# ushasigh/srsran-edgeric-5g

Measured on AMD Instinct MI355X. Metric: pdsch_slots_per_sec, higher is better.
Workload: dtype u32 bit-packed GF(2) + bf16 grid + f32 IQ

## Files before the change

### profiles/check_re_loop.py

```python
#!/usr/bin/env python3
import os
import subprocess
import tempfile

ROOT = os.path.dirname(os.path.dirname(os.path.abspath(__file__)))
C = os.path.join(ROOT, "srsran-edgeric-5g_amd", "csrc")
with tempfile.TemporaryDirectory() as tmp:
    subprocess.run(["/opt/rocm/bin/hipcc", "--offload-arch=gfx950", "-O3", "-std=c++17", "-fPIC", "-I" + os.path.join(ROOT, "include"), "-I" + C,
                    "-ffp-contract=off", "-x", "hip", "-c", os.path.join(C, "pdsch_kernels.hip"), "-o", os.path.join(tmp, "o.o"), "-save-temps"],
                   cwd=tmp, check=True, capture_output=True)
    isa = open(os.path.join(tmp, "pdsch_kernels-hip-amdgcn-amd-amdhsa-gfx950.s")).read().split("\n")
begin = next(i for i, l in enumerate(isa) if l.startswith("_ZN5nrphy18codeblock_kernel_tILi8ELi4EEE"))
end = next(i for i in range(begin, len(isa)) if "s_endpgm" in isa[i])
k = isa[begin:end + 1]
code = [l for l in k if l.startswith("\t") and not l.strip().startswith(";")]
print("codeblock_kernel_t<8, 4>: %d instructions, v_readlane %d, v_writelane %d (the v_readlane are the wave reductions' row folds)" % (
    len(code), sum("v_readlane" in l for l in code), sum("v_writelane" in l for l in code)))
idx = [i for i, l in enumerate(k) if "v_pk_mul_f32" in l and ", s[" in l][-16:]
start = max(i for i in range(idx[0]) if "Loop Header" in k[i])
stop = next(i for i in range(idx[-1], len(k)) if "s_cbranch" in k[i] or "s_endpgm" in k[i])
body = [l for l in k[start:stop + 1] if l.startswith("\t") and not l.strip().startswith(";")]
print("grid loop, four ports (from its loop header to the branch behind the last product): %d instructions" % len(body))
for what in ("v_pk_mul_f32", "v_pk_fma_f32", "v_pk_add_f32", "v_cvt_pk_bf16_f32", "buffer_store_dword", "ds_read", "global_load", "s_load", "v_readlane", "v_writelane"):
    print("  %-20s %d" % (what, sum(what in l for l in body)))
print("  scalar loads in the loop region (symbol change and the rare group that straddles a symbol; none per 64 RE, none of weights):")
for l in body:
    if "s_load" in l:
        print("     " + l.strip())
```

### srsran-edgeric-5g_amd/csrc/nrphy_host.cpp

```cpp
#include "nrphy_host_internal.h"
#include "nrphy_trace.h"

#include <algorithm>
#include <cmath>
#include <complex>
#include <cstdlib>
#include <cstring>
#include <array>
#include <map>
#include <mutex>
#include <new>
#include <vector>

using namespace nrphy;

namespace {

struct nr_ldpc_edge_t {
  uint8_t  row;
  uint8_t  col;
  uint16_t shift[8];
};
#include "nr_ldpc_bg.inc"

const uint16_t LIFTING_SIZES[NOF_LIFTING_SIZES] = {
    2,  3,  4,  5,  6,  7,  8,  9,  10, 11, 12, 13,  14,  15,  16,  18,  20,  22,  24,  26,  28,  30,  32,  36,  40, 44,
    48, 52, 56, 60, 64, 72, 80, 88, 96, 104, 112, 120, 128, 144, 160, 176, 192, 208, 224, 240, 256, 288, 320, 352, 384};

int lifting_position(unsigned zc)
{
  for (int i = 0; i != NOF_LIFTING_SIZES; ++i) {
    if (LIFTING_SIZES[i] == zc) {
      return i;
    }
  }
  return -1;
}

int lifting_set_index(unsigned zc)
{
  static const unsigned base[8] = {2, 3, 5, 7, 9, 11, 13, 15};
  for (int i = 0; i != 8; ++i) {
    for (unsigned v = base[i]; v <= 384; v *= 2) {
      if (v == zc) {
        return i;
      }
    }
  }
  return -1;
}

unsigned divide_ceil(unsigned a, unsigned b)
{
  return (a + b - 1) / b;
}

bool mask_test(const uint64_t* w, unsigned i)
{
  return (w[i >> 6] >> (i & 63)) & 1U;
}

int mask_lowest(const uint64_t* w)
{
  for (unsigned i = 0; i != 64 * NRPHY_PRB_WORDS; ++i) {
    if (mask_test(w, i)) {
      return (int)i;
    }
  }
  return -1;
}

int mask_highest(const uint64_t* w)
{
  int hi = -1;
  for (unsigned i = 0; i != 64 * NRPHY_PRB_WORDS; ++i) {
    if (mask_test(w, i)) {
      hi = (int)i;
    }
  }
  return hi;
}

void build_lifted_graph(unsigned bg, unsigned zc, LiftedGraph& g)
{
  const nr_ldpc_edge_t* edges   = (bg == 1) ? NR_LDPC_BG1_EDGES : NR_LDPC_BG2_EDGES;
  const unsigned        n_edges = (bg == 1) ? NR_LDPC_BG1_NOF_EDGES : NR_LDPC_BG2_NOF_EDGES;
  const unsigned        kb      = (bg == 1) ? 22 : 10;
  const unsigned        rows    = (bg == 1) ? 46 : 42;
  const int             ils     = lifting_set_index(zc);
  std::memset(&g, 0, sizeof(g));
  int      core_shift[4] = {-1, -1, -1, -1};
  unsigned count         = 0;
  for (unsigned m = 0; m != rows; ++m) {
    g.row_ptr[m] = (uint16_t)count;
    for (unsigned e = 0; e != n_edges; ++e) {
      if (edges[e].row != m) {
        continue;
      }
      unsigned col = edges[e].col, shift = edges[e].shift[ils] % zc;
      if (m < 4) {
        if (col == kb) {
          core_shift[m] = (int)shift;
        }
        if (col >= kb) {
          continue;
        }
      } else if (col >= kb + 4) {
        continue;
      }
      if (m < 4 && (zc & 31U) == 0) {
        const unsigned wpb = zc / 32, sh = shift & 31U, q = shift >> 5;
        const unsigned qd = (sh != 0) ? q : (q + wpb - 1) % wpb, sd = (32U - sh) & 31U;
        g.edge[count++] = ((4U * (2U * wpb * col + qd)) << 16) | sd;
        continue;
      }
      g.edge[count++] = ((col * zc) << 16) | shift;
    }
  }
  for (unsigned m = rows; m != MAX_BG_ROWS + 2; ++m) {
    g.row_ptr[m] = (uint16_t)count;
  }
  unsigned mid = (core_shift[1] >= 0) ? 1 : 2;
  int      s0 = core_shift[0], s3 = core_shift[3], sm = core_shift[mid];
  g.core_mid = (uint16_t)mid;
  g.core_s0  = (uint16_t)s0;
  g.core_s3  = (uint16_t)s3;
  g.core_b   = (uint16_t)((s0 == s3) ? sm : ((s0 == sm) ? s3 : s0));
}

void mat_mul(const uint32_t* a, const uint32_t* b, uint32_t* out)
{
  uint32_t bt[31];
  for (int c = 0; c != 31; ++c) {
    uint32_t col = 0;
    for (int r = 0; r != 31; ++r) {
      col |= ((b[r] >> c) & 1U) << r;
    }
    bt[c] = col;
  }
  uint32_t tmp[31];
  for (int r = 0; r != 31; ++r) {
    uint32_t row = 0;
    for (int c = 0; c != 31; ++c) {
      row |= (uint32_t)(__builtin_popcount(a[r] & bt[c]) & 1) << c;
    }
    tmp[r] = row;
  }
  std::memcpy(out, tmp, sizeof(tmp));
}


void build_tbcrc_tables(TbCrcTables& t)
{
  const CrcField* field[2] = {&CRC24A_FIELD, &CRC16_FIELD};
  for (unsigned s = 0; s != 2; ++s) {
    const CrcField& f  = *field[s];
    const uint32_t  y32 = f.xpow(32), y1k = f.xpow(32 * 1024), y8k = f.xpow(128 * 64), yz = f.xpow(8 * (int64_t)TB_CRC_REGION_BYTES);
    for (unsigned k = 0; k != 4; ++k) {
      for (uint32_t b = 0; b != 256; ++b) {
        t.y32[s][k][b] = f.mul(y32, b << (8 * k));
        t.y1k[s][k][b] = f.mul(y1k, b << (8 * k));
        t.y8k[s][k][b] = f.mul(y8k, b << (8 * k));
        t.yz[s][k][b]  = f.mul(yz, b << (8 * k));
      }
    }
    for (unsigned l = 0; l != 64; ++l) {
      t.lane[s][l] = f.xpow(128 * (63 - (int)l));
    }
  }
}

void build_gold_tables(GoldTables& t, std::vector<uint32_t>& x1_words)
{
  std::memset(&t, 0, sizeof(t));
  uint32_t m[31];
  for (int r = 0; r != 30; ++r) {
    m[r] = 1U << (r + 1);
  }
  m[30] = 0xF;
  for (int k = 0; k != GOLD_JUMP_BITS; ++k) {
    std::memcpy(t.x2_jump[k], m, sizeof(m));
    mat_mul(m, m, m);
  }
  for (int i = 0; i != 31; ++i) {
    uint32_t st = 1U << i;
    for (int n = 0; n != 992; ++n) {
      if (st & 1U) {
        t.x2_head[n & 31][n >> 5] |= 1U << i;
      }
      uint32_t f = ((st >> 3) ^ (st >> 2) ^ (st >> 1) ^ st) & 1U;
      st         = (st >> 1) | (f << 30);
    }
  }
  const uint32_t poly = 0x1800063U, top = 1U << 24;
  uint32_t       v    = 1;
  for (int i = 0; i != CRC_POW_WORDS; ++i) {
    t.crc24b_pow32[i] = v;
    for (int s = 0; s != 32; ++s) {
      v <<= 1;
      if (v & top) {
        v ^= poly;
      }
    }
  }
  for (uint32_t b = 0; b != 256; ++b) {
    uint32_t r = b << 16;
    for (int k = 0; k != 8; ++k) {
      r <<= 1;
      if (r & top) {
        r ^= poly;
      }
    }
    t.crc24b_table[b] = r & (top - 1);
  }
  for (uint32_t b = 0; b != 256; ++b) {
    uint32_t r            = t.crc24b_table[b];
    t.crc24b_slice[0][b] = r;
    for (int k = 1; k != 4; ++k) {
      for (int s = 0; s != 8; ++s) {
        r <<= 1;
        if (r & top) {
          r ^= poly;
        }
      }
      t.crc24b_slice[k][b] = r;
    }
  }
  {
    auto mulx = [&](uint32_t a, unsigned e) {
      for (unsigned s = 0; s != e; ++s) {
        a <<= 1;
        if (a & top) {
          a ^= poly;
        }
      }
      return a;
    };
    for (unsigned m = 0; m != CRC_POW_WORDS; ++m) {
      for (unsigned n = 0; n != 6; ++n) {
        uint32_t e = mulx(t.crc24b_pow32[m], 4 * n);
        uint32_t bit[4];
        for (unsigned k = 0; k != 4; ++k) {
          bit[k] = mulx(e, k);
        }
        for (uint32_t nib = 0; nib != 16; ++nib) {
          uint32_t acc = 0;
          for (unsigned k = 0; k != 4; ++k) {
            acc ^= ((nib >> k) & 1U) ? bit[k] : 0U;
          }
          t.crc24b_mul[m][n][nib] = acc;
        }
      }
    }
  }
  for (unsigned q = 0; q != 4; ++q) {
    const unsigned qm = 2 * (q + 1), h = q + 1;
    for (unsigned idx = 0; idx != (1U << qm); ++idx) {
      int re = 1 - 2 * (int)((idx >> 1) & 1U), im = 1 - 2 * (int)(idx & 1U);
      for (unsigned lvl = 1; lvl < h; ++lvl) {
        re = (1 - 2 * (int)((idx >> (2 * lvl + 1)) & 1U)) * ((1 << lvl) - re);
        im = (1 - 2 * (int)((idx >> (2 * lvl)) & 1U)) * ((1 << lvl) - im);
      }
      t.qam_lut[q][idx] = make_float2((float)re, (float)im);
    }
  }
  x1_words.assign(GOLD_X1_WORDS, 0);
  uint32_t x1 = 1;
  for (int i = 0; i != 1600; ++i) {
    uint32_t f = ((x1 >> 3) ^ x1) & 1U;
    x1         = (x1 >> 1) | (f << 30);
  }
  for (size_t n = 0; n != (size_t)GOLD_X1_WORDS * 32; ++n) {
    if (x1 & 1U) {
      x1_words[n >> 5] |= 0x80000000U >> (n & 31);
    }
    uint32_t f = ((x1 >> 3) ^ x1) & 1U;
    x1         = (x1 >> 1) | (f << 30);
  }
}

}

struct nrphy_pdsch_plan {
  nrphy_ctx*            ctx = nullptr;
  std::vector<PduDev>   pdus;
  std::vector<uint64_t> cw_offset;
  uint64_t              cw_bits = 0;
  uint32_t              nof_grids = 0, grid_nof_ports = 0, grid_nof_subc = 0;
  void*                 d_arena = nullptr;
  bool                  arena_external = false;
  PduDev*               d_pdus = nullptr;
  CbWork*               d_work = nullptr;
  DmrsWork*             d_dmrs = nullptr;
  float*                d_weights = nullptr;
  uint16_t*             d_re_table = nullptr;
  uint32_t*             d_tb_crc = nullptr;
  CrcWork*              d_crc_work = nullptr;
  ScrWork*              d_scr_work = nullptr;
  uint32_t              n_scr_work = 0;
  ZeroWork*             d_zero_work = nullptr;
  ZeroSeg*              d_zero_segs = nullptr;
  uint32_t*             d_scr = nullptr;
  uint64_t              scr_words = 0;
  uint64_t              seed_offset = 0;
  uint32_t              n_zero_work = 0;
  bool                  encode_only = false;
  bool                  dmrs_separate = false;
  uint32_t              n_work = 0, n_dmrs = 0, n_cb = 0, n_crc_work = 0;
  uint32_t              lds_lin_words = 0, lds_symb_words = 0, lds_graph_words = 0, lds_u_words = 0;
  uint32_t              bucket_begin[CB_BUCKETS + 1] = {};
  static constexpr uint32_t MAX_AUX = 3;
  hipStream_t           aux_stream[MAX_AUX] = {};
  hipEvent_t            fork_event = nullptr, join_event[MAX_AUX] = {};
  uint32_t              n_aux = 0;
  std::vector<hipEvent_t> events;
  std::vector<uint8_t>  timed_dmrs;
  uint32_t              timed_runs = 0, max_timed_runs = 0;
  uint32_t              timing_stride = 1, timing_counter = 0;
};

static bool plan_side_streams(nrphy_pdsch_plan* plan, uint32_t want);

struct nrphy_ofdm_plan {
  nrphy_ctx*          ctx = nullptr;
  nrphy_ofdm_config_t cfg;
  uint32_t            nof_ports = 0, nsymb = 14, slot_stride = 0, nsym_subframe = 0;
  const float2*       d_twiddle = nullptr;
  float2*             d_phase = nullptr;
  float2*             d_phase_rx = nullptr;
  uint32_t*           d_cp = nullptr;
  uint32_t*           d_off = nullptr;
  std::vector<uint32_t> cp, off;
  std::map<uint32_t, float2*> d_window_phase;
  std::mutex          window_mutex;
  std::vector<hipEvent_t> events;
  uint32_t            timed_runs = 0, max_timed_runs = 0;
  uint32_t            timing_stride = 1, timing_counter = 0;
  uint4*              d_wire_partials = nullptr;
  size_t              wire_partials_cap = 0;
};

extern "C" const char* nrphy_version(void)
{
  return "mi355-nrphy 0.1 (gfx950)";
}

extern "C" int nrphy_trace_enabled(void)
{
  return trace_enabled() ? 1 : 0;
}

extern "C" const char* nrphy_strerror(int status)
{
  switch (status) {
    case NRPHY_OK:
      return "ok";
    case NRPHY_ERR_INVALID_PDU:
      return "invalid PDSCH PDU (pdsch_pdu_validator::is_valid is false)";
    case NRPHY_ERR_ARGUMENT:
      return "invalid argument";
    case NRPHY_ERR_DEVICE:
      return "HIP device error (no GPU or kernel launch failure); there is no CPU fallback";
    case NRPHY_ERR_CAPACITY:
      return "capacity exceeded";
    default:
      return "unknown status";
  }
}

extern "C" int nrphy_pdsch_validate(const nrphy_pdsch_pdu_t* pdu)
{
  if (pdu == nullptr) {
    return NRPHY_ERR_ARGUMENT;
  }
  const unsigned nsymb = pdu->cp ? 12 : 14;
  const int      lo = mask_lowest(pdu->prb_mask), hi = mask_highest(pdu->prb_mask);
  if (lo < 0 || (unsigned)lo < pdu->bwp_start_rb || (unsigned)hi >= pdu->bwp_start_rb + pdu->bwp_size_rb ||
      pdu->bwp_start_rb + pdu->bwp_size_rb > NRPHY_MAX_RB) {
    return NRPHY_ERR_INVALID_PDU;
  }
  if (pdu->dmrs_symbol_mask == 0 || (pdu->dmrs_symbol_mask >> nsymb) != 0) {
    return NRPHY_ERR_INVALID_PDU;
  }
  const unsigned first_dmrs = (unsigned)__builtin_ctz(pdu->dmrs_symbol_mask);
  const unsigned last_dmrs  = 31U - (unsigned)__builtin_clz(pdu->dmrs_symbol_mask);
  if (first_dmrs < pdu->start_symbol_index || last_dmrs >= pdu->start_symbol_index + pdu->nof_symbols ||
      nsymb < pdu->start_symbol_index + pdu->nof_symbols) {
    return NRPHY_ERR_INVALID_PDU;
  }
  if (pdu->dmrs_type != 1 || pdu->nof_cdm_groups_without_data > 2 || !pdu->vrb_contiguous) {
    return NRPHY_ERR_INVALID_PDU;
  }
  for (int prb = lo; prb <= hi; ++prb) {
    if (!mask_test(pdu->prb_mask, (unsigned)prb)) {
      return NRPHY_ERR_INVALID_PDU;
    }
  }
  if (pdu->nof_ports == 0 || pdu->nof_ports > NRPHY_MAX_PORTS || pdu->nof_layers == 0 ||
      pdu->nof_layers > pdu->nof_ports) {
    return NRPHY_ERR_INVALID_PDU;
  }
  if (pdu->nof_codewords != 1 || pdu->tbs_lbrm_bytes == 0 || pdu->nof_reserved > NRPHY_MAX_RESERVED) {
    return NRPHY_ERR_INVALID_PDU;
  }
  for (unsigned r = 0; r != pdu->nof_reserved; ++r) {
    if (pdu->reserved[r].symbol_mask & pdu->dmrs_symbol_mask) {
      return NRPHY_ERR_INVALID_PDU;
    }
  }
  if ((pdu->qm != 2 && pdu->qm != 4 && pdu->qm != 6 && pdu->qm != 8) || pdu->rv > 3 ||
      (pdu->ldpc_base_graph != 1 && pdu->ldpc_base_graph != 2) || pdu->tb_size_bytes == 0 ||
      pdu->tb_size_bytes > NRPHY_MAX_TB_BYTES || pdu->nof_prg == 0 || pdu->nof_prg > NRPHY_MAX_PRG || pdu->prg_size_rb == 0 || pdu->prg_size_rb > NRPHY_MAX_RB || pdu->precoding == nullptr || pdu->cp > 1) {
    return NRPHY_ERR_INVALID_PDU;
  }
  return NRPHY_OK;
}

namespace {

void data_re_mask(const nrphy_pdsch_pdu_t& pdu, unsigned l, std::vector<uint8_t>& mask)
{
  std::fill(mask.begin(), mask.end(), 0);
  if (l < pdu.start_symbol_index || l >= pdu.start_symbol_index + pdu.nof_symbols) {
    return;
  }
  const unsigned nof_prb = (unsigned)mask.size() / 12;
  for (unsigned p = 0; p != nof_prb; ++p) {
    if (mask_test(pdu.prb_mask, p)) {
      std::fill(mask.begin() + 12 * p, mask.begin() + 12 * p + 12, 1);
    }
  }
  for (unsigned r = 0; r != pdu.nof_reserved; ++r) {
    const nrphy_re_pattern_t& pat = pdu.reserved[r];
    if (!((pat.symbol_mask >> l) & 1U)) {
      continue;
    }
    for (unsigned p = 0; p != nof_prb; ++p) {
      if (!mask_test(pat.prb_mask, p)) {
        continue;
      }
      for (unsigned k = 0; k != 12; ++k) {
        if ((pat.re_mask >> k) & 1U) {
          mask[12 * p + k] = 0;
        }
      }
    }
  }
  if ((pdu.dmrs_symbol_mask >> l) & 1U) {
    for (unsigned p = pdu.bwp_start_rb; p < pdu.bwp_start_rb + pdu.bwp_size_rb && p < nof_prb; ++p) {
      for (unsigned k = 0; k != 12; ++k) {
        if ((k % 2) < pdu.nof_cdm_groups_without_data) {
          mask[12 * p + k] = 0;
        }
      }
    }
  }
}

void derive(const nrphy_pdsch_pdu_t& pdu, unsigned nof_re, nrphy_pdsch_derived_t& d,
            const uint32_t* nref_override = nullptr)
{
  const unsigned bg      = pdu.ldpc_base_graph;
  const unsigned tb_bits = 8 * pdu.tb_size_bytes;
  const unsigned tb_crc  = (tb_bits <= 3824) ? 16 : 24;
  const unsigned b       = tb_bits + tb_crc;
  const unsigned kcb     = (bg == 1) ? 8448 : 3840;
  const unsigned C       = (b <= kcb) ? 1 : divide_ceil(b, kcb - 24);
  const unsigned b_out   = b + ((C > 1) ? 24 * C : 0);
  unsigned       ref_len = 22;
  if (bg == 2) {
    ref_len = (b > 640) ? 10 : (b > 560) ? 9 : (b > 192) ? 8 : 6;
  }
  unsigned zc = 0;
  for (unsigned i = 0; i != NOF_LIFTING_SIZES; ++i) {
    if (LIFTING_SIZES[i] * C * ref_len >= b_out) {
      zc = LIFTING_SIZES[i];
      break;
    }
  }
  const unsigned K      = ((bg == 1) ? 22 : 10) * zc;
  const unsigned cb_crc = (C > 1) ? 24 : 0;
  const unsigned info   = divide_ceil(b_out, C) - cb_crc;
  const unsigned N      = ((bg == 1) ? 66 : 50) * zc;
  uint64_t       nref   = ((uint64_t)pdu.tbs_lbrm_bytes * 8 * 3) / (2 * C);
  if (nref_override != nullptr) {
    nref = *nref_override;
  }
  nref                  = std::min<uint64_t>(nref, 66 * 384);
  d.nof_re              = nof_re;
  d.nof_codeblocks      = C;
  d.lifting_size        = zc;
  d.segment_length      = K;
  d.cb_info_bits        = info;
  d.nof_filler_bits     = K - info - cb_crc;
  d.nof_tb_crc_bits     = tb_crc;
  d.nof_cb_crc_bits     = cb_crc;
  d.zero_pad            = (info + cb_crc) * C - b_out;
  d.full_length         = N;
  d.n_ref               = (uint32_t)nref;
  d.n_cb                = (nref > 0 && nref < N) ? (uint32_t)nref : N;
  static const double shift_bg1[4] = {0, 17, 33, 56};
  static const double shift_bg2[4] = {0, 13, 25, 43};
  const double tmp      = (((bg == 1) ? shift_bg1 : shift_bg2)[pdu.rv] * d.n_cb) / N;
  d.k0                  = (uint32_t)((uint16_t)std::floor(tmp)) * zc;
  d.nof_short_segments  = C - (nof_re % C);
  d.rm_length_short     = (nof_re / C) * pdu.nof_layers * pdu.qm;
  d.rm_length_long      = divide_ceil(nof_re, C) * pdu.nof_layers * pdu.qm;
  d.codeword_bits       = nof_re * pdu.nof_layers * pdu.qm;
}

unsigned count_data_re(const nrphy_pdsch_pdu_t& pdu)
{
  std::vector<uint8_t> mask(NRPHY_MAX_RB * 12);
  unsigned             count = 0;
  for (unsigned l = 0; l != NRPHY_NSYMB; ++l) {
    data_re_mask(pdu, l, mask);
    for (uint8_t m : mask) {
      count += m;
    }
  }
  return count;
}

}

extern "C" int nrphy_pdsch_derive(const nrphy_pdsch_pdu_t* pdu, nrphy_pdsch_derived_t* out)
{
  if (pdu == nullptr || out == nullptr || pdu->tb_size_bytes == 0 || pdu->nof_layers == 0 || pdu->qm == 0 ||
      (pdu->ldpc_base_graph != 1 && pdu->ldpc_base_graph != 2) || pdu->rv > 3) {
    return NRPHY_ERR_ARGUMENT;
  }
  derive(*pdu, count_data_re(*pdu), *out);
  return NRPHY_OK;
}

extern "C" uint32_t nrphy_tbs_calculate(uint32_t nof_symb_sh, uint32_t nof_dmrs_prb, uint32_t nof_oh_prb, uint32_t qm,
                                        float target_code_rate, uint32_t nof_layers, uint32_t n_prb)
{
  static const uint16_t table[93] = {
      24,   32,   40,   48,   56,   64,   72,   80,   88,   96,   104,  112,  120,  128,  136,  144,  152,  160,  168,
      176,  184,  192,  208,  224,  240,  256,  272,  288,  304,  320,  336,  352,  368,  384,  408,  432,  456,  480,
      504,  528,  552,  576,  608,  640,  672,  704,  736,  768,  808,  848,  888,  928,  984,  1032, 1064, 1128, 1160,
      1192, 1224, 1256, 1288, 1320, 1352, 1416, 1480, 1544, 1608, 1672, 1736, 1800, 1864, 1928, 2024, 2088, 2152, 2216,
      2280, 2408, 2472, 2536, 2600, 2664, 2728, 2792, 2856, 2976, 3104, 3240, 3368, 3496, 3624, 3752, 3824};
  const unsigned nof_re_prime = 12 * nof_symb_sh - nof_dmrs_prb - nof_oh_prb;
  const unsigned nof_re       = std::min(nof_re_prime, 156U) * n_prb;
  const float    tcr          = target_code_rate * (1.F / 1024);
  const float    nof_info     = 1.0F * (float)nof_re * tcr * (float)qm * (float)nof_layers;
  if (nof_info <= 3824) {
    unsigned n = 3;
    if (nof_info > 512) {
      n = (unsigned)std::floor(std::log2(nof_info)) - 6U;
    }
    const unsigned p2    = 1U << n;
    const unsigned prime = std::max(24U, p2 * (unsigned)std::floor(nof_info / (float)p2));
    for (uint16_t v : table) {
      if (v >= prime) {
        return v;
      }
    }
    return 3824;
  }
  const unsigned n     = (unsigned)(std::floor(std::log2(nof_info - 24)) - 5.0F);
  const unsigned p2    = 1U << n;
  const unsigned prime = std::max(3840U, p2 * (unsigned)std::round((nof_info - 24) / (float)p2));
  unsigned       C     = 1;
  if (tcr <= 0.25F) {
    C = divide_ceil(prime + 24, 3816);
  } else if (prime > 8424) {
    C = divide_ceil(prime + 24, 8424);
  }
  return 8 * C * divide_ceil(prime + 24, 8 * C) - 24;
}

namespace {

unsigned cp_length(const nrphy_ofdm_config_t& c, unsigned symbol_index)
{
  const unsigned mu    = c.numerology;
  unsigned       units = 144U >> mu;
  if (c.cp) {
    units = 512U >> mu;
  } else if (symbol_index == 0 || symbol_index == 7U * (1U << mu)) {
    units += 16;
  }
  return (unsigned)(((uint64_t)units * c.dft_size * (1U << mu)) / 2048U);
}

}

extern "C" uint32_t nrphy_ofdm_symbol_size(const nrphy_ofdm_config_t* cfg, uint32_t symbol_index)
{
  return cp_length(*cfg, symbol_index) + cfg->dft_size;
}

extern "C" uint32_t nrphy_ofdm_slot_size(const nrphy_ofdm_config_t* cfg, uint32_t slot_index)
{
  const unsigned nsymb = cfg->cp ? 12 : 14;
  unsigned       n     = 0;
  for (unsigned l = 0; l != nsymb; ++l) {
    n += nrphy_ofdm_symbol_size(cfg, nsymb * slot_index + l);
  }
  return n;
}


Tunables read_tunables()
{
  Tunables t;
  auto     number = [](const char* name, int unset) {
    const char* e = std::getenv(name);
    return (e != nullptr && e[0] != 0) ? std::atoi(e) : unset;
  };
  t.cb_dispatch       = number("NRPHY_CB_DISPATCH", 0);
  t.crc_regions       = number("NRPHY_CRC_REGIONS", 0);
  t.scr_parts_big     = number("NRPHY_SCR_PARTS_BIG", 0);
  t.extras_nt         = (uint32_t)number("NRPHY_EXTRAS_NT", 1);
  t.prologue_order    = (uint32_t)number("NRPHY_PROLOGUE_ORDER", 0);
  t.decoder_pairs     = number("NRPHY_DECODER_PAIRS", -1);
  t.decoder_msg       = number("NRPHY_DECODER_MSG", -1);
  t.decoder_ldsmsg    = number("NRPHY_DECODER_LDSMSG", -1);
  t.decoder_slots_all = number("NRPHY_DECODER_SLOTS_ALL", 0) == 1;
#ifdef NRPHY_PROBES
  t.profile_stage = (uint32_t)number("NRPHY_PROFILE_STAGE", 0);
  t.ofdm_probe    = (uint32_t)number("NRPHY_OFDM_PROBE", 0);
#endif
  return t;
}

extern "C" int nrphy_create(nrphy_ctx_t** out, int device_id)
{
  if (out == nullptr) {
    return NRPHY_ERR_ARGUMENT;
  }
  *out      = nullptr;
  int count = 0;
  if (hipGetDeviceCount(&count) != hipSuccess || count <= 0 || device_id < 0 || device_id >= count) {
    return NRPHY_ERR_DEVICE;
  }
  HIP_TRY(hipSetDevice(device_id));
  nrphy_ctx* ctx = new (std::nothrow) nrphy_ctx;
  if (ctx == nullptr) {
    return NRPHY_ERR_CAPACITY;
  }
  ctx->device = device_id;
  ctx->tune   = read_tunables();
  {
    hipDeviceProp_t prop;
    if (hipGetDeviceProperties(&prop, device_id) == hipSuccess && prop.multiProcessorCount > 0) {
      ctx->nof_cus = (uint32_t)prop.multiProcessorCount;
    }
  }
  if (hipStreamCreateWithFlags(&ctx->stream, hipStreamNonBlocking) != hipSuccess) {
    delete ctx;
    return NRPHY_ERR_DEVICE;
  }
  std::vector<LiftedGraph> graphs(NOF_GRAPHS);
  for (unsigned bg = 1; bg <= 2; ++bg) {
    for (int i = 0; i != NOF_LIFTING_SIZES; ++i) {
      build_lifted_graph(bg, LIFTING_SIZES[i], graphs[(bg - 1) * NOF_LIFTING_SIZES + i]);
    }
  }
  GoldTables            gold;
  std::vector<uint32_t> x1;
  build_gold_tables(gold, x1);
  ctx->graphs = graphs;
  std::vector<TbCrcTables> tbcrc(1);
  build_tbcrc_tables(tbcrc[0]);
  if (upload(&ctx->d_tbcrc, tbcrc.data(), sizeof(TbCrcTables)) != hipSuccess ||
      upload(&ctx->d_graphs, graphs.data(), graphs.size() * sizeof(LiftedGraph)) != hipSuccess ||
      upload(&ctx->d_gold, &gold, sizeof(gold)) != hipSuccess ||
      upload(&ctx->d_x1, x1.data(), x1.size() * sizeof(uint32_t)) != hipSuccess) {
    nrphy_destroy(ctx);
    return NRPHY_ERR_DEVICE;
  }
  *out = ctx;
  return NRPHY_OK;
}

extern "C" int nrphy_destroy(nrphy_ctx_t* ctx)
{
  if (ctx == nullptr) {
    return NRPHY_OK;
  }
  (void)hipSetDevice(ctx->device);
  (void)hipFree(ctx->d_graphs);
  (void)hipFree(ctx->d_gold);
  (void)hipFree(ctx->d_tbcrc);
  for (void* b : ctx->scratch) {
    (void)hipFree(b);
  }
  for (DecoderGraph* g : ctx->d_dec_graph) {
    (void)hipFree(g);
  }
  for (uint32_t* a : ctx->d_dec_addr) {
    (void)hipFree(a);
  }
  for (auto& kv : ctx->d_dec_crc) {
    (void)hipFree(kv.second);
  }
  for (auto& kv : ctx->d_tb_crc_w) {
    (void)hipFree(kv.second);
  }
  (void)hipFree(ctx->d_x1);
  for (auto& kv : ctx->d_twiddle) {
    (void)hipFree(kv.second);
  }
  if (ctx->stream) {
    (void)hipStreamDestroy(ctx->stream);
  }
  delete ctx;
  return NRPHY_OK;
}

extern "C" int nrphy_synchronize(nrphy_ctx_t* ctx, void* stream)
{
  if (ctx == nullptr) {
    return NRPHY_ERR_ARGUMENT;
  }
  HIP_TRY(hipStreamSynchronize(stream ? (hipStream_t)stream : ctx->stream));
  return NRPHY_OK;
}

namespace {

const float2* get_twiddle(nrphy_ctx* ctx, uint32_t size)
{
  if (!dft_size_supported(size)) {
    return nullptr;
  }
  std::lock_guard<std::recursive_mutex> lock(ctx->host_mutex);
  auto it = ctx->d_twiddle.find(size);
  if (it != ctx->d_twiddle.end()) {
    return it->second;
  }
  std::vector<float2> tw(size);
  for (uint32_t k = 0; k != size; ++k) {
    double ang = 2.0 * M_PI * (double)k / (double)size;
    tw[k]      = make_float2((float)std::cos(ang), (float)std::sin(ang));
  }
  float2* d = nullptr;
  if (upload(&d, tw.data(), tw.size() * sizeof(float2)) != hipSuccess) {
    return nullptr;
  }
  ctx->d_twiddle[size] = d;
  return d;
}

}

namespace {

void append_allocation_signature(const nrphy_pdsch_pdu_t& pdu, std::vector<uint64_t>& sig)
{
  sig.insert(sig.end(), std::begin(pdu.prb_mask), std::end(pdu.prb_mask));
  sig.push_back(((uint64_t)pdu.start_symbol_index << 48) | ((uint64_t)pdu.nof_symbols << 40) |
                ((uint64_t)pdu.nof_cdm_groups_without_data << 36) | ((uint64_t)pdu.nof_layers << 32) |
                pdu.dmrs_symbol_mask);
  sig.push_back(((uint64_t)pdu.bwp_start_rb << 32) | ((uint64_t)pdu.bwp_size_rb << 8) | pdu.nof_reserved);
  for (unsigned r = 0; r != pdu.nof_reserved; ++r) {
    sig.insert(sig.end(), std::begin(pdu.reserved[r].prb_mask), std::end(pdu.reserved[r].prb_mask));
    sig.push_back(((uint64_t)pdu.reserved[r].re_mask << 32) | pdu.reserved[r].symbol_mask);
  }
}

struct ReMapping {
  uint32_t sym_re_start[NRPHY_NSYMB + 1];
  uint32_t sym_kind[NRPHY_NSYMB];
  uint32_t sym_arg[NRPHY_NSYMB];
};

}

struct PlanShapeCache {
  struct Remap {
    ReMapping             m;
    std::vector<uint16_t> table;
  };
  struct Zero {
    std::vector<ZeroSeg> segs;
    uint32_t             nof_long = 0;
  };
  std::map<std::vector<uint64_t>, Remap> remap;
  std::map<std::vector<uint64_t>, Zero>  zero;
  static constexpr size_t MAX_ENTRIES = 256;
};

PlanShapeCache* plan_shape_cache_create()
{
  return new (std::nothrow) PlanShapeCache;
}
void plan_shape_cache_destroy(PlanShapeCache* c)
{
  delete c;
}

namespace {

struct EncodeOnly {
  uint32_t nof_re;
  uint32_t nref;
};

int plan_create(nrphy_ctx_t* ctx, uint32_t n_pdu, const nrphy_pdsch_pdu_t* pdus, const uint64_t* tb_offset,
                const uint32_t* grid_index, uint32_t nof_grids, uint32_t grid_nof_ports, uint32_t grid_nof_subc,
                const EncodeOnly* enc, nrphy_pdsch_plan_t** out, PlanPlacement* place = nullptr);

}

int nrphy_pdsch_plan_create_placed(nrphy_ctx_t* ctx, uint32_t n_pdu, const nrphy_pdsch_pdu_t* pdus, const uint64_t* tb_offset,
                                   const uint32_t* grid_index, uint32_t nof_grids, uint32_t grid_nof_ports,
                                   uint32_t grid_nof_subc, PlanPlacement* place, nrphy_pdsch_plan_t** out)
{
  return plan_create(ctx, n_pdu, pdus, tb_offset, grid_index, nof_grids, grid_nof_ports, grid_nof_subc, nullptr, out, place);
}

extern "C" int nrphy_pdsch_plan_create(nrphy_ctx_t* ctx, uint32_t n_pdu, const nrphy_pdsch_pdu_t* pdus,
                                       const uint64_t* tb_offset, const uint32_t* grid_index, uint32_t nof_grids,
                                       uint32_t grid_nof_ports, uint32_t grid_nof_subc, nrphy_pdsch_plan_t** out)
{
  return plan_create(ctx, n_pdu, pdus, tb_offset, grid_index, nof_grids, grid_nof_ports, grid_nof_subc, nullptr, out);
}

namespace {

int plan_create(nrphy_ctx_t* ctx, uint32_t n_pdu, const nrphy_pdsch_pdu_t* pdus, const uint64_t* tb_offset,
                const uint32_t* grid_index, uint32_t nof_grids, uint32_t grid_nof_ports, uint32_t grid_nof_subc,
                const EncodeOnly* enc, nrphy_pdsch_plan_t** out, PlanPlacement* place)
{
  if (ctx == nullptr || out == nullptr || (n_pdu != 0 && (pdus == nullptr || tb_offset == nullptr)) ||
      grid_nof_ports == 0 || grid_nof_ports > NRPHY_MAX_PORTS || grid_nof_subc == 0 || grid_nof_subc % 12 != 0 ||
      grid_nof_subc > NRPHY_MAX_RB * 12) {
    return NRPHY_ERR_ARGUMENT;
  }
  *out = nullptr;
  if (place == nullptr) {
    HIP_TRY(hipSetDevice(ctx->device));
  }
  nrphy_pdsch_plan* plan = new (std::nothrow) nrphy_pdsch_plan;
  if (plan == nullptr) {
    return NRPHY_ERR_CAPACITY;
  }
  PlanShapeCache* shapes = place ? place->cache : nullptr;
  if (shapes != nullptr && shapes->remap.size() + shapes->zero.size() > PlanShapeCache::MAX_ENTRIES) {
    shapes->remap.clear();
    shapes->zero.clear();
  }
  plan->ctx            = ctx;
  plan->nof_grids      = nof_grids;
  plan->grid_nof_ports = grid_nof_ports;
  plan->grid_nof_subc  = grid_nof_subc;
  plan->encode_only    = enc != nullptr;

  std::vector<CbWork>   work;
  std::vector<DmrsWork> dmrs;
  std::vector<CrcWork>  crc_work;
  std::vector<uint64_t> remap_sig;
  std::map<std::vector<uint64_t>, ReMapping> remap_cache;
  std::vector<ScrWork>  scr_work;
  std::vector<std::vector<uint32_t>> pdus_of_grid(nof_grids);
  std::vector<float>    weights;
  std::vector<uint16_t> re_table;
  std::vector<uint8_t>  mask(grid_nof_subc);
  std::vector<uint16_t> list;
  uint64_t              cw_bits = 0;
  int                   status  = NRPHY_OK;

  for (uint32_t i = 0; i != n_pdu && status == NRPHY_OK; ++i) {
    const nrphy_pdsch_pdu_t& pdu = pdus[i];
    if (enc == nullptr ? nrphy_pdsch_validate(&pdu) != NRPHY_OK
                       : (pdu.qm < 2 || pdu.qm > 8 || (pdu.qm & 1U) || pdu.rv > 3 || pdu.nof_layers == 0 ||
                          pdu.nof_layers > NRPHY_MAX_LAYERS || pdu.tb_size_bytes == 0 ||
                          pdu.tb_size_bytes > NRPHY_MAX_TB_BYTES || (pdu.ldpc_base_graph != 1 && pdu.ldpc_base_graph != 2))) {
      status = NRPHY_ERR_INVALID_PDU;
      break;
    }
    const uint32_t g = grid_index ? grid_index[i] : 0;
    if (g >= nof_grids || pdu.nof_ports > grid_nof_ports || (tb_offset[i] & 3U) != 0 ||
        (enc == nullptr && 12U * (unsigned)(mask_highest(pdu.prb_mask) + 1) > grid_nof_subc)) {
      status = NRPHY_ERR_ARGUMENT;
      break;
    }
    PduDev pd;
    std::memset(&pd, 0, sizeof(pd));
    unsigned nof_re = 0;
    remap_sig.clear();
    append_allocation_signature(pdu, remap_sig);
    auto cached = remap_cache.find(remap_sig);
    if (enc != nullptr) {
      nof_re = enc[i].nof_re;
      for (unsigned l = 0; l <= NRPHY_NSYMB; ++l) {
        pd.sym_re_start[l] = (l == NRPHY_NSYMB) ? nof_re : 0;
      }
    } else if (cached != remap_cache.end()) {
      std::memcpy(pd.sym_re_start, cached->second.sym_re_start, sizeof(pd.sym_re_start));
      std::memcpy(pd.sym_kind, cached->second.sym_kind, sizeof(pd.sym_kind));
      std::memcpy(pd.sym_arg, cached->second.sym_arg, sizeof(pd.sym_arg));
      nof_re = pd.sym_re_start[NRPHY_NSYMB];
    } else {
      PlanShapeCache::Remap        built;
      const PlanShapeCache::Remap* rel = nullptr;
      if (shapes != nullptr) {
        auto known = shapes->remap.find(remap_sig);
        if (known != shapes->remap.end()) {
          rel = &known->second;
        }
      }
      if (rel == nullptr) {
        for (unsigned l = 0; l != NRPHY_NSYMB; ++l) {
          built.m.sym_re_start[l] = nof_re;
          built.m.sym_arg[l]      = 0;
          data_re_mask(pdu, l, mask);
          list.clear();
          for (unsigned k = 0; k != grid_nof_subc; ++k) {
            if (mask[k]) {
              list.push_back((uint16_t)k);
            }
          }
          if (list.empty()) {
            built.m.sym_kind[l] = SYM_NONE;
          } else if ((unsigned)(list.back() - list.front()) + 1 == list.size()) {
            built.m.sym_kind[l] = SYM_CONTIGUOUS;
            built.m.sym_arg[l]  = list.front();
          } else {
            built.m.sym_kind[l] = SYM_TABLE;
            built.m.sym_arg[l]  = (uint32_t)built.table.size();
            for (unsigned lp = 0; lp != l; ++lp) {
              if (built.m.sym_kind[lp] == SYM_TABLE && built.m.sym_re_start[lp + 1] - built.m.sym_re_start[lp] == list.size() &&
                  std::equal(list.begin(), list.end(), built.table.begin() + built.m.sym_arg[lp])) {
                built.m.sym_arg[l] = built.m.sym_arg[lp];
                break;
              }
            }
            if (built.m.sym_arg[l] == built.table.size()) {
              built.table.insert(built.table.end(), list.begin(), list.end());
            }
          }
          nof_re += (unsigned)list.size();
          built.m.sym_re_start[l + 1] = nof_re;
        }
        rel = &built;
        if (shapes != nullptr) {
          rel = &shapes->remap.insert({remap_sig, built}).first->second;
        }
      }
      const uint32_t base = (uint32_t)re_table.size();
      re_table.insert(re_table.end(), rel->table.begin(), rel->table.end());
      std::memcpy(pd.sym_re_start, rel->m.sym_re_start, sizeof(pd.sym_re_start));
      std::memcpy(pd.sym_kind, rel->m.sym_kind, sizeof(pd.sym_kind));
      for (unsigned l = 0; l != NRPHY_NSYMB; ++l) {
        pd.sym_arg[l] = rel->m.sym_arg[l] + (rel->m.sym_kind[l] == SYM_TABLE ? base : 0U);
      }
      nof_re = pd.sym_re_start[NRPHY_NSYMB];
      ReMapping m;
      std::memcpy(m.sym_re_start, pd.sym_re_start, sizeof(m.sym_re_start));
      std::memcpy(m.sym_kind, pd.sym_kind, sizeof(m.sym_kind));
      std::memcpy(m.sym_arg, pd.sym_arg, sizeof(m.sym_arg));
      remap_cache.insert({remap_sig, m});
    }
    if (nof_re == 0) {
      status = NRPHY_ERR_INVALID_PDU;
      break;
    }
    nrphy_pdsch_derived_t d;
    derive(pdu, nof_re, d, enc ? &enc[i].nref : nullptr);
    if (d.lifting_size == 0 || d.nof_codeblocks > NRPHY_MAX_CODEBLOCKS || d.nof_codeblocks > nof_re ||
        d.rm_length_short == 0) {
      status = NRPHY_ERR_INVALID_PDU;
      break;
    }
    const unsigned kb = (pdu.ldpc_base_graph == 1) ? 22 : 10;
    pd.tb_offset      = tb_offset[i];
    pd.cw_bit_offset  = cw_bits;
    pd.tb_bytes       = pdu.tb_size_bytes;
    pd.grid_index     = g;
    pd.graph          = (pdu.ldpc_base_graph - 1) * NOF_LIFTING_SIZES + (uint32_t)lifting_position(d.lifting_size);
    pd.zc             = d.lifting_size;
    pd.kb             = kb;
    pd.K              = d.segment_length;
    pd.info_bits      = d.cb_info_bits;
    pd.filler         = d.nof_filler_bits;
    pd.tb_crc_bits    = d.nof_tb_crc_bits;
    pd.cb_crc_bits    = d.nof_cb_crc_bits;
    pd.zero_pad       = d.zero_pad;
    pd.C              = d.nof_codeblocks;
    pd.n_short        = d.nof_short_segments;
    pd.e_short        = d.rm_length_short;
    pd.e_long         = d.rm_length_long;
    pd.n_cb           = d.n_cb;
    pd.k0             = d.k0;
    pd.qm             = pdu.qm;
    pd.nof_layers     = pdu.nof_layers;
    pd.nof_ports      = pdu.nof_ports;
    pd.c_init         = (pdu.rnti << 15) + pdu.n_id;
    pd.nof_re         = nof_re;
    {
      const unsigned nsys = (kb - 2) * d.lifting_size;
      unsigned       fs = std::min(nsys - d.nof_filler_bits, d.n_cb), fe = std::min(nsys, d.n_cb);
      const unsigned flen = fe - fs, n_valid = d.n_cb - flen;
      const unsigned rank0 = d.k0 < fs ? d.k0 : (d.k0 < fe ? fs : d.k0 - flen);
      unsigned       last;
      if (rank0 + d.rm_length_long > n_valid) {
        last = d.n_cb - 1;
      } else {
        unsigned u = rank0 + d.rm_length_long - 1;
        last       = u < fs ? u : u + flen;
      }
      const unsigned nodes = divide_ceil(last + 1 + 2 * d.lifting_size, d.lifting_size);
      pd.nof_rows          = std::max(4U, nodes > kb ? nodes - kb : 0U);
    }
    {
      const float avg     = (pdu.qm == 2) ? 2.0F : (pdu.qm == 4) ? 10.0F : (pdu.qm == 6) ? 42.0F : 170.0F;
      float       scaling = std::sqrt(1 / avg);
      const float cfg     = std::pow(10.0F, -pdu.ratio_pdsch_data_to_sss_dB / 20.0F);
      if (std::isnormal(cfg)) {
        scaling *= cfg;
      }
      const unsigned nw      = 2 * pdu.nof_prg * pdu.nof_ports * pdu.nof_layers;
      pd.weights_offset      = (uint32_t)weights.size();
      for (unsigned k = 0; k != nw; ++k) {
        weights.push_back(pdu.precoding ? pdu.precoding[k] * scaling : 0.0F);
      }
      pd.dmrs_weights_offset = (uint32_t)weights.size();
      for (unsigned k = 0; k != nw; ++k) {
        weights.push_back(pdu.precoding ? pdu.precoding[k] : 0.0F);
      }
      pd.nof_prg       = pdu.nof_prg;
      pd.prg_size_subc = pdu.prg_size_rb * 12;
    }
    pd.dmrs_symbol_mask = pdu.dmrs_symbol_mask;
    pd.dmrs_zero_other_group = (pdu.nof_cdm_groups_without_data == 2 && (pdu.nof_layers + 1) / 2 == 1) ? 1U : 0U;
    pd.dmrs_ref_rb      = (pdu.ref_point == 1) ? pdu.bwp_start_rb : 0;
    {
      const float amp   = std::pow(10.0F, -pdu.ratio_pdsch_dmrs_to_sss_dB / 20.0F);
      pd.dmrs_amplitude = (float)(M_SQRT1_2 * (double)amp);
    }
    for (unsigned l = 0; l != NRPHY_NSYMB; ++l) {
      const uint64_t a  = (uint64_t)(14 * pdu.slot_index + l + 1) * (2 * pdu.scrambling_id + 1);
      pd.dmrs_c_init[l] = (uint32_t)(((a << 17) + (2 * pdu.scrambling_id + (pdu.n_scid ? 1 : 0))) & 0x7FFFFFFFULL);
      if ((pdu.dmrs_symbol_mask >> l) & 1U) {
        const uint32_t first = (uint32_t)mask_lowest(pdu.prb_mask), end = (uint32_t)mask_highest(pdu.prb_mask) + 1;
        for (uint32_t b = first; b < end; b += DMRS_PRB_CHUNK) {
          dmrs.push_back({i, l, b, std::min<uint32_t>(end, b + DMRS_PRB_CHUNK)});
        }
      }
    }
    for (unsigned w = 0; w != NRPHY_PRB_WORDS; ++w) {
      pd.prb_mask[2 * w]     = (uint32_t)pdu.prb_mask[w];
      pd.prb_mask[2 * w + 1] = (uint32_t)(pdu.prb_mask[w] >> 32);
    }
    pd.first_prb = (uint32_t)mask_lowest(pdu.prb_mask);
    pd.end_prb   = (uint32_t)mask_highest(pdu.prb_mask) + 1;
    if (pdu.nof_cdm_groups_without_data < (pdu.nof_layers + 1) / 2) {
      plan->dmrs_separate = true;
    }
    pdus_of_grid[g].push_back(i);
    {
      const CrcField& f = (d.nof_tb_crc_bits == 16) ? CRC16_FIELD : CRC24A_FIELD;
      const uint32_t  n = pdu.tb_size_bytes;
      const uint32_t  regions = divide_ceil(n, TB_CRC_REGION_BYTES);
      const uint32_t  want  = std::max<uint32_t>(1, std::min<uint32_t>(regions, TB_CRC_TARGET_WORK / std::max<uint32_t>(1, n_pdu)));
      uint32_t        per   = std::min<uint32_t>(TB_CRC_MAX_REGIONS_PER_WORK, divide_ceil(regions, want));
      if (ctx->tune.crc_regions > 0) {
        per = std::max(1, std::min((int)TB_CRC_MAX_REGIONS_PER_WORK, ctx->tune.crc_regions));
      }
      pd.crc_first      = (uint32_t)crc_work.size();
      pd.crc_count      = divide_ceil(regions, per);
      if (pd.crc_count > 64) {
        status = NRPHY_ERR_INVALID_PDU;
        break;
      }
      for (uint32_t region = 0; region < regions; region += per) {
        const uint32_t count      = std::min(per, regions - region);
        const int64_t  region_end = (int64_t)(region + count) * TB_CRC_REGION_BYTES;
        crc_work.push_back({i, region, f.xpow((int64_t)f.order + 8 * ((int64_t)n - region_end)), count});
      }
    }
    const unsigned lq = pdu.nof_layers * pdu.qm;
    for (unsigned cb = 0; cb != d.nof_codeblocks; ++cb) {
      const unsigned nre = ((cb < d.nof_short_segments) ? d.rm_length_short : d.rm_length_long) / lq;
      for (unsigned begin = 0; begin < nre; begin += RE_CHUNK) {
        const unsigned count = std::min<unsigned>(RE_CHUNK, nre - begin);
        work.push_back({i, cb, begin, count});
        {
          const uint64_t bit0 = (uint64_t)(cb < d.nof_short_segments ? cb * d.rm_length_short
                                                                     : d.nof_short_segments * d.rm_length_short +
                                                                           (cb - d.nof_short_segments) * d.rm_length_long) +
                                (uint64_t)begin * lq;
          const uint32_t need = std::max<uint32_t>(31U, (uint32_t)(((bit0 & 31U) + (uint64_t)count * lq + 31U) / 32U) + 1U);
          plan->lds_lin_words = std::max<uint32_t>(plan->lds_lin_words, (need + 3U) & ~3U);
        }
        plan->lds_symb_words = std::max<uint32_t>(plan->lds_symb_words,
                                                  (((count * pdu.nof_layers + 31) / 32) * 8 + 8 + 3) & ~3U);
      }
    }
    plan->lds_lin_words = std::max<uint32_t>(plan->lds_lin_words,
                                             ((((kb + pd.nof_rows) * d.lifting_size + 31) / 32) + 2 + 3) & ~3U);
    plan->lds_graph_words = std::max<uint32_t>(
        plan->lds_graph_words, (48U + ctx->graphs[pd.graph].row_ptr[std::min<uint32_t>(pd.nof_rows, MAX_BG_ROWS)] + 3U) & ~3U);
    pd.scr_words  = (d.codeword_bits + 31U) / 32U + 1U + 31U;
    pd.dmrs_seq_offset = (uint32_t)plan->scr_words;
    pd.dmrs_seq_words  = (12U * (pd.end_prb - pd.dmrs_ref_rb) + 31U) / 32U + 1U;
    plan->scr_words += ((uint64_t)pd.dmrs_seq_words * (unsigned)__builtin_popcount(pdu.dmrs_symbol_mask) + 3U) & ~3ULL;
    {
      const uint32_t     parts_big = ctx->tune.scr_parts_big > 0 ? (uint32_t)std::min((int)SCR_PARTS, ctx->tune.scr_parts_big) : 1U;
      const uint32_t parts_max = n_pdu >= 128 ? parts_big : SCR_PARTS;
      const uint32_t parts     = std::min<uint32_t>(parts_max, std::max<uint32_t>(1, pd.scr_words >> 11));
      const uint32_t chunk = divide_ceil(pd.scr_words, parts);
      for (uint32_t first = 0, k = 0; first < pd.scr_words; first += chunk, ++k) {
        scr_work.push_back({i, first, std::min(chunk, pd.scr_words - first), k == 0 ? 1U : 0U});
      }
    }
    plan->n_cb += d.nof_codeblocks;
    plan->cw_offset.push_back(cw_bits);
    cw_bits += (d.codeword_bits + 31U) & ~31ULL;
    plan->pdus.push_back(pd);
  }
  if (status != NRPHY_OK) {
    delete plan;
    return status;
  }
  std::vector<ZeroWork> zero_work;
  std::vector<ZeroSeg>  zero_segs;
  {
    std::map<std::vector<uint64_t>, std::array<uint32_t, 3>> seen;
    std::vector<uint8_t>  cov((size_t)NRPHY_NSYMB * grid_nof_subc);
    std::vector<uint64_t> key, sig;
    std::map<std::vector<uint64_t>, std::array<uint32_t, 3>> by_signature;
    for (uint32_t g = 0; g != (enc ? 0U : nof_grids); ++g) {
      for (uint32_t port = 0; port != grid_nof_ports; ++port) {
        sig.clear();
        for (uint32_t i : pdus_of_grid[g]) {
          const nrphy_pdsch_pdu_t& pdu = pdus[i];
          if (port >= pdu.nof_ports) {
            continue;
          }
          append_allocation_signature(pdu, sig);
        }
        auto known = by_signature.find(sig);
        if (known != by_signature.end()) {
          if (known->second[1] != 0) {
            zero_work.push_back({g, port, known->second[0], known->second[1], known->second[2]});
          }
          continue;
        }
        if (shapes != nullptr) {
          sig.push_back(((uint64_t)grid_nof_subc << 32) | port);
          auto kept = shapes->zero.find(sig);
          sig.pop_back();
          if (kept != shapes->zero.end()) {
            const std::array<uint32_t, 3> where = {(uint32_t)zero_segs.size(), (uint32_t)kept->second.segs.size(),
                                                   kept->second.nof_long};
            zero_segs.insert(zero_segs.end(), kept->second.segs.begin(), kept->second.segs.end());
            by_signature.insert({sig, where});
            if (where[1] != 0) {
              zero_work.push_back({g, port, where[0], where[1], where[2]});
            }
            continue;
          }
        }
        std::fill(cov.begin(), cov.end(), 0);
        for (uint32_t i : pdus_of_grid[g]) {
          const nrphy_pdsch_pdu_t& pdu = pdus[i];
          if (port >= pdu.nof_ports) {
            continue;
          }
          for (unsigned l = 0; l != NRPHY_NSYMB; ++l) {
            uint8_t* row = &cov[(size_t)l * grid_nof_subc];
            data_re_mask(pdu, l, mask);
            for (unsigned k = 0; k != grid_nof_subc; ++k) {
              row[k] |= mask[k];
            }
            if ((pdu.dmrs_symbol_mask >> l) & 1U) {
              const unsigned groups = (pdu.nof_cdm_groups_without_data == 2) ? 2 : (pdu.nof_layers + 1) / 2;
              for (unsigned prb = 0; 12 * prb < grid_nof_subc; ++prb) {
                if (mask_test(pdu.prb_mask, prb)) {
                  for (unsigned k = 0; k != 12; ++k) {
                    row[12 * prb + k] |= (k % 2) < groups;
                  }
                }
              }
            }
          }
        }
        key.clear();
        for (unsigned l = 0; l != NRPHY_NSYMB; ++l) {
          const uint8_t* row = &cov[(size_t)l * grid_nof_subc];
          unsigned       k   = 0;
          while (k < grid_nof_subc) {
            if (row[k]) {
              ++k;
              continue;
            }
            unsigned k0 = k;
            while (k < grid_nof_subc && !row[k]) {
              ++k;
            }
            key.push_back(((uint64_t)l << 32) | ((uint64_t)k0 << 16) | (k - k0));
          }
        }
        if (key.empty()) {
          by_signature.insert({sig, {0, 0, 0}});
          if (shapes != nullptr) {
            sig.push_back(((uint64_t)grid_nof_subc << 32) | port);
            shapes->zero.insert({sig, PlanShapeCache::Zero()});
            sig.pop_back();
          }
          continue;
        }
        auto it = seen.find(key);
        if (it == seen.end()) {
          const uint32_t begin = (uint32_t)zero_segs.size();
          uint32_t       nof_long = 0;
          for (int pass = 0; pass != 2; ++pass) {
            for (uint64_t v : key) {
              const bool is_long = (v & 0xFFFF) >= ZERO_LONG_RUN;
              if (is_long == (pass == 0)) {
                zero_segs.push_back({(uint16_t)(v >> 32), (uint16_t)((v >> 16) & 0xFFFF), (uint16_t)(v & 0xFFFF), 0});
                nof_long += is_long ? 1U : 0U;
              }
            }
          }
          it = seen.insert({key, {begin, (uint32_t)key.size(), nof_long}}).first;
        }
        by_signature.insert({sig, it->second});
        zero_work.push_back({g, port, it->second[0], it->second[1], it->second[2]});
        if (shapes != nullptr) {
          PlanShapeCache::Zero z;
          z.segs.assign(zero_segs.begin() + it->second[0], zero_segs.begin() + it->second[0] + it->second[1]);
          z.nof_long = it->second[2];
          sig.push_back(((uint64_t)grid_nof_subc << 32) | port);
          shapes->zero.insert({sig, std::move(z)});
          sig.pop_back();
        }
      }
    }
  }
  plan->n_zero_work = (uint32_t)zero_work.size();
  plan->cw_bits = cw_bits;
  plan->n_work  = (uint32_t)work.size();
  {
    const auto bucket_of = [&](const CbWork& w) { return cb_bucket(plan->pdus[w.pdu].qm, plan->pdus[w.pdu].nof_layers); };
    std::stable_sort(work.begin(), work.end(), [&](const CbWork& a, const CbWork& b) { return bucket_of(a) < bucket_of(b); });
    for (const CbWork& w : work) {
      ++plan->bucket_begin[bucket_of(w) + 1];
    }
    for (uint32_t b = 0; b != CB_BUCKETS; ++b) {
      plan->bucket_begin[b + 1] += plan->bucket_begin[b];
    }
    for (size_t k = work.size(); k-- != 0;) {
      plan->pdus[work[k].pdu].item_first = (uint32_t)k;
    }
    plan->scr_words  = (plan->scr_words + 3U) & ~3ULL;
    plan->seed_offset = plan->scr_words;
    plan->scr_words += 32ULL * work.size();
    weights.insert(weights.end(), 2 * NRPHY_MAX_PORTS * NRPHY_MAX_PORTS, 0.0F);
  }
  plan->n_dmrs  = (uint32_t)dmrs.size();
  plan->n_crc_work = (uint32_t)crc_work.size();
  plan->n_scr_work = (uint32_t)scr_work.size();
  {
    DeviceArena          arena;
    arena.add(&plan->d_crc_work, crc_work.data(), crc_work.size() * sizeof(CrcWork));
    arena.add(&plan->d_scr_work, scr_work.data(), scr_work.size() * sizeof(ScrWork));
    arena.add(&plan->d_pdus, plan->pdus.data(), plan->pdus.size() * sizeof(PduDev));
    arena.add(&plan->d_work, work.data(), work.size() * sizeof(CbWork));
    arena.add(&plan->d_dmrs, dmrs.data(), dmrs.size() * sizeof(DmrsWork));
    arena.add(&plan->d_weights, weights.data(), weights.size() * sizeof(float));
    arena.add(&plan->d_re_table, re_table.data(), re_table.size() * sizeof(uint16_t));
    arena.add(&plan->d_zero_work, zero_work.data(), zero_work.size() * sizeof(ZeroWork));
    arena.add(&plan->d_zero_segs, zero_segs.data(), zero_segs.size() * sizeof(ZeroSeg));
    void* scratch = nullptr;
    const uint64_t scr_alloc = (std::max<uint64_t>(4, plan->scr_words) + 3U) & ~3ULL;
    const uint64_t scratch_words = scr_alloc + std::max<size_t>(4, crc_work.size());
    if (place != nullptr) {
      if (arena.bytes() > place->table_capacity || scratch_words > place->scratch_capacity_words) {
        delete plan;
        return NRPHY_ERR_CAPACITY;
      }
      arena.place(place->h_tables, place->d_tables);
      place->table_bytes  = arena.bytes();
      plan->arena_external = true;
      scratch              = place->d_scratch;
    } else if (arena.commit(&plan->d_arena, sizeof(uint32_t) * scratch_words, &scratch) != hipSuccess) {
      nrphy_pdsch_plan_destroy(plan);
      return NRPHY_ERR_DEVICE;
    }
    plan->d_scr    = (uint32_t*)scratch;
    plan->d_tb_crc = plan->d_scr + scr_alloc;
  }
  {
    uint32_t nof_buckets = 0;
    for (uint32_t b = 0; b != CB_BUCKETS; ++b) {
      nof_buckets += plan->bucket_begin[b + 1] != plan->bucket_begin[b] ? 1U : 0U;
    }
    if (place == nullptr && nof_buckets > 1 && plan->n_work >= CB_MIXED_MAX_WORK &&
        !plan_side_streams(plan, std::min<uint32_t>(nof_buckets - 1, nrphy_pdsch_plan::MAX_AUX))) {
      nrphy_pdsch_plan_destroy(plan);
      return NRPHY_ERR_DEVICE;
    }
  }
  plan->lds_lin_words = std::max<uint32_t>(plan->lds_lin_words, 64);
  plan->lds_u_words = std::max<uint32_t>({256U * NRPHY_CRC_SLICES, NRPHY_CB_U_GRAPH_OFFSET + plan->lds_graph_words, 512U + plan->lds_symb_words});
  *out = plan;
  return NRPHY_OK;
}

}

static bool plan_side_streams(nrphy_pdsch_plan* plan, uint32_t want)
{
  while (plan->n_aux < want) {
    const uint32_t k = plan->n_aux;
    if (plan->fork_event == nullptr && hipEventCreateWithFlags(&plan->fork_event, hipEventDisableTiming) != hipSuccess) {
      return false;
    }
    if (hipStreamCreateWithFlags(&plan->aux_stream[k], hipStreamNonBlocking) != hipSuccess) {
      return false;
    }
    if (hipEventCreateWithFlags(&plan->join_event[k], hipEventDisableTiming) != hipSuccess) {
      (void)hipStreamDestroy(plan->aux_stream[k]);
      return false;
    }
    ++plan->n_aux;
  }
  return true;
}

extern "C" int nrphy_pdsch_plan_destroy(nrphy_pdsch_plan_t* plan)
{
  if (plan == nullptr) {
    return NRPHY_OK;
  }
  if (!plan->arena_external) {
    (void)hipSetDevice(plan->ctx->device);
    (void)hipFree(plan->d_arena);
  }
  for (uint32_t k = 0; k != plan->n_aux; ++k) {
    (void)hipStreamDestroy(plan->aux_stream[k]);
    (void)hipEventDestroy(plan->join_event[k]);
  }
  if (plan->fork_event != nullptr) {
    (void)hipEventDestroy(plan->fork_event);
  }
  for (hipEvent_t e : plan->events) {
    (void)hipEventDestroy(e);
  }
  delete plan;
  return NRPHY_OK;
}

extern "C" uint32_t nrphy_pdsch_plan_nof_codeblocks(const nrphy_pdsch_plan_t* plan)
{
  return plan ? plan->n_cb : 0;
}

extern "C" uint64_t nrphy_pdsch_plan_codeword_bits(const nrphy_pdsch_plan_t* plan)
{
  return plan ? plan->cw_bits : 0;
}

extern "C" uint64_t nrphy_pdsch_plan_codeword_offset(const nrphy_pdsch_plan_t* plan, uint32_t pdu)
{
  return (plan && pdu < plan->cw_offset.size()) ? plan->cw_offset[pdu] : 0;
}

extern "C" int nrphy_pdsch_run(nrphy_pdsch_plan_t* plan, const uint8_t* d_tb, void* d_grid, uint8_t* d_cw_rm,
                               uint8_t* d_cw_scrambled, int zero_grids, void* stream)
{
  if (plan == nullptr || d_tb == nullptr || (plan->encode_only && d_grid != nullptr)) {
    return NRPHY_ERR_ARGUMENT;
  }
  const TraceRange trace_run("process_pdsch");
  nrphy_ctx*  ctx = plan->ctx;
  hipStream_t s   = stream ? (hipStream_t)stream : ctx->stream;
  PdschLaunch p;
  p.pdus           = plan->d_pdus;
  p.work           = plan->d_work;
  p.dmrs_work      = plan->d_dmrs;
  p.crc_work       = plan->d_crc_work;
  p.scr_work       = plan->d_scr_work;
  p.n_scr_work     = plan->n_scr_work;
  p.tbcrc          = ctx->d_tbcrc;
  p.n_crc_work     = plan->n_crc_work;
  p.weights        = plan->d_weights;
  p.re_table       = plan->d_re_table;
  p.graphs         = ctx->d_graphs;
  p.gold           = ctx->d_gold;
  p.x1_words       = ctx->d_x1;
  p.tb_crc_part        = plan->d_tb_crc;
  const bool merge_dmrs = d_grid != nullptr && !plan->dmrs_separate;
  p.zero_work          = plan->d_zero_work;
  p.zero_segs          = plan->d_zero_segs;
  p.scr                = plan->d_scr;
  p.scr_seed           = plan->d_scr + plan->seed_offset;
  p.n_zero_work        = (d_grid != nullptr && zero_grids) ? plan->n_zero_work : 0;
  p.zero_fill          = (d_grid != nullptr && zero_grids) ? 1U : 0U;
  p.n_dmrs_in_launch   = merge_dmrs ? plan->n_dmrs : 0;
  p.n_pdu          = (uint32_t)plan->pdus.size();
  p.n_work         = plan->n_work;
  p.work_base      = 0;
  p.n_dmrs_work    = plan->n_dmrs;
  p.grid_nof_ports = plan->grid_nof_ports;
  p.grid_nof_subc  = plan->grid_nof_subc;
  p.lds_lin_words  = plan->lds_lin_words;
  p.lds_u_words    = plan->lds_u_words;
  p.extras_nt      = ctx->tune.extras_nt;
  p.prologue_order = ctx->tune.prologue_order;
#ifdef NRPHY_PROBES
  p.profile_stage = ctx->tune.profile_stage;
#else
  p.profile_stage = 0;
#endif
  const size_t cw_bytes = (size_t)(plan->cw_bits / 8);
  if (d_cw_rm) {
    HIP_TRY(hipMemsetAsync(d_cw_rm, 0, cw_bytes, s));
  }
  if (d_cw_scrambled) {
    HIP_TRY(hipMemsetAsync(d_cw_scrambled, 0, cw_bytes, s));
  }
  hipEvent_t* ev = nullptr;
  if (plan->timed_runs < plan->max_timed_runs && plan->timing_counter++ % plan->timing_stride == 0) {
    ev = &plan->events[4 * plan->timed_runs++];
    HIP_TRY(hipEventRecord(ev[0], s));
  }
  HIP_TRY(launch_prologue(p, d_tb, s));
  if (ev) {
    HIP_TRY(hipEventRecord(ev[1], s));
  }
  {
    const TraceRange trace_cb("CB batch");
    const int   dispatch     = ctx->tune.cb_dispatch;
    uint32_t    nof_buckets  = 0;
    hipStream_t streams[1 + nrphy_pdsch_plan::MAX_AUX] = {s};
    uint32_t    n_streams = 1;
    if (codeblocks_take_bucket_launches(p, plan->bucket_begin, dispatch, &nof_buckets) && nof_buckets > 1) {
      const uint32_t want = std::min<uint32_t>(nof_buckets - 1, nrphy_pdsch_plan::MAX_AUX);
      if (!plan_side_streams(plan, want)) {
        return NRPHY_ERR_DEVICE;
      }
      HIP_TRY(hipEventRecord(plan->fork_event, s));
      for (uint32_t k = 0; k != want; ++k) {
        HIP_TRY(hipStreamWaitEvent(plan->aux_stream[k], plan->fork_event, 0));
        streams[n_streams++] = plan->aux_stream[k];
      }
    }
    HIP_TRY(launch_codeblocks(p, plan->bucket_begin, dispatch, d_tb, (uint32_t*)d_grid, (uint32_t*)d_cw_rm,
                              (uint32_t*)d_cw_scrambled, streams, n_streams));
    for (uint32_t k = 1; k < n_streams; ++k) {
      HIP_TRY(hipEventRecord(plan->join_event[k - 1], streams[k]));
      HIP_TRY(hipStreamWaitEvent(s, plan->join_event[k - 1], 0));
    }
  }
  if (ev) {
    HIP_TRY(hipEventRecord(ev[2], s));
  }
  if (d_grid && !merge_dmrs) {
    const TraceRange trace_dmrs("process_dmrs");
    HIP_TRY(launch_dmrs(p, (uint32_t*)d_grid, s));
    if (ev) {
      HIP_TRY(hipEventRecord(ev[3], s));
    }
  }
  if (ev) {
    plan->timed_dmrs[plan->timed_runs - 1] = (d_grid && !merge_dmrs) ? 1 : 0;
  }
  return NRPHY_OK;
}

extern "C" int nrphy_pdsch_plan_enable_timing(nrphy_pdsch_plan_t* plan, uint32_t max_runs)
{
  if (plan == nullptr) {
    return NRPHY_ERR_ARGUMENT;
  }
  for (hipEvent_t e : plan->events) {
    (void)hipEventDestroy(e);
  }
  plan->events.assign(4 * (size_t)max_runs, nullptr);
  for (hipEvent_t& e : plan->events) {
    HIP_TRY(hipEventCreate(&e));
  }
  plan->timed_dmrs.assign(max_runs, 0);
  plan->max_timed_runs = max_runs;
  plan->timed_runs     = 0;
  plan->timing_counter = 0;
  return NRPHY_OK;
}

extern "C" int nrphy_pdsch_plan_timing_stride(nrphy_pdsch_plan_t* plan, uint32_t stride)
{
  if (plan == nullptr || stride == 0) {
    return NRPHY_ERR_ARGUMENT;
  }
  plan->timing_stride  = stride;
  plan->timing_counter = 0;
  return NRPHY_OK;
}

extern "C" int nrphy_pdsch_plan_kernel_times(nrphy_pdsch_plan_t* plan, float avg_ms[4], uint32_t* nof_runs)
{
  if (plan == nullptr || avg_ms == nullptr) {
    return NRPHY_ERR_ARGUMENT;
  }
  double sum[4] = {0, 0, 0, 0};
  for (uint32_t r = 0; r != plan->timed_runs; ++r) {
    hipEvent_t*    ev   = &plan->events[4 * r];
    const unsigned last = plan->timed_dmrs[r] ? 3 : 2;
    HIP_TRY(hipEventSynchronize(ev[last]));
    float ms = 0;
    for (unsigned k = 0; k != last; ++k) {
      HIP_TRY(hipEventElapsedTime(&ms, ev[k], ev[k + 1]));
      sum[k] += ms;
    }
    HIP_TRY(hipEventElapsedTime(&ms, ev[0], ev[last]));
    sum[3] += ms;
  }
  for (int k = 0; k != 4; ++k) {
    avg_ms[k] = plan->timed_runs ? (float)(sum[k] / plan->timed_runs) : 0.f;
  }
  if (nof_runs) {
    *nof_runs = plan->timed_runs;
  }
  plan->timed_runs = 0;
  return NRPHY_OK;
}

extern "C" int nrphy_pdsch_process_host(nrphy_ctx_t* ctx, const nrphy_pdsch_pdu_t* pdu, const uint8_t* tb, void* grid,
                                        uint32_t grid_nof_ports, uint32_t grid_nof_subc, uint8_t* cw_rm,
                                        uint8_t* cw_scrambled)
{
  if (ctx == nullptr || pdu == nullptr || tb == nullptr) {
    return NRPHY_ERR_ARGUMENT;
  }
  HostCall            call(ctx);
  nrphy_pdsch_plan_t* plan   = nullptr;
  uint64_t            tb_off = 0;
  uint32_t            gi     = 0;
  int rc = nrphy_pdsch_plan_create(ctx, 1, pdu, &tb_off, &gi, 1, grid_nof_ports, grid_nof_subc, &plan);
  if (rc != NRPHY_OK) {
    return rc;
  }
  const size_t tb_alloc   = ((size_t)pdu->tb_size_bytes + 7) & ~(size_t)3;
  const size_t grid_bytes = (size_t)grid_nof_ports * NRPHY_NSYMB * grid_nof_subc * 4;
  const size_t cw_bytes   = (size_t)(plan->cw_bits / 8);
  uint8_t* d_tb   = call.mem<uint8_t>(SCRATCH_TB, tb_alloc);
  uint8_t* d_grid = grid ? call.mem<uint8_t>(SCRATCH_GRID, grid_bytes) : nullptr;
  uint8_t* d_rm   = cw_rm ? call.mem<uint8_t>(SCRATCH_CW_RM, cw_bytes) : nullptr;
  uint8_t* d_scr  = cw_scrambled ? call.mem<uint8_t>(SCRATCH_CW_SCR, cw_bytes) : nullptr;
  rc = NRPHY_ERR_DEVICE;
  do {
    if (d_tb == nullptr || (grid && d_grid == nullptr) || (cw_rm && d_rm == nullptr) ||
        (cw_scrambled && d_scr == nullptr)) {
      break;
    }
    if (hipMemsetAsync(d_tb + (tb_alloc - 8), 0, 8, ctx->stream) != hipSuccess ||
        hipMemcpyAsync(d_tb, tb, pdu->tb_size_bytes, hipMemcpyHostToDevice, ctx->stream) != hipSuccess) {
      break;
    }
    if (grid && hipMemcpyAsync(d_grid, grid, grid_bytes, hipMemcpyHostToDevice, ctx->stream) != hipSuccess) {
      break;
    }
    rc = nrphy_pdsch_run(plan, d_tb, d_grid, d_rm, d_scr, 0, ctx->stream);
    if (rc != NRPHY_OK) {
      break;
    }
    rc = NRPHY_ERR_DEVICE;
    nrphy_pdsch_derived_t d;
    nrphy_pdsch_derive(pdu, &d);
    const size_t cw_out = (d.codeword_bits + 7) / 8;
    if (grid && hipMemcpyAsync(grid, d_grid, grid_bytes, hipMemcpyDeviceToHost, ctx->stream) != hipSuccess) {
      break;
    }
    if (cw_rm && hipMemcpyAsync(cw_rm, d_rm, cw_out, hipMemcpyDeviceToHost, ctx->stream) != hipSuccess) {
      break;
    }
    if (cw_scrambled && hipMemcpyAsync(cw_scrambled, d_scr, cw_out, hipMemcpyDeviceToHost, ctx->stream) != hipSuccess) {
      break;
    }
    if (call.sync() != hipSuccess) {
      break;
    }
    rc = NRPHY_OK;
  } while (false);
  nrphy_pdsch_plan_destroy(plan);
  return rc;
}

extern "C" int nrphy_pdsch_process_slot_host(nrphy_ctx_t* ctx, uint32_t n_pdu, const nrphy_pdsch_pdu_t* pdus,
                                             const uint8_t* const* tbs, void* grid, uint32_t grid_nof_ports, uint32_t grid_nof_subc)
{
  if (ctx == nullptr || grid == nullptr || (n_pdu != 0 && (pdus == nullptr || tbs == nullptr))) {
    return NRPHY_ERR_ARGUMENT;
  }
  if (n_pdu == 0) {
    return NRPHY_OK;
  }
  std::vector<uint64_t> tb_off(n_pdu);
  std::vector<uint32_t> grid_of(n_pdu, 0);
  size_t                tb_total = 0;
  for (uint32_t i = 0; i != n_pdu; ++i) {
    if (tbs[i] == nullptr) {
      return NRPHY_ERR_ARGUMENT;
    }
    tb_off[i] = tb_total;
    tb_total += ((size_t)pdus[i].tb_size_bytes + 7) & ~(size_t)3;
  }
  HostCall            call(ctx);
  nrphy_pdsch_plan_t* plan = nullptr;
  int rc = nrphy_pdsch_plan_create(ctx, n_pdu, pdus, tb_off.data(), grid_of.data(), 1, grid_nof_ports, grid_nof_subc, &plan);
  if (rc != NRPHY_OK) {
    return rc;
  }
  const size_t grid_bytes = (size_t)grid_nof_ports * NRPHY_NSYMB * grid_nof_subc * 4;
  uint8_t* d_tb   = call.mem<uint8_t>(SCRATCH_TB, tb_total + 8);
  uint8_t* d_grid = call.mem<uint8_t>(SCRATCH_GRID, grid_bytes);
  rc              = NRPHY_ERR_DEVICE;
  do {
    if (d_tb == nullptr || d_grid == nullptr || hipMemsetAsync(d_tb, 0, tb_total + 8, ctx->stream) != hipSuccess) {
      break;
    }
    bool ok = true;
    for (uint32_t i = 0; ok && i != n_pdu; ++i) {
      ok = hipMemcpyAsync(d_tb + tb_off[i], tbs[i], pdus[i].tb_size_bytes, hipMemcpyHostToDevice, ctx->stream) == hipSuccess;
    }
    if (!ok || hipMemcpyAsync(d_grid, grid, grid_bytes, hipMemcpyHostToDevice, ctx->stream) != hipSuccess) {
      break;
    }
    rc = nrphy_pdsch_run(plan, d_tb, d_grid, nullptr, nullptr, 0, ctx->stream);
    if (rc != NRPHY_OK) {
      break;
    }
    rc = NRPHY_ERR_DEVICE;
    if (hipMemcpyAsync(grid, d_grid, grid_bytes, hipMemcpyDeviceToHost, ctx->stream) != hipSuccess ||
        call.sync() != hipSuccess) {
      break;
    }
    rc = NRPHY_OK;
  } while (false);
  nrphy_pdsch_plan_destroy(plan);
  return rc;
}

extern "C" int nrphy_pdsch_encode_host(nrphy_ctx_t* ctx, const nrphy_pdsch_encoder_cfg_t* cfg, const uint8_t* tb,
                                       uint8_t* codeword_bits, uint8_t* codeword_packed)
{
  if (ctx == nullptr || cfg == nullptr || tb == nullptr || cfg->nof_layers == 0 ||
      cfg->nof_ch_symbols % cfg->nof_layers != 0) {
    return NRPHY_ERR_ARGUMENT;
  }
  nrphy_pdsch_pdu_t pdu;
  std::memset(&pdu, 0, sizeof(pdu));
  pdu.qm              = cfg->qm;
  pdu.rv              = cfg->rv;
  pdu.nof_codewords   = 1;
  pdu.ldpc_base_graph = cfg->base_graph;
  pdu.tb_size_bytes   = cfg->tb_size_bytes;
  pdu.nof_layers      = cfg->nof_layers;
  pdu.nof_ports       = 1;
  pdu.nof_prg         = 1;
  pdu.prg_size_rb     = NRPHY_MAX_RB;
  pdu.tbs_lbrm_bytes  = 1;
  const EncodeOnly    enc    = {cfg->nof_ch_symbols / cfg->nof_layers, cfg->nref};
  std::vector<uint8_t> packed_local;
  HostCall             call(ctx);
  nrphy_pdsch_plan_t* plan   = nullptr;
  uint64_t            tb_off = 0;
  uint32_t            gi     = 0;
  int                 rc     = plan_create(ctx, 1, &pdu, &tb_off, &gi, 1, 1, 12, &enc, &plan);
  if (rc != NRPHY_OK) {
    return rc;
  }
  const size_t cw_bits  = (size_t)cfg->nof_ch_symbols * cfg->qm;
  const size_t cw_bytes = (size_t)(plan->cw_bits / 8);
  const size_t tb_alloc = ((size_t)cfg->tb_size_bytes + 7) & ~(size_t)3;
  uint8_t*     packed   = codeword_packed;
  if (packed == nullptr) {
    packed_local.resize((cw_bits + 7) / 8);
    packed = packed_local.data();
  }
  uint8_t* d_tb = call.mem<uint8_t>(SCRATCH_TB, tb_alloc);
  uint8_t* d_rm = call.mem<uint8_t>(SCRATCH_CW_RM, cw_bytes);
  rc            = NRPHY_ERR_DEVICE;
  do {
    if (d_tb == nullptr || d_rm == nullptr ||
        hipMemsetAsync(d_tb + (tb_alloc - 8), 0, 8, ctx->stream) != hipSuccess ||
        hipMemcpyAsync(d_tb, tb, cfg->tb_size_bytes, hipMemcpyHostToDevice, ctx->stream) != hipSuccess) {
      break;
    }
    rc = nrphy_pdsch_run(plan, d_tb, nullptr, d_rm, nullptr, 0, ctx->stream);
    if (rc != NRPHY_OK) {
      break;
    }
    rc = NRPHY_ERR_DEVICE;
    if (hipMemcpyAsync(packed, d_rm, (cw_bits + 7) / 8, hipMemcpyDeviceToHost, ctx->stream) != hipSuccess ||
        call.sync() != hipSuccess) {
      break;
    }
    rc = NRPHY_OK;
  } while (false);
  nrphy_pdsch_plan_destroy(plan);
  if (rc == NRPHY_OK && codeword_bits != nullptr) {
    for (size_t i = 0; i != cw_bits; ++i) {
      codeword_bits[i] = (packed[i >> 3] >> (7U - (i & 7U))) & 1U;
    }
  }
  return rc;
}

namespace {
// ... 1809 lines not shown
```

### srsran-edgeric-5g_amd/csrc/nrphy_host_internal.h

```cpp
#pragma once

#include "nrphy_internal.h"

#include <algorithm>
#include <cstring>
#include <map>
#include <mutex>
#include <vector>

using namespace nrphy;

#define HIP_TRY(expr)                                                                                                  \
  do {                                                                                                                 \
    if ((expr) != hipSuccess) {                                                                                        \
      return NRPHY_ERR_DEVICE;                                                                                         \
    }                                                                                                                  \
  } while (0)

namespace {

struct CrcField {
  uint32_t poly, order;
  uint32_t mul(uint32_t a, uint32_t b) const
  {
    const uint32_t top = 1U << order;
    uint32_t       r   = 0;
    for (int k = 31; k >= 0; --k) {
      r <<= 1;
      if (r & top) {
        r ^= poly;
      }
      if ((b >> k) & 1U) {
        r ^= a;
      }
    }
    return r;
  }
  uint32_t xpow(int64_t e) const
  {
    uint32_t base = (e >= 0) ? 2U : (poly >> 1);
    uint64_t n    = (uint64_t)(e >= 0 ? e : -e);
    uint32_t r    = 1;
    while (n) {
      if (n & 1U) {
        r = mul(r, base);
      }
      base = mul(base, base);
      n >>= 1;
    }
    return r;
  }
};
const CrcField CRC24A_FIELD = {0x1864CFBU, 24};
const CrcField CRC16_FIELD  = {0x11021U, 16};

template <typename T>
hipError_t upload(T** dptr, const void* src, size_t bytes)
{
  *dptr = nullptr;
  if (bytes == 0) {
    bytes = 16;
    hipError_t e = hipMalloc((void**)dptr, bytes);
    return e;
  }
  hipError_t e = hipMalloc((void**)dptr, bytes);
  if (e != hipSuccess) {
    return e;
  }
  return hipMemcpy(*dptr, src, bytes, hipMemcpyHostToDevice);
}

class DeviceArena
{
public:
  template <typename T>
  void add(T** dptr, const void* src, size_t bytes)
  {
    items.push_back({(void**)dptr, src, bytes, total});
    total += (bytes + 255) & ~(size_t)255;
  }
  size_t bytes() const { return std::max<size_t>(total, 256); }
  void place(uint8_t* h_base, uint8_t* d_base)
  {
    for (const Item& it : items) {
      if (it.bytes != 0) {
        std::memcpy(h_base + it.offset, it.src, it.bytes);
      }
      *it.dptr = d_base + it.offset;
    }
  }
  hipError_t commit(void** base, size_t scratch_bytes, void** scratch)
  {
    std::vector<uint8_t> staging(std::max<size_t>(total, 256), 0);
    for (const Item& it : items) {
      if (it.bytes != 0) {
        std::memcpy(&staging[it.offset], it.src, it.bytes);
      }
    }
    hipError_t e = hipMalloc(base, staging.size() + scratch_bytes);
    if (e != hipSuccess) {
      return e;
    }
    for (const Item& it : items) {
      *it.dptr = (uint8_t*)*base + it.offset;
    }
    *scratch = (uint8_t*)*base + staging.size();
    return hipMemcpy(*base, staging.data(), staging.size(), hipMemcpyHostToDevice);
  }

private:
  struct Item {
    void**      dptr;
    const void* src;
    size_t      bytes, offset;
  };
  std::vector<Item> items;
  size_t            total = 0;
};

}

struct Tunables {
  int      cb_dispatch     = 0;
  int      crc_regions     = 0;
  int      scr_parts_big   = 0;
  uint32_t extras_nt       = 1;
  uint32_t prologue_order  = 0;
  int      decoder_pairs   = -1;
  int      decoder_msg     = -1;
  int      decoder_ldsmsg  = -1;
  bool     decoder_slots_all = false;
#ifdef NRPHY_PROBES
  uint32_t profile_stage   = 0;
  uint32_t ofdm_probe      = 0;
#endif
};
Tunables read_tunables();

enum ScratchSlot { SCRATCH_TB = 0, SCRATCH_GRID, SCRATCH_CW_RM, SCRATCH_CW_SCR, SCRATCH_IQ, SCRATCH_SMALL,
                   SCRATCH_DECODER, SCRATCH_RX, SCRATCH_COUNT };

struct nrphy_ctx {
  int          device   = 0;
  Tunables     tune;
  uint32_t     nof_cus  = 256;
  hipStream_t  stream   = nullptr;
  LiftedGraph* d_graphs = nullptr;
  GoldTables*  d_gold   = nullptr;
  TbCrcTables* d_tbcrc  = nullptr;
  uint32_t*    d_x1     = nullptr;
  std::map<uint32_t, float2*> d_twiddle;
  DecoderGraph* d_dec_graph[NOF_GRAPHS] = {};
  uint32_t*     d_dec_addr[NOF_GRAPHS]  = {};
  std::map<uint64_t, uint32_t*> d_dec_crc;
  std::map<uint32_t, uint32_t*> d_tb_crc_w;
  std::vector<LiftedGraph> graphs;
  std::recursive_mutex host_mutex;
  void*      scratch[SCRATCH_COUNT]       = {};
  size_t     scratch_bytes[SCRATCH_COUNT] = {};
};

struct PlanShapeCache;
PlanShapeCache* plan_shape_cache_create();
void            plan_shape_cache_destroy(PlanShapeCache* cache);
struct PlanPlacement {
  uint8_t*        h_tables = nullptr;
  uint8_t*        d_tables = nullptr;
  size_t          table_capacity = 0;
  size_t          table_bytes    = 0;
  uint32_t*       d_scratch = nullptr;
  size_t          scratch_capacity_words = 0;
  PlanShapeCache* cache = nullptr;
};
int nrphy_pdsch_plan_create_placed(nrphy_ctx_t* ctx, uint32_t n_pdu, const nrphy_pdsch_pdu_t* pdus, const uint64_t* tb_offset,
                                   const uint32_t* grid_index, uint32_t nof_grids, uint32_t grid_nof_ports,
                                   uint32_t grid_nof_subc, PlanPlacement* place, nrphy_pdsch_plan_t** out);

namespace {

void* ctx_scratch(nrphy_ctx* ctx, ScratchSlot slot, size_t bytes)
{
  if (bytes > ctx->scratch_bytes[slot]) {
    (void)hipFree(ctx->scratch[slot]);
    ctx->scratch[slot]       = nullptr;
    ctx->scratch_bytes[slot] = 0;
    const size_t want        = (bytes + (bytes >> 2) + 4095) & ~(size_t)4095;
    if (hipMalloc(&ctx->scratch[slot], want) != hipSuccess) {
      return nullptr;
    }
    ctx->scratch_bytes[slot] = want;
  }
  return ctx->scratch[slot];
}

class HostCall
{
public:
  explicit HostCall(nrphy_ctx* c) : ctx(c), lock(c->host_mutex), device_set(hipSetDevice(c->device) == hipSuccess) {}
  HostCall(const HostCall&)            = delete;
  HostCall& operator=(const HostCall&) = delete;
  ~HostCall()
  {
    if (!drained) {
      (void)hipStreamSynchronize(ctx->stream);
    }
  }
  template <typename T = void>
  T* mem(ScratchSlot slot, size_t bytes)
  {
    return device_set ? (T*)ctx_scratch(ctx, slot, bytes) : nullptr;
  }
  template <size_t N>
  bool carve(ScratchSlot slot, const size_t (&bytes)[N], uint8_t* (&piece)[N])
  {
    size_t offset[N + 1] = {};
    for (size_t i = 0; i != N; ++i) {
      offset[i + 1] = offset[i] + ((bytes[i] + 255) & ~(size_t)255);
    }
    uint8_t* base = mem<uint8_t>(slot, offset[N]);
    for (size_t i = 0; i != N; ++i) {
      piece[i] = base ? base + offset[i] : nullptr;
    }
    return base != nullptr;
  }
  hipError_t sync()
  {
    drained = true;
    return hipStreamSynchronize(ctx->stream);
  }

private:
  nrphy_ctx*                            ctx;
  std::lock_guard<std::recursive_mutex> lock;
  bool                                  device_set;
  bool                                  drained = false;
};

class StreamStaging
{
public:
  explicit StreamStaging(hipStream_t s) : stream(s) {}
  StreamStaging(const StreamStaging&)            = delete;
  StreamStaging& operator=(const StreamStaging&) = delete;
  ~StreamStaging()
  {
    if (ptr != nullptr) {
      (void)hipFreeAsync(ptr, stream);
    }
  }
  void* alloc(size_t bytes)
  {
    if (hipMallocAsync(&ptr, std::max<size_t>(bytes, 16), stream) != hipSuccess) {
      ptr = nullptr;
    }
    return ptr;
  }

private:
  hipStream_t stream;
  void*       ptr = nullptr;
};

}
```

### srsran-edgeric-5g_amd/csrc/nrphy_internal.h

```cpp
#pragma once

#include "mi355_nrphy.h"

#include <hip/hip_runtime.h>
#include <stdint.h>

namespace nrphy {

constexpr int NOF_LIFTING_SIZES = 51;
constexpr int NOF_GRAPHS        = 2 * NOF_LIFTING_SIZES;
constexpr int MAX_BG_ROWS       = 46;
constexpr int MAX_BG_EDGES      = 316;

struct LiftedGraph {
  uint16_t row_ptr[MAX_BG_ROWS + 2];
  uint16_t core_b;
  uint16_t core_s0;
  uint16_t core_s3;
  uint16_t core_mid;
  uint32_t edge[MAX_BG_EDGES];
};

constexpr int GOLD_JUMP_BITS  = 24;
constexpr int GOLD_X1_WORDS   = 1 << 16;

constexpr uint32_t SCR_PARTS = 4;

constexpr int CRC_POW_WORDS = 288;

struct GoldTables {
  uint32_t x2_jump[GOLD_JUMP_BITS][32];
  uint32_t x2_head[32][32];
  uint32_t crc24b_pow32[CRC_POW_WORDS];
  uint32_t crc24b_table[256];
  uint32_t crc24b_slice[4][256];
  uint32_t crc24b_mul[CRC_POW_WORDS][6][16];
  float2 qam_lut[4][256];
};

constexpr int RE_CHUNK = 512;
#ifndef NRPHY_CRC_SLICES
#define NRPHY_CRC_SLICES 3
#endif
#define NRPHY_CB_U_GRAPH_OFFSET (2 * 22 * 12 + 80)

enum SymKind : uint32_t { SYM_NONE = 0, SYM_CONTIGUOUS = 1, SYM_TABLE = 2 };

struct PduDev {
  uint64_t tb_offset;
  uint64_t cw_bit_offset;
  uint32_t tb_bytes;
  uint32_t grid_index;
  uint32_t graph;
  uint32_t zc;
  uint32_t kb;
  uint32_t K;
  uint32_t info_bits;
  uint32_t filler;
  uint32_t tb_crc_bits;
  uint32_t cb_crc_bits;
  uint32_t zero_pad;
  uint32_t C;
  uint32_t n_short;
  uint32_t e_short;
  uint32_t e_long;
  uint32_t n_cb;
  uint32_t k0;
  uint32_t nof_rows;
  uint32_t qm;
  uint32_t nof_layers;
  uint32_t nof_ports;
  uint32_t c_init;
  uint32_t item_first;
  uint32_t scr_words;
  uint32_t nof_re;
  uint32_t weights_offset;
  uint32_t dmrs_weights_offset;
  uint32_t nof_prg;
  uint32_t prg_size_subc;
  uint32_t sym_re_start[NRPHY_NSYMB + 1];
  uint32_t sym_kind[NRPHY_NSYMB];
  uint32_t sym_arg[NRPHY_NSYMB];
  uint32_t dmrs_symbol_mask;
  uint32_t dmrs_zero_other_group;
  uint32_t dmrs_c_init[NRPHY_NSYMB];
  uint32_t dmrs_ref_rb;
  uint32_t dmrs_seq_offset;
  uint32_t dmrs_seq_words;
  float    dmrs_amplitude;
  uint32_t prb_mask[2 * NRPHY_PRB_WORDS];
  uint32_t first_prb;
  uint32_t end_prb;
  uint32_t crc_first;
  uint32_t crc_count;
};

struct CbWork {
  uint32_t pdu;
  uint32_t cb;
  uint32_t re_begin;
  uint32_t re_count;
};

constexpr int DMRS_PRB_CHUNK = 32;
#ifndef NRPHY_CRC_WORDS_PER_THREAD
#define NRPHY_CRC_WORDS_PER_THREAD 16
#endif
constexpr uint32_t TB_CRC_REGION_WORDS = 256 * NRPHY_CRC_WORDS_PER_THREAD;
constexpr uint32_t TB_CRC_REGION_BYTES = 4 * TB_CRC_REGION_WORDS;

struct TbCrcTables {
  uint32_t y32[2][4][256];
  uint32_t y1k[2][4][256];
  uint32_t y8k[2][4][256];
  uint32_t yz[2][4][256];
  uint32_t lane[2][64];
};

struct DmrsWork {
  uint32_t pdu;
  uint32_t symbol;
  uint32_t prb_begin;
  uint32_t prb_end;
};

struct ScrWork {
  uint32_t pdu;
  uint32_t first;
  uint32_t count;
  uint32_t with_dmrs;
};

struct CrcWork {
  uint32_t pdu;
  uint32_t region;
  uint32_t factor;
  uint32_t count;
};
constexpr uint32_t TB_CRC_MAX_REGIONS_PER_WORK = 8;
constexpr uint32_t TB_CRC_TARGET_WORK          = 1024;

struct ZeroSeg {
  uint16_t symbol;
  uint16_t k0;
  uint16_t count;
  uint16_t pad_;
};
constexpr uint32_t ZERO_LONG_RUN = 32;
struct ZeroWork {
  uint32_t grid;
  uint32_t port;
  uint32_t seg_begin;
  uint32_t seg_count;
  uint32_t seg_long;
};

struct PdschLaunch {
  const ZeroWork*    zero_work;
  const ZeroSeg*     zero_segs;
  uint32_t           n_zero_work;
  uint32_t           n_dmrs_in_launch;
  uint32_t*          scr;
  uint32_t*          scr_seed;
  const PduDev*      pdus;
  const CbWork*      work;
  const DmrsWork*    dmrs_work;
  const CrcWork*     crc_work;
  const ScrWork*     scr_work;
  uint32_t           n_scr_work;
  const TbCrcTables* tbcrc;
  uint32_t           n_crc_work;
  const float*       weights;
  const uint16_t*    re_table;
  const LiftedGraph* graphs;
  const GoldTables*  gold;
  const uint32_t*    x1_words;
  uint32_t*          tb_crc_part;
  uint32_t           n_pdu;
  uint32_t           n_work;
  uint32_t           work_base;
  uint32_t           n_dmrs_work;
  uint32_t           grid_nof_ports;
  uint32_t           grid_nof_subc;
  uint32_t           lds_lin_words;
  uint32_t           lds_u_words;
  uint32_t           profile_stage;
  uint32_t           extras_nt;
  uint32_t           prologue_order;
  uint32_t           zero_fill;
};

hipError_t launch_prologue(const PdschLaunch& p, const uint8_t* d_tb, hipStream_t stream);
constexpr uint32_t CB_BUCKETS        = 16;
constexpr uint32_t CB_MIXED_MAX_WORK = 4096;
inline uint32_t cb_bucket(uint32_t qm, uint32_t nof_layers)
{
  return (qm / 2u - 1u) * 4u + (nof_layers - 1u);
}
bool       codeblocks_take_bucket_launches(const PdschLaunch& p, const uint32_t* bucket_begin, int dispatch, uint32_t* nof_buckets);
hipError_t launch_codeblocks(const PdschLaunch& p, const uint32_t* bucket_begin, int dispatch, const uint8_t* d_tb,
                             uint32_t* d_grid, uint32_t* d_cw_rm, uint32_t* d_cw_scr, const hipStream_t* streams, uint32_t n_streams);
hipError_t launch_dmrs(const PdschLaunch& p, uint32_t* d_grid, hipStream_t stream);
hipError_t launch_ldpc_encode(const LiftedGraph* graphs, uint32_t graph, uint32_t kb, uint32_t zc, uint32_t n_cb,
                              const uint8_t* d_msg, uint32_t msg_stride, uint32_t out_bits, uint8_t* d_out,
                              uint32_t out_stride, hipStream_t stream);

struct DecoderGraph {
  uint32_t row_ptr[MAX_BG_ROWS + 2];
  uint32_t pair_ptr[MAX_BG_ROWS + 2];
  uint32_t quad_ptr[MAX_BG_ROWS + 2];
  uint32_t edge[MAX_BG_EDGES];
};

constexpr uint32_t DEC_CRC_TABLE_WORDS = 8 * 16;

struct LdpcDecodeLaunch {
  const DecoderGraph* graph;
  const uint32_t*     pair_addr;
  const int8_t*       llr;
  uint2*              scratch;
  uint32_t*           slot_flags;
  uint32_t            nof_slots;
  uint32_t            slot_bytes;
  uint8_t*            out;
  uint32_t*           iterations;
  const uint32_t*     crc_weight;
  const uint8_t*      skip;
  uint8_t*            ok_flags;
  uint32_t            crc_at_end;
  uint32_t            zc, bg_k, nof_nodes, nof_layers_max;
  uint32_t            nof_llr, llr_stride, out_stride, nof_filler;
  uint32_t            crc_poly, crc_order;
  uint32_t            max_iterations;
  float               scaling_factor;
  uint32_t            lm_lds_bytes;
  uint32_t            lds_tail_off;
  uint32_t            scale_arithmetic;
  uint32_t            scale_fixed;
  int                 knob_pairs, knob_msg, knob_ldsmsg;
};
hipError_t launch_ldpc_decode(const LdpcDecodeLaunch& p, uint32_t n_cb, hipStream_t stream);

enum DematchKind : uint32_t { DEMATCH_ZERO = 0, DEMATCH_FILL, DEMATCH_COPY, DEMATCH_COMBINE };
struct DematchOp {
  uint32_t kind, begin, count, src;
};
constexpr uint32_t MAX_DEMATCH_OPS = 60;
struct DematchLaunch {
  const int8_t* in;
  int8_t*       out;
  uint32_t      in_stride, out_stride, block_length, qm, cols, n_ops;
  uint32_t      in_stride_outer, out_stride_outer;
  uint32_t      skip_load;
  uint32_t      disjoint;
  const DematchOp* ops_ext;
  DematchOp        ops[MAX_DEMATCH_OPS];
};
hipError_t launch_ldpc_dematch(const DematchLaunch& p, uint32_t n_cb, hipStream_t stream, uint32_t n_outer = 1);

struct PuschAssembleLaunch {
  const uint8_t* cb_msg;
  uint8_t*       cb_ok;
  const uint32_t* cb_iter;
  const uint8_t* skipped;
  uint8_t*       tb;
  uint32_t*      result;
  const uint32_t* crc_weight;
  const TbCrcTables* tbcrc;
  uint32_t       crc_factor;
  uint32_t       C, msg_stride, tb_stride, tb_bytes, cb_info_bits, max_iterations;
};
constexpr uint32_t PUSCH_ASSEMBLE_THREADS = 1024;
hipError_t launch_pusch_assemble(const PuschAssembleLaunch& p, uint32_t n_tb, hipStream_t stream);

constexpr uint32_t CSI_RS_MAX_SEQ_WORDS = 128;
struct CsiRsWork {
  uint32_t grid_index, symbol, c_init;
  uint32_t advance, seq_len;
  uint32_t rb_begin, rb_stride, re_mask, n_re_prb;
  uint32_t nof_ports, first_layer, group_size;
  uint32_t weights_offset;
  float    amplitude;
};
struct CsiRsLaunch {
  const CsiRsWork*  work;
  const float*      weights;
  const GoldTables* gold;
  const uint32_t*   x1_words;
  uint32_t*         grid;
  uint32_t          grid_nof_ports, grid_nof_subc;
};
hipError_t launch_csi_rs(const CsiRsLaunch& p, uint32_t n_work, hipStream_t stream);
hipError_t launch_llr_descramble(const GoldTables* gold, const uint32_t* x1_words, const uint32_t* d_c_init, uint32_t n_cw,
                                 uint32_t length, const int8_t* d_in, size_t in_stride, int8_t* d_out, size_t out_stride,
                                 hipStream_t stream);
constexpr uint32_t DEMOD_MAX_PAIRS = 4;
struct DemodLaunch {
  uint32_t modulation;
  uint32_t span_len;
  uint32_t nof_vector;
  float    range, scale;
  float    qam16_gain, qam16_threshold;
  uint32_t nof_intervals[DEMOD_MAX_PAIRS];
  float    width[DEMOD_MAX_PAIRS], rcp_width[DEMOD_MAX_PAIRS];
  float    slope[DEMOD_MAX_PAIRS][16], intercept[DEMOD_MAX_PAIRS][16];
};
hipError_t launch_demodulate_soft(const DemodLaunch& p, uint32_t nof_spans, const float* d_symbols, const float* d_noise,
                                  int8_t* d_llr, hipStream_t stream);
bool demod_params(uint32_t modulation, uint32_t span_len, DemodLaunch& p);

constexpr uint32_t PUSCH_DEMOD_THREADS = 256;
struct PuschDemodDesc {
  uint32_t grid_index, nof_rx_ports, nof_layers, qm;
  uint32_t equalizer, c_init, prb_first, dmrs_re_per_prb;
  uint32_t rx_ports[NRPHY_MAX_PORTS];
  uint8_t  dmrs_subc[NRPHY_NRE];
  uint32_t item_first, nof_items;
  uint64_t ce_offset;
};
struct PuschDemodItem {
  uint32_t pusch, symbol, dmrs;
  uint32_t re_first, count;
  uint32_t bit_offset;
  uint32_t span_pos, nof_vector;
};
struct PuschDemodLaunch {
  const PuschDemodDesc* desc;
  const PuschDemodItem* items;
  const uint16_t*       prbs;
  const DemodLaunch*    demod;
  const GoldTables*     gold;
  const uint32_t*       x1_words;
  const uint32_t*       grid;
  const uint32_t*       ch;
  const float*          noise;
  int8_t*               llr;
  uint64_t              llr_stride;
  double*               partial;
  float*                sinr;
  uint32_t              grid_nof_ports, grid_nof_subc, n_pusch, n_items;
};
hipError_t launch_pusch_demod(const PuschDemodLaunch& p, hipStream_t stream);
struct EqualizeLaunch {
  uint32_t        algorithm, n_batch, nof_re, nof_layers, nof_rx_ports;
  float           tx_scaling;
  const uint32_t* rx;
  const uint32_t* ch;
  const float*    noise;
  float*          eq;
  float*          eq_nvars;
};
hipError_t launch_channel_equalize(const EqualizeLaunch& p, hipStream_t stream);
constexpr uint32_t PUSCH_CHEST_TA_WINDOW  = 144;
constexpr uint32_t PUSCH_CHEST_MAX_LAYERS = 2;
struct PuschChestDesc {
  uint32_t grid_index, nof_rx_ports, nof_layers, nprb;
  uint32_t prb_first;
  uint32_t first_symbol, nof_symbols, nof_dmrs;
  uint32_t nwords;
  uint32_t ntaps, nof_v;
  uint32_t dc;
  uint32_t scs_hz;
  uint32_t rx_ports[NRPHY_MAX_PORTS];
  uint32_t dmrs_symbol[NRPHY_NSYMB];
  uint32_t c_init[NRPHY_NSYMB];
  float    epoch[NRPHY_NSYMB];
  float    taps[16];
  float    beta, ls_scale;
  uint64_t ce_offset;
  uint64_t row_offset;
};
struct PuschChestLaunch {
  const PuschChestDesc*     desc;
  const uint32_t*           jobs;
  const uint16_t*           prbs;
  const float2*             twiddle;
  const GoldTables*         gold;
  const uint32_t*           x1_words;
  const uint32_t*           grid;
  uint32_t*                 ch;
  float*                    noise_vars;
  nrphy_pusch_chest_meas_t* meas;
  uint32_t*                 rows;
  float2*                   rot;
  uint32_t                  grid_nof_ports, grid_nof_subc, n_jobs;
};
hipError_t launch_pusch_chest(const PuschChestLaunch& p, hipStream_t stream);
hipError_t launch_grid_put(const uint32_t* d_index, const uint32_t* d_value, uint32_t n, uint32_t* d_grid, hipStream_t stream);

struct PdcchWork {
  uint32_t grid_index;
  uint32_t A, E, N;
  uint32_t mode;
  uint32_t rnti, crc_const;
  uint32_t c_init_data;
  uint32_t start_symbol, duration, n_prb, ref_rb, top_prb;
  uint32_t nof_ports, prg_size_subc;
  uint32_t dmrs_c_init[3];
  float    data_amp, dmrs_amp;
  uint32_t weights_offset, src_offset, prb_offset, payload_offset, crcw_offset, enc_offset;
};
struct SsbWork {
  uint32_t grid_index, l0, k0, pci;
  uint32_t a_bits;
  uint32_t scr_mask;
  uint32_t scr_adv;
  uint32_t ssb_adv;
  uint32_t dmrs_c_init;
  uint32_t m_pss, m0, m1;
  float    pss_amp;
  uint32_t nof_ports;
  uint8_t  ports[NRPHY_MAX_PORTS];
  uint32_t src_offset, crcw_offset, enc_offset;
};
struct DlControlLaunch {
  const PdcchWork*  pdcch;
  const SsbWork*    ssb;
  const float*      weights;
  const uint16_t*   tab16;
  const uint8_t*    bytes;
  const uint32_t*   words;
  const GoldTables* gold;
  const uint32_t*   x1_words;
  uint32_t*         grid;
  uint8_t*          enc;
  uint32_t          grid_nof_ports, grid_nof_subc;
};
hipError_t launch_pdcch(const DlControlLaunch& p, uint32_t n, hipStream_t stream);
hipError_t launch_ssb(const DlControlLaunch& p, uint32_t n, hipStream_t stream);

struct OfdmLaunch {
  uint32_t       dft_size;
  uint32_t       rg_size;
  uint32_t       nof_ports;
  uint32_t       nsymb;
  uint32_t       slot_stride;
  const float2*  twiddle;
  const float2*  phase;
  const float2*  window_phase;
  const uint32_t* cp_len;
  const uint32_t* sym_offset;
  uint32_t       probe;
  uint32_t       wire = 0, wire_clip = 0;
  float          wire_gain = 1.f, wire_ceiling = 0.f, wire_scale = 1.f;
  float          wire_limit = 0.f;
  nrphy_amplitude_stats_t* wire_stats = nullptr;
  uint4*         wire_partials = nullptr;
};

struct AmplitudeLaunch {
  const float* in;
  float*       out;
  size_t       in_stride, out_stride;
  uint32_t     nof_samples, measure, clip;
  float        gain, ceiling;
  nrphy_amplitude_stats_t* stats;
};
hipError_t launch_amplitude(const AmplitudeLaunch& p, uint32_t n_buffers, hipStream_t stream);
hipError_t launch_convert_ci16(const float* in, size_t in_stride, int16_t* out, size_t out_stride, uint32_t n_buffers,
                               uint32_t nof_samples, float scale, hipStream_t stream);
struct OfhCompressLaunch {
  const uint32_t* prbs;
  uint8_t*        out;
  size_t          row_stride, out_row_stride;
  uint32_t        nof_prb, data_width, bfp, whole_span;
  float           scale;
};
hipError_t launch_ofh_compress(const OfhCompressLaunch& p, uint32_t n_rows, hipStream_t stream);
hipError_t launch_ofdm(const OfdmLaunch& p, uint32_t nof_grids, const uint32_t* d_grid, const uint32_t* d_slot_index,
                       float2* d_iq, hipStream_t stream);
hipError_t launch_ofdm_demod(const OfdmLaunch& p, uint32_t nof_grids, const float2* d_iq, const uint32_t* d_slot_index,
                             uint32_t window_offset, uint32_t* d_grid, hipStream_t stream);
bool       dft_split(uint32_t size, uint32_t* n1, uint32_t* n2);
bool       dft_size_supported(uint32_t size);
inline bool dft_size_in_lds(uint32_t size)
{
  uint32_t n1 = 0, n2 = 0;
  return dft_split(size, &n1, &n2) && n1 == 1;
}
hipError_t launch_dft(uint32_t size, int inverse, uint32_t batch, const float2* twiddle, const float2* twiddle_n2,
                      float2* d_tmp, const float2* d_in, float2* d_out, hipStream_t stream);

}
```

### srsran-edgeric-5g_amd/csrc/pdsch_kernels.hip

```cpp
#include "ldpc_device.h"

#ifndef NRPHY_PHASE_A_STAGED
#define NRPHY_PHASE_A_STAGED 1
#endif

#ifdef NRPHY_PROBES
#define NRPHY_STAGE(p) ((p).profile_stage)
#else
#define NRPHY_STAGE(p) 0u
#endif

namespace nrphy {

__global__ __launch_bounds__(TB_CRC_THREADS) void prologue_kernel(PdschLaunch p, const uint8_t* __restrict__ d_tb)
{
  constexpr uint32_t LDS_WORDS = TB_CRC_LDS_WORDS;
  __shared__ __attribute__((aligned(16))) uint32_t lds[LDS_WORDS];
  static_assert(LDS_WORDS >= GOLD_RING_WORDS, "LDS of the sequence role");
  const uint32_t tid = threadIdx.x;

  uint32_t scr_index = blockIdx.x, crc_index = blockIdx.x - p.n_scr_work;
  bool     scr_role  = blockIdx.x < p.n_scr_work;
  if (p.prologue_order == 1 && p.n_scr_work != 0 && p.n_crc_work != 0) {
    const uint32_t total = p.n_scr_work + p.n_crc_work;
    const uint32_t xcd = blockIdx.x & 7u, turn = blockIdx.x >> 3, q = total >> 3, r = total & 7u;
    const uint32_t pos = xcd * q + (xcd < r ? xcd : r) + turn;
    const uint32_t s0 = (uint32_t)(((uint64_t)pos * p.n_scr_work + total - 1u) / total);
    const uint32_t s1 = (uint32_t)(((uint64_t)(pos + 1u) * p.n_scr_work + total - 1u) / total);
    scr_role  = s1 > s0;
    scr_index = s0;
    crc_index = pos - s0;
  }
  NRPHY_WG_TRACE_MARK(0);
  NRPHY_WG_TRACE_WHERE(scr_role ? 1 : 2);
  if (scr_role) {
    if (NRPHY_STAGE(p) == 8) {
      return;
    }
    const auto*    swc   = to_constant(&p.scr_work[scr_index]);
    const uint32_t first = swc->first, count = swc->count;
    const bool     with_dmrs = swc->with_dmrs != 0;
    PduRef         pd    = *to_constant(&p.pdus[swc->pdu]);
    const uint32_t wave = tid / WAVE, lane = tid % WAVE;
    constexpr uint32_t DMRS_WAVES = TB_CRC_THREADS / WAVE - 1, DMRS_SCRATCH = (GOLD_RING_WORDS - 2048u) / DMRS_WAVES;
    static_assert(GOLD_SEED_WORDS <= 2048u && GOLD_RING_WORDS > 2048u, "LDS of the sequence role");
    static_assert((12u * NRPHY_MAX_RB + 31u) / 32u + 1u <= DMRS_SCRATCH, "DM-RS scratch per wave");
    if (wave == 0) {
      const uint32_t lq = pd.qm * pd.nof_layers, n_short = pd.n_short, e_short = pd.e_short, e_long = pd.e_long, C = pd.C;
      const uint32_t nre_short = e_short / lq, nre_long = e_long / lq;
      struct Cursor {
        uint32_t cb, re_begin, item, bit_cb, nre;
      };
      Cursor resume = {0u, 0u, pd.item_first, 0u, n_short != 0 ? nre_short : nre_long};
      auto   advance = [&](Cursor& c) {
        c.re_begin += RE_CHUNK;
        if (c.re_begin >= c.nre) {
          c.bit_cb += c.cb < n_short ? e_short : e_long;
          ++c.cb;
          c.re_begin = 0;
          c.nre      = c.cb < n_short ? nre_short : nre_long;
        }
        ++c.item;
      };
      gold_sequence_blocks_wave(p.gold, pd.c_init, first, count, lds, lane, [&](uint32_t base, uint32_t avail) {
        const uint32_t lo = first + base, hi = lo + avail;
        Cursor c        = resume;
        bool   resuming = false;
        while (c.cb < C) {
          const uint32_t w0 = (c.bit_cb + c.re_begin * lq) >> 5;
          if (w0 >= hi) {
            break;
          }
          if (w0 + 31u > lo) {
            const uint32_t k = w0 + lane;
            if (lane < 31u && k >= lo && k < hi) {
              p.scr_seed[(size_t)c.item * 32u + lane] = lds[k - lo];
            }
          }
          if (w0 + 31u > hi && !resuming) {
            resume   = c;
            resuming = true;
          }
          advance(c);
        }
        if (!resuming) {
          resume = c;
        }
      });
      NRPHY_WG_TRACE_MARK(6);
    } else if (with_dmrs && pd.dmrs_seq_words <= DMRS_SCRATCH) {
      uint32_t ordinal = 0;
      for (uint32_t mask = pd.dmrs_symbol_mask; mask != 0; mask &= mask - 1u, ++ordinal) {
        if (ordinal % DMRS_WAVES == wave - 1u) {
          const uint32_t l = (uint32_t)__ffs(mask) - 1u;
          gold_sequence_wave(p.gold, p.x1_words, pd.dmrs_c_init[l], pd.dmrs_seq_words,
                             p.scr + pd.dmrs_seq_offset + ordinal * pd.dmrs_seq_words,
                             lds + 2048u + (wave - 1u) * DMRS_SCRATCH, lane);
        }
      }
    }
    return;
  }

  if (NRPHY_STAGE(p) == 9) {
    return;
  }
  const auto*     wkc = to_constant(&p.crc_work[crc_index]);
  const uint32_t  wk_pdu = wkc->pdu, wk_region = wkc->region, wk_factor = wkc->factor, wk_count = wkc->count;
  PduRef          pd  = *to_constant(&p.pdus[wk_pdu]);
  const uint32_t  sel = (pd.tb_crc_bits == 16) ? 1u : 0u;
  const CrcPoly   c   = sel ? crc16() : crc24a();
  const uint32_t  n   = pd.tb_bytes;
  const uint32_t* tbw = reinterpret_cast<const uint32_t*>(d_tb + pd.tb_offset);
#ifdef NRPHY_WG_TRACE
  asm volatile("s_waitcnt lgkmcnt(0)" ::: "memory");
  NRPHY_WG_TRACE_MARK(3);
#endif
  const uint32_t share = tbcrc_regions_workgroup(p.tbcrc, sel, c, tbw, n, wk_region, wk_count, wk_factor, lds, tid);
  if (tid == 0) {
    p.tb_crc_part[crc_index] = share;
  }
  NRPHY_WG_TRACE_MARK(6);
}

#ifdef NRPHY_WG_TRACE
extern "C" int nrphy_debug_wg_trace(uint64_t* out, uint32_t nof_blocks)
{
  const size_t n = 8 * (size_t)(nof_blocks < WG_TRACE_MAX ? nof_blocks : WG_TRACE_MAX) * sizeof(uint64_t);
  return (int)hipMemcpyFromSymbol(out, HIP_SYMBOL(g_wg_trace), n, 0, hipMemcpyDeviceToHost);
}
#endif

hipError_t launch_prologue(const PdschLaunch& p, const uint8_t* d_tb, hipStream_t stream)
{
  if (p.n_crc_work + p.n_scr_work == 0) {
    return hipSuccess;
  }
  hipLaunchKernelGGL(prologue_kernel, dim3(p.n_crc_work + p.n_scr_work), dim3(TB_CRC_THREADS), 0, stream, p, d_tb);
  return hipGetLastError();
}

constexpr uint32_t CB_U_QAM_WORDS     = 512;
constexpr uint32_t CB_U_LDPC_WORDS    = (sizeof(LdpcScratch) / 4u + 3u) & ~3u;
constexpr uint32_t CB_U_GRAPH_OFFSET  = LDPC_DBL_WORDS + CB_U_LDPC_WORDS;
static_assert(CB_U_GRAPH_OFFSET == NRPHY_CB_U_GRAPH_OFFSET, "host and device agree on the layout of the scratch region");

struct CbShared {
  uint32_t* lin;
  uint32_t* u;
  uint32_t* symb;
  uint32_t* graph;
  LdpcScratch* ldpc;
};

#ifndef NRPHY_LDS_PROBE
#define NRPHY_LDS_PROBE 0
#endif
__device__ __forceinline__ uint32_t lds_probe_index(uint32_t idx, uint32_t bit)
{
  if ((NRPHY_LDS_PROBE >> bit) & 1) {
    uint32_t zero = 0;
    asm volatile("" : "+v"(zero));
    const uint32_t lane = __builtin_amdgcn_mbcnt_hi(~0u, __builtin_amdgcn_mbcnt_lo(~0u, 0u));
    return (idx & zero) + lane;
  }
  return idx;
}

__device__ __forceinline__ uint32_t crc24_word_step(const uint32_t* tab, uint32_t reg, uint32_t word)
{
#if NRPHY_CRC_SLICES == 4
  const uint32_t v = (reg << 8) ^ word;
  return tab[v & 0xFFu] ^ tab[256u + ((v >> 8) & 0xFFu)] ^ tab[512u + ((v >> 16) & 0xFFu)] ^ tab[768u + (v >> 24)];
#else
  const uint32_t v = reg ^ (word >> 8);
  uint32_t       r = tab[lds_probe_index(v & 0xFFu, 1)] ^ tab[256u + lds_probe_index((v >> 8) & 0xFFu, 1)] ^ tab[512u + lds_probe_index(v >> 16, 1)];
  return ((r << 8) & 0xFFFFFFu) ^ tab[lds_probe_index(((r >> 16) ^ word) & 0xFFu, 1)];
#endif
}

__device__ inline void build_codeblock(PduRef pd, uint32_t cb, const uint32_t* tbw, const uint32_t* tb_crc_part,
                                       const GoldTables* tables, CbShared* sh, uint32_t total_words, uint32_t lane,
                                       uint32_t profile_stage)
{
  const bool     last    = (cb == pd.C - 1);
  const uint32_t used    = pd.info_bits - (last ? pd.tb_crc_bits + pd.zero_pad : 0u);
  const uint32_t tb_pos  = cb * pd.info_bits;
  const uint32_t tb_bits = pd.tb_bytes * 8u;
  const uint4* crc_src = reinterpret_cast<const uint4*>(&tables->crc24b_slice[0][0]);
  const uint4  crc_tab0 = crc_src[lane], crc_tab1 = crc_src[lane + WAVE], crc_tab2 = crc_src[lane + 2 * WAVE];
#if NRPHY_CRC_SLICES == 4
  const uint4 crc_tab3 = crc_src[lane + 3 * WAVE];
#endif
  constexpr uint32_t SEG_UNROLL = 5;
  for (uint32_t base = lane; base < total_words; base += WAVE * SEG_UNROLL) {
    uint32_t hi[SEG_UNROLL], lo[SEG_UNROLL];
#pragma unroll
    for (uint32_t k = 0; k != SEG_UNROLL; ++k) {
      const uint32_t pos = 32u * (base + WAVE * k);
      hi[k] = 0;
      lo[k] = 0;
      if (pos < used) {
        const uint32_t abs_pos = tb_pos + pos;
        const uint32_t i = abs_pos >> 5, sft = abs_pos & 31u;
        hi[k] = tbw[i];
        if (sft != 0 && 32u * (i + 1) < tb_bits) {
          lo[k] = tbw[i + 1];
        }
      }
    }
#pragma unroll
    for (uint32_t k = 0; k != SEG_UNROLL; ++k) {
      const uint32_t j = base + WAVE * k, pos = 32u * j;
      if (j < total_words) {
        uint32_t v = 0;
        if (pos < used) {
          v = __funnelshift_l(__builtin_bswap32(lo[k]), __builtin_bswap32(hi[k]), (tb_pos + pos) & 31u);
          const uint32_t remaining = used - pos;
          if (remaining < 32u) {
            v &= topmask(remaining);
          }
        }
        sh->lin[j] = v;
      }
    }
  }
  {
    uint4* dst           = reinterpret_cast<uint4*>(sh->u);
    dst[lane]            = crc_tab0;
    dst[lane + WAVE]     = crc_tab1;
    dst[lane + 2 * WAVE] = crc_tab2;
#if NRPHY_CRC_SLICES == 4
    dst[lane + 3 * WAVE] = crc_tab3;
#endif
  }
  wave_sync();
  if (profile_stage == 7) {
    return;
  }
  if (last) {
    const uint32_t tb_crc = wave_xor(lane < pd.crc_count ? tb_crc_part[pd.crc_first + lane] : 0u);
    if (lane == 0) {
      or_bits_lds_exclusive(sh->lin, used, tb_crc << (32u - pd.tb_crc_bits), pd.tb_crc_bits);
    }
  }
  wave_sync();
  if (pd.cb_crc_bits) {
    const uint32_t n   = pd.info_bits;
    const uint32_t pad = (32u - (n & 31u)) & 31u;
    const uint32_t nw  = (n + pad) >> 5;
    const uint32_t per = (nw + WAVE - 1) / WAVE;
    uint32_t       a   = lane * per;
    uint32_t       b   = a + per;
    a                  = a > nw ? nw : a;
    b                  = b > nw ? nw : b;
    uint32_t reg       = 0;
    for (uint32_t j = a; j < b; ++j) {
      uint32_t word;
      if (pad == 0) {
        word = sh->lin[j];
      } else if (j == 0) {
        word = sh->lin[0] >> pad;
      } else {
        word = ext32(sh->lin, 32u * j - pad);
      }
      reg = crc24_word_step(sh->u, reg, word);
    }
    uint32_t part = 0;
    {
      const uint32_t m = nw - b;
#pragma unroll
      for (uint32_t k = 0; k != 6; ++k) {
        part ^= tables->crc24b_mul[m][k][(reg >> (4u * k)) & 15u];
      }
    }
    uint32_t crc = wave_xor(part);
    if (lane == 0) {
      or_bits_lds_exclusive(sh->lin, n, crc << 8, 24);
    }
    wave_sync();
  }
}

struct RmIndex {
  uint32_t fs;
  uint32_t flen;
  uint32_t n_valid;
  uint32_t rank0;
  float    inv_valid;
};

__device__ __forceinline__ RmIndex rm_index_init(PduRef pd)
{
  RmIndex  r;
  uint32_t nsys = (pd.kb - 2u) * pd.zc;
  uint32_t fs   = nsys - pd.filler;
  uint32_t fe   = nsys;
  fs            = fs > pd.n_cb ? pd.n_cb : fs;
  fe            = fe > pd.n_cb ? pd.n_cb : fe;
  r.fs          = fs;
  r.flen        = fe - fs;
  r.n_valid     = pd.n_cb - r.flen;
  r.rank0       = pd.k0 < fs ? pd.k0 : (pd.k0 < fe ? fs : pd.k0 - r.flen);
  r.inv_valid   = 1.0f / (float)r.n_valid;
  return r;
}

template <bool WRAP>
__device__ __forceinline__ uint32_t rm_gather32(const RmIndex& r, const uint32_t* lin, uint32_t zc2, uint32_t t)
{
  uint32_t u = r.rank0 + t;
  if (WRAP && u >= r.n_valid) {
    uint32_t q = (uint32_t)((float)u * r.inv_valid);
    u -= q * r.n_valid;
    if ((int32_t)u < 0) {
      u += r.n_valid;
    } else if (u >= r.n_valid) {
      u -= r.n_valid;
    }
  }
  uint32_t run = (u < r.fs) ? r.fs - u : r.n_valid - u;
  uint32_t out = ext32(lin, (u < r.fs ? u : u + r.flen) + zc2);
  if (run >= 32u) {
    return out;
  }
  out &= topmask(run);
  uint32_t filled = run;
  while (filled < 32u) {
    u += run;
    if (u >= r.n_valid) {
      if (!WRAP) {
        break;
      }
      u = 0;
    }
    run            = (u < r.fs) ? r.fs - u : r.n_valid - u;
    run            = run > 32u - filled ? 32u - filled : run;
    uint32_t piece = ext32(lin, (u < r.fs ? u : u + r.flen) + zc2);
    out |= (piece & topmask(run)) >> filled;
    filled += run;
  }
  return out;
}

__device__ __forceinline__ uint32_t bit_select(uint32_t m, uint32_t a, uint32_t b)
{
  return __builtin_amdgcn_bitop3_b32(m, a, b, 0xCA);
}

__device__ __forceinline__ void transpose8x8(uint32_t& hi, uint32_t& lo)
{
  hi = bit_select(0xAA55AA55u, hi, bit_select(0x55005500u, hi << 7, hi >> 7));
  lo = bit_select(0xAA55AA55u, lo, bit_select(0x55005500u, lo << 7, lo >> 7));
  hi = bit_select(0xCCCC3333u, hi, bit_select(0x33330000u, hi << 14, hi >> 14));
  lo = bit_select(0xCCCC3333u, lo, bit_select(0x33330000u, lo << 14, lo >> 14));
  const uint32_t nhi = bit_select(0xF0F0F0F0u, hi, lo >> 4);
  const uint32_t nlo = bit_select(0x0F0F0F0Fu, lo, hi << 4);
  hi                 = nhi;
  lo                 = nlo;
}

__device__ __forceinline__ void cmul_ref(float xr, float xi, float wr, float wi, float& outr, float& outi)
{
  float t0 = __fmul_rn(xi, wi);
  float t1 = __fmul_rn(xr, wi);
  outr     = __fmaf_rn(xr, wr, -t0);
  outi     = __fmaf_rn(xi, wr, t1);
}

typedef float cf2 __attribute__((ext_vector_type(2)));
__device__ __forceinline__ cf2 cmul_ref_packed(cf2 x, cf2 w)
{
  cf2 t, r;
  asm("v_pk_mul_f32 %0, %1, %2 op_sel:[1,1] op_sel_hi:[0,1]" : "=v"(t) : "v"(x), "v"(w));
  asm("v_pk_fma_f32 %0, %1, %2, %3 op_sel_hi:[1,0,1] neg_lo:[0,0,1]" : "=v"(r) : "v"(x), "v"(w), "v"(t));
  return r;
}
__device__ __forceinline__ cf2 cmul_ref_packed_uniform(cf2 x, cf2 w)
{
  cf2 t, r;
  asm("v_pk_mul_f32 %0, %1, %2 op_sel:[1,1] op_sel_hi:[0,1]" : "=v"(t) : "v"(x), "s"(w));
  asm("v_pk_fma_f32 %0, %1, %2, %3 op_sel_hi:[1,0,1] neg_lo:[0,0,1]" : "=v"(r) : "v"(x), "s"(w), "v"(t));
  return r;
}

typedef __bf16 bf16x2_t __attribute__((ext_vector_type(2)));
typedef float  f32x2_t __attribute__((ext_vector_type(2)));
__device__ __forceinline__ uint32_t pack_cbf16(float re, float im)
{
  f32x2_t  v = {re, im};
  bf16x2_t b = __builtin_convertvector(v, bf16x2_t);
  return *reinterpret_cast<uint32_t*>(&b);
}

__device__ __forceinline__ void grid_store(uint32_t* p, uint32_t v)
{
  __builtin_nontemporal_store(v, p);
}

#ifndef NRPHY_GRID_STORE_AUX
#define NRPHY_GRID_STORE_AUX 2
#endif
#ifndef NRPHY_GRID_BUFFER_STORES
#define NRPHY_GRID_BUFFER_STORES 1
#endif

struct ChunkGeom {
  uint32_t E;
  uint32_t cw_cb;
  uint32_t bit0;
};

template <int QM, int L, bool WRAP>
__device__ __forceinline__ void phase_a(const PdschLaunch& p, PduRef pd, const CbWork& wk, const CbShared& sh,
                                        uint32_t E, uint32_t lane)
{
  const uint32_t esym = E / QM;
  const uint32_t zc2  = 2u * pd.zc;
  const RmIndex  rm   = rm_index_init(pd);
  const uint32_t s0   = wk.re_begin * L;
  const uint32_t nblk = (wk.re_count * L + 31u) >> 5;
  constexpr uint32_t LUT_TRIPS = ((1u << QM) + WAVE - 1u) / WAVE;
  float2             lut[LUT_TRIPS];
#pragma unroll
  for (uint32_t k = 0; k != LUT_TRIPS; ++k) {
    lut[k] = lane + WAVE * k < (1u << QM) ? p.gold->qam_lut[QM / 2 - 1][lane + WAVE * k] : make_float2(0.f, 0.f);
  }
#if NRPHY_PHASE_A_STAGED
  for (uint32_t item = lane; item < QM * nblk; item += WAVE) {
    const uint32_t blk = item / QM, j = item - blk * QM;
    sh.symb[8u * blk + j] = rm_gather32<WRAP>(rm, sh.lin, zc2, j * esym + s0 + 32u * blk);
  }
  wave_sync();
  const uint8_t* rows = reinterpret_cast<const uint8_t*>(sh.symb);
  for (uint32_t item = lane; item < 4u * nblk; item += WAVE) {
    const uint32_t blk = item >> 2, m = item & 3u;
    const uint8_t* b   = rows + 32u * blk + (3u - m);
    uint32_t       r8[8];
#pragma unroll
    for (int j = 0; j != 8; ++j) {
      r8[j] = (j < QM) ? b[4 * j] : 0u;
    }
    uint32_t hi = (r8[0] << 24) | (r8[1] << 16) | (r8[2] << 8) | r8[3];
    uint32_t lo = (r8[4] << 24) | (r8[5] << 16) | (r8[6] << 8) | r8[7];
    transpose8x8(hi, lo);
    sh.symb[8u * blk + 2u * m]      = hi;
    sh.symb[8u * blk + 2u * m + 1u] = lo;
  }
#else
  for (uint32_t blk = lane; blk < nblk; blk += WAVE) {
    uint32_t row[8];
#pragma unroll
    for (int j = 0; j != 8; ++j) {
      row[j] = (j < QM) ? rm_gather32<WRAP>(rm, sh.lin, zc2, (uint32_t)j * esym + s0 + 32u * blk) : 0u;
    }
#pragma unroll
    for (int m = 0; m != 4; ++m) {
      const int sft = 24 - 8 * m;
      uint32_t  hi  = (((row[0] >> sft) & 0xFFu) << 24) | (((row[1] >> sft) & 0xFFu) << 16) |
                    (((row[2] >> sft) & 0xFFu) << 8) | ((row[3] >> sft) & 0xFFu);
      uint32_t lo = (((row[4] >> sft) & 0xFFu) << 24) | (((row[5] >> sft) & 0xFFu) << 16) |
                    (((row[6] >> sft) & 0xFFu) << 8) | ((row[7] >> sft) & 0xFFu);
      transpose8x8(hi, lo);
      sh.symb[8u * blk + 2u * m]      = hi;
      sh.symb[8u * blk + 2u * m + 1u] = lo;
    }
  }
#endif
  if (lane < 8) {
    sh.symb[8u * nblk + lane] = 0;
  }
#pragma unroll
  for (uint32_t k = 0; k != LUT_TRIPS; ++k) {
    if (lane + WAVE * k < (1u << QM)) {
      reinterpret_cast<float2*>(sh.u)[lane + WAVE * k] = lut[k];
    }
  }
  wave_sync();
}

__device__ __forceinline__ void pin_scalar(cf2& w)
{
  asm volatile("" : "+s"(w));
}

struct ChunkMap {
  uint32_t re0;
  uint32_t word0;
  bool     aligned;
};

template <int QM, int L>
__device__ __forceinline__ uint32_t x1_bits(const PdschLaunch& p, const ChunkGeom& g, const ChunkMap& cm, uint32_t re_count,
                                            uint32_t r)
{
  uint32_t bits = 0;
  if (r < re_count) {
    if (QM * L == 32 && cm.aligned) {
      bits = (p.x1_words + cm.word0)[r];
    } else {
      bits = ext32(p.x1_words, g.bit0 + r * (uint32_t)(QM * L));
    }
  }
  return bits;
}
template <int QM, int L>
__device__ __forceinline__ uint32_t x2_bits(const uint32_t* x2, const ChunkGeom& g, const ChunkMap& cm, uint32_t r)
{
  if (QM * L == 32 && cm.aligned) {
    return x2[r];
  }
  return ext32(x2, (g.bit0 & 31u) + r * (uint32_t)(QM * L));
}

template <int QM, int L>
__device__ __forceinline__ void re_bits(const PdschLaunch& p, const CbShared& sh, const ChunkGeom& g, const ChunkMap& cm,
                                        uint32_t re_count, uint32_t r, uint32_t& bytes, uint32_t& gbits)
{
  if constexpr (L == 4) {
    bytes = sh.symb[r];
  } else {
    bytes = ext32(sh.symb, 8u * r * L);
  }
  gbits = x1_bits<QM, L>(p, g, cm, re_count, r) ^ x2_bits<QM, L>(sh.lin, g, cm, r);
}

template <int QM, int L, int P>
__device__ __forceinline__ void phase_b_grid(const PdschLaunch& p, PduRef pd, const PduDev* __restrict__ pd_global,
                                             const CbWork& wk, const CbShared& sh, const ChunkGeom& g, const ChunkMap& cm,
                                             uint32_t first_gbits, uint32_t lane, uint32_t* __restrict__ d_grid)
{
  const size_t   grid_base   = (size_t)pd.grid_index * p.grid_nof_ports * NRPHY_NSYMB * p.grid_nof_subc;
  const uint32_t plane_words = NRPHY_NSYMB * p.grid_nof_subc;
  const __amdgpu_buffer_rsrc_t grid_rsrc = __builtin_amdgcn_make_buffer_rsrc(
      d_grid + grid_base, 0, (int)(NRPHY_STAGE(p) == 11 ? 0u : p.grid_nof_ports * plane_words * 4u), 0x00020000);
  cf2 wu[P > 0 ? P : 1][L];
  if constexpr (P > 0) {
    const float NRPHY_CONSTANT* wuni = to_constant(p.weights + pd.weights_offset);
#pragma unroll
    for (int port = 0; port != P; ++port) {
#pragma unroll
      for (int l = 0; l != L; ++l) {
        wu[port][l] = cf2{wuni[2 * (port * L + l)], wuni[2 * (port * L + l) + 1]};
      }
    }
#pragma unroll
    for (int port = 0; port != P; ++port) {
#pragma unroll
      for (int l = 0; l != L; ++l) {
        pin_scalar(wu[port][l]);
      }
    }
  }
  uint32_t l_cur = 0;
#pragma unroll 1
  while (l_cur + 1u < NRPHY_NSYMB && cm.re0 >= pd.sym_re_start[l_cur + 1u]) {
    ++l_cur;
  }
  uint32_t cur_start = pd.sym_re_start[l_cur], cur_end = pd.sym_re_start[l_cur + 1u];
  uint32_t cur_arg = pd.sym_arg[l_cur], cur_row = l_cur * p.grid_nof_subc;
  bool     cur_table = pd.sym_kind[l_cur] == SYM_TABLE;
  uint32_t gbits_next = first_gbits;

  for (uint32_t r0 = 0; r0 < wk.re_count; r0 += WAVE) {
    const uint32_t r        = r0 + lane;
    const uint32_t x1       = gbits_next;
    gbits_next              = x1_bits<QM, L>(p, g, cm, wk.re_count, r + WAVE);
    const uint32_t re_first = cm.re0 + r0;
    const uint32_t re_last  = re_first + ((wk.re_count - r0 < WAVE ? wk.re_count - r0 : WAVE) - 1u);
    if (re_first >= cur_end && l_cur + 1u < NRPHY_NSYMB) {
#pragma unroll 1
      do {
        ++l_cur;
        cur_start = cur_end;
        cur_end   = pd.sym_re_start[l_cur + 1u];
      } while (re_first >= cur_end && l_cur + 1u < NRPHY_NSYMB);
      cur_arg   = pd.sym_arg[l_cur];
      cur_row   = l_cur * p.grid_nof_subc;
      cur_table = pd.sym_kind[l_cur] == SYM_TABLE;
    }
    if (r >= wk.re_count) {
      continue;
    }
    __builtin_assume(r < (uint32_t)RE_CHUNK + WAVE);
    const uint32_t gbits = x1 ^ x2_bits<QM, L>(sh.lin, g, cm, r);
    uint32_t bytes;
    if constexpr (L == 4) {
      bytes = sh.symb[r];
    } else {
      bytes = ext32(sh.symb, 8u * r * L);
    }
    const uint32_t re_pdu = re_first + lane;
    uint32_t       subc, word_offset;
    if (re_last < cur_end) {
      subc = cur_arg + (re_pdu - cur_start);
      if (cur_table) {
        subc = (uint32_t)p.re_table[subc];
      }
      word_offset = cur_row + subc;
    } else {
      uint32_t l_sym = l_cur, start = cur_start, end = cur_end;
#pragma unroll 1
      while (re_pdu >= end && l_sym + 1u < NRPHY_NSYMB) {
        ++l_sym;
        start = end;
        end   = pd_global->sym_re_start[l_sym + 1u];
      }
      subc = pd_global->sym_arg[l_sym] + (re_pdu - start);
      if (pd_global->sym_kind[l_sym] == SYM_TABLE) {
        subc = (uint32_t)p.re_table[subc];
      }
      word_offset = l_sym * p.grid_nof_subc + subc;
    }
    cf2 x[L];
#pragma unroll
    for (int l = 0; l != L; ++l) {
      const uint32_t raw   = ((bytes >> (24 - 8 * l)) & 0xFFu) >> (8 - QM);
      const uint32_t idx   = raw ^ ((gbits >> (32 - (l + 1) * QM)) & ((1u << QM) - 1u));
      const float2   point = reinterpret_cast<const float2*>(sh.u)[lds_probe_index(idx, 0)];
      x[l]                 = cf2{point.x, point.y};
    }
    if constexpr (P > 0) {
#pragma unroll
      for (int port = 0; port != P; ++port) {
        cf2 acc = cmul_ref_packed_uniform(x[0], wu[port][0]);
#pragma unroll
        for (int l = 1; l != L; ++l) {
          acc += cmul_ref_packed_uniform(x[l], wu[port][l]);
        }
        __builtin_amdgcn_raw_buffer_store_b32(pack_cbf16(acc.x, acc.y), grid_rsrc, (int)(word_offset * 4u),
                                              (int)(port * plane_words * 4u), NRPHY_GRID_STORE_AUX);
      }
    } else {
      const uint32_t nof_ports = pd.nof_ports;
      uint32_t       prg       = subc / pd.prg_size_subc;
      prg                      = prg >= pd.nof_prg ? pd.nof_prg - 1 : prg;
      const float* w = p.weights + pd.weights_offset + 2u * prg * nof_ports * L;
#pragma unroll 1
      for (uint32_t port = 0; port != nof_ports; ++port) {
        cf2 acc = cmul_ref_packed(x[0], cf2{w[2 * port * L], w[2 * port * L + 1]});
#pragma unroll
        for (int l = 1; l != L; ++l) {
          acc += cmul_ref_packed(x[l], cf2{w[2 * (port * L + l)], w[2 * (port * L + l) + 1]});
        }
        __builtin_amdgcn_raw_buffer_store_b32(pack_cbf16(acc.x, acc.y), grid_rsrc, (int)(word_offset * 4u),
                                              (int)(port * plane_words * 4u), NRPHY_GRID_STORE_AUX);
      }
    }
  }
}

template <int QM, int L>
__device__ __forceinline__ void phase_b(const PdschLaunch& p, PduRef pd, const PduDev* __restrict__ pd_global,
                                        const CbWork& wk, const CbShared& sh, const ChunkGeom& g, const ChunkMap& cm,
                                        uint32_t first_gbits, uint32_t lane, uint32_t* __restrict__ d_grid,
                                        uint32_t* __restrict__ d_cw_rm, uint32_t* __restrict__ d_cw_scr)
{
  constexpr uint32_t LQ = QM * L;
  if (d_cw_rm != nullptr || d_cw_scr != nullptr) {
    const uint64_t cw_bit0 = pd.cw_bit_offset + g.cw_cb + (uint64_t)wk.re_begin * LQ;
    for (uint32_t r = lane; r < wk.re_count; r += WAVE) {
      uint32_t bytes, gbits;
      re_bits<QM, L>(p, sh, g, cm, wk.re_count, r, bytes, gbits);
      uint32_t v_rm = 0;
#pragma unroll
      for (int l = 0; l != L; ++l) {
        const uint32_t raw = ((bytes >> (24 - 8 * l)) & 0xFFu) >> (8 - QM);
        v_rm |= raw << (32 - (l + 1) * QM);
      }
      if (d_cw_rm) {
        or_bits_global(d_cw_rm, cw_bit0 + (uint64_t)r * LQ, v_rm, LQ);
      }
      if (d_cw_scr) {
        or_bits_global(d_cw_scr, cw_bit0 + (uint64_t)r * LQ, v_rm ^ (gbits & topmask(LQ)), LQ);
      }
    }
  }
  if (d_grid == nullptr) {
    return;
  }
  const uint32_t nof_ports = pd.nof_prg == 1 ? pd.nof_ports : 0u;
  if (nof_ports == 4u) {
    phase_b_grid<QM, L, 4>(p, pd, pd_global, wk, sh, g, cm, first_gbits, lane, d_grid);
  } else if (L <= 3 && nof_ports == 3u) {
    phase_b_grid<QM, (L <= 3 ? L : 1), 3>(p, pd, pd_global, wk, sh, g, cm, first_gbits, lane, d_grid);
  } else if (L <= 2 && nof_ports == 2u) {
    phase_b_grid<QM, (L <= 2 ? L : 1), 2>(p, pd, pd_global, wk, sh, g, cm, first_gbits, lane, d_grid);
  } else if (L == 1 && nof_ports == 1u) {
    phase_b_grid<QM, 1, 1>(p, pd, pd_global, wk, sh, g, cm, first_gbits, lane, d_grid);
  } else {
    phase_b_grid<QM, L, 0>(p, pd, pd_global, wk, sh, g, cm, first_gbits, lane, d_grid);
  }
}

template <int QM, int L>
__device__ __forceinline__ void map_chunk(const PdschLaunch& p, PduRef pd, const PduDev* pd_global, const CbWork& wk,
                                          uint32_t item, const CbShared& sh, uint32_t lane, uint32_t* d_grid,
                                          uint32_t* d_cw_rm, uint32_t* d_cw_scr)
{
  const bool is_long = wk.cb >= pd.n_short;
  ChunkGeom  g;
  g.E     = is_long ? pd.e_long : pd.e_short;
  g.cw_cb = is_long ? pd.n_short * pd.e_short + (wk.cb - pd.n_short) * pd.e_long : wk.cb * pd.e_short;
  g.bit0  = g.cw_cb + wk.re_begin * (uint32_t)(QM * L);
  if (NRPHY_STAGE(p) == 3) {
    return;
  }
  ChunkMap cm;
  cm.re0     = g.cw_cb / (uint32_t)(QM * L) + wk.re_begin;
  cm.word0   = g.bit0 >> 5;
  cm.aligned = (g.bit0 & 31u) == 0;
  const uint32_t seed_word   = lane < 31u ? p.scr_seed[(size_t)item * 32u + lane] : 0u;
  const uint32_t first_gbits = x1_bits<QM, L>(p, g, cm, wk.re_count, lane);
  {
    const RmIndex rm = rm_index_init(pd);
    if (rm.rank0 + g.E > rm.n_valid) {
      phase_a<QM, L, true>(p, pd, wk, sh, g.E, lane);
    } else {
      phase_a<QM, L, false>(p, pd, wk, sh, g.E, lane);
    }
  }
  if (NRPHY_STAGE(p) == 4) {
    return;
  }
  NRPHY_WG_TRACE_MARK(3);
  static_assert((31u + (uint32_t)RE_CHUNK * 32u + 31u) / 32u + 1u <= GOLD_EXPAND_MAX_WORDS, "a work item's scrambling words");
  gold_expand_seed_wave(sh.lin, seed_word, ((g.bit0 & 31u) + wk.re_count * (uint32_t)(QM * L) + 31u) / 32u + 1u, lane);
  phase_b<QM, L>(p, pd, pd_global, wk, sh, g, cm, first_gbits, lane, d_grid, d_cw_rm, d_cw_scr);
}

template <int QM>
__device__ __forceinline__ void map_chunk_layers(const PdschLaunch& p, PduRef pd, const PduDev* pd_global,
                                                 const CbWork& wk, uint32_t item, const CbShared& sh, uint32_t lane,
                                                 uint32_t* d_grid, uint32_t* d_cw_rm, uint32_t* d_cw_scr)
{
  switch (pd.nof_layers) {
    case 1:
      map_chunk<QM, 1>(p, pd, pd_global, wk, item, sh, lane, d_grid, d_cw_rm, d_cw_scr);
      break;
    case 2:
      map_chunk<QM, 2>(p, pd, pd_global, wk, item, sh, lane, d_grid, d_cw_rm, d_cw_scr);
      break;
    case 3:
      map_chunk<QM, 3>(p, pd, pd_global, wk, item, sh, lane, d_grid, d_cw_rm, d_cw_scr);
      break;
    default:
      map_chunk<QM, 4>(p, pd, pd_global, wk, item, sh, lane, d_grid, d_cw_rm, d_cw_scr);
      break;
  }
}

template <int L, typename W>
__device__ __forceinline__ void dmrs_port_words(float dr, float di, bool odd, uint32_t port, W w, uint32_t (&word)[(L + 1) / 2])
{
  const float sr = odd ? -dr : dr, si = odd ? -di : di;
#pragma unroll
  for (int g = 0; g != (L + 1) / 2; ++g) {
    float accr, acci;
    cmul_ref(dr, di, w[2 * (port * L + 2 * g)], w[2 * (port * L + 2 * g) + 1], accr, acci);
    if (2 * g + 1 < L) {
      float pr, pi;
      cmul_ref(sr, si, w[2 * (port * L + 2 * g + 1)], w[2 * (port * L + 2 * g + 1) + 1], pr, pi);
      accr = __fadd_rn(accr, pr);
      acci = __fadd_rn(acci, pi);
    }
    word[g] = pack_cbf16(accr, acci);
  }
}

typedef uint32_t u32x2_t __attribute__((ext_vector_type(2)));
typedef uint32_t u32x4_t __attribute__((ext_vector_type(4)));
template <int L>
__device__ __forceinline__ void dmrs_store(uint32_t* out, const uint32_t (&word)[(L + 1) / 2], bool zero_other_group, bool nt = false)
{
  if ((L + 1) / 2 == 2 || zero_other_group) {
    const u32x2_t v = {word[0], (L + 1) / 2 == 2 ? word[(L + 1) / 2 - 1] : 0u};
    if (nt) {
      __builtin_nontemporal_store(v, reinterpret_cast<u32x2_t*>(out));
    } else {
      *reinterpret_cast<u32x2_t*>(out) = v;
    }
  } else if (nt) {
    __builtin_nontemporal_store(word[0], out);
  } else {
    out[0] = word[0];
  }
}

template <int L, typename W>
__device__ __forceinline__ void dmrs_precode(float dr, float di, bool odd, uint32_t P, W w, uint32_t* out,
                                             size_t port_stride, bool zero_other_group)
{
#pragma unroll 1
  for (uint32_t port = 0; port != P; ++port) {
    uint32_t word[(L + 1) / 2];
    dmrs_port_words<L>(dr, di, odd, port, w, word);
    dmrs_store<L>(out + port * port_stride, word, zero_other_group);
  }
}

template <int L>
__device__ __forceinline__ void dmrs_items(const PdschLaunch& p, PduRef pd, const DmrsWork& wk,
                                           uint32_t* __restrict__ d_grid, uint32_t lane, uint32_t* tab)
{
  const uint32_t  P       = pd.nof_ports;
  const uint32_t  ordinal = __popc(pd.dmrs_symbol_mask & ((1u << wk.symbol) - 1u));
  const uint32_t* seq     = p.scr + pd.dmrs_seq_offset + ordinal * pd.dmrs_seq_words;
  const float     a       = pd.dmrs_amplitude;
  const uint32_t  nof_items = (wk.prb_end - wk.prb_begin) * 6u;
  const size_t    port_stride = (size_t)NRPHY_NSYMB * p.grid_nof_subc;
  uint32_t*       row = d_grid + (size_t)pd.grid_index * p.grid_nof_ports * port_stride + (size_t)wk.symbol * p.grid_nof_subc;
  const bool      wideband = pd.nof_prg == 1;
  const bool      zero_other = pd.dmrs_zero_other_group != 0 && p.zero_fill != 0;
  if (wideband) {
    if (lane < 8u) {
      const float dr = (lane & 4u) ? -a : a, di = (lane & 2u) ? -a : a;
#pragma unroll 1
      for (uint32_t port = 0; port != P; ++port) {
        uint32_t word[(L + 1) / 2];
        dmrs_port_words<L>(dr, di, (lane & 1u) != 0, port, to_constant(p.weights + pd.dmrs_weights_offset), word);
        tab[(lane * NRPHY_MAX_PORTS + port) * 2u]      = word[0];
        tab[(lane * NRPHY_MAX_PORTS + port) * 2u + 1u] = word[(L + 1) / 2 - 1];
      }
    }
    wave_sync();
  }
  for (uint32_t item = lane; item < nof_items; item += WAVE) {
    const uint32_t prb = wk.prb_begin + item / 6u;
    const uint32_t kp  = item % 6u;
    if (!((pd.prb_mask[prb >> 5] >> (prb & 31u)) & 1u)) {
      continue;
    }
    const uint32_t bit  = 12u * (prb - pd.dmrs_ref_rb) + 2u * kp;
    const uint32_t word = seq[bit >> 5] << (bit & 31u);
    uint32_t*      out  = row + 12u * prb + 2u * kp;
    if (wideband) {
      const uint32_t variant = ((word >> 29) & 6u) | (kp & 1u);
#pragma unroll 1
      for (uint32_t port = 0; port != P; ++port) {
        uint32_t words[(L + 1) / 2];
        words[0] = tab[(variant * NRPHY_MAX_PORTS + port) * 2u];
        if ((L + 1) / 2 == 2) {
          words[(L + 1) / 2 - 1] = tab[(variant * NRPHY_MAX_PORTS + port) * 2u + 1u];
        }
        dmrs_store<L>(out + port * port_stride, words, zero_other, p.extras_nt != 0);
      }
      continue;
    }
    const float dr = (word & 0x80000000u) ? -a : a;
    const float di = (word & 0x40000000u) ? -a : a;
    uint32_t    prg = (12u * prb) / pd.prg_size_subc;
    prg             = prg >= pd.nof_prg ? pd.nof_prg - 1 : prg;
    dmrs_precode<L>(dr, di, (kp & 1u) != 0, P, p.weights + pd.dmrs_weights_offset + 2u * prg * P * L, out, port_stride,
                    zero_other);
  }
}

__device__ __forceinline__ void dmrs_wave(const PdschLaunch& p, uint32_t item_index, uint32_t* __restrict__ d_grid,
                                          uint32_t lane, uint32_t* tab)
{
  const auto*    wkc = to_constant(&p.dmrs_work[item_index]);
  const DmrsWork wk  = {wkc->pdu, wkc->symbol, wkc->prb_begin, wkc->prb_end};
  PduRef         pd  = *to_constant(&p.pdus[wk.pdu]);
  switch (pd.nof_layers) {
    case 1:
      dmrs_items<1>(p, pd, wk, d_grid, lane, tab);
      break;
    case 2:
      dmrs_items<2>(p, pd, wk, d_grid, lane, tab);
      break;
    case 3:
      dmrs_items<3>(p, pd, wk, d_grid, lane, tab);
      break;
    default:
      dmrs_items<4>(p, pd, wk, d_grid, lane, tab);
      break;
  }
}

__device__ __forceinline__ void zero_wave(const PdschLaunch& p, uint32_t item_index, uint32_t* __restrict__ d_grid, uint32_t lane)
{
  const auto*    wkc  = to_constant(&p.zero_work[item_index]);
  const uint32_t seg_begin = wkc->seg_begin, seg_count = wkc->seg_count, seg_long = wkc->seg_long;
  uint32_t*      base = d_grid + ((size_t)wkc->grid * p.grid_nof_ports + wkc->port) * NRPHY_NSYMB * p.grid_nof_subc;
  static_assert(sizeof(ZeroSeg) == 8, "one run descriptor per lane as two dwords");
  for (uint32_t first = 0; first < seg_long; first += WAVE) {
    const uint32_t n = seg_long - first < WAVE ? seg_long - first : WAVE;
    uint2          d = make_uint2(0u, 0u);
    if (lane < n) {
      d = *reinterpret_cast<const uint2*>(&p.zero_segs[seg_begin + first + lane]);
    }
    for (uint32_t i = 0; i != n; ++i) {
      const uint32_t lo_word = (uint32_t)__builtin_amdgcn_readlane((int)d.x, (int)i);
      const uint32_t count   = (uint32_t)__builtin_amdgcn_readlane((int)d.y, (int)i) & 0xFFFFu;
      uint32_t*      row     = base + (size_t)(lo_word & 0xFFFFu) * p.grid_nof_subc + (lo_word >> 16);
      const uint32_t off      = (uint32_t)((reinterpret_cast<uintptr_t>(row) >> 2) & 3u);
      uint32_t*      aligned  = row - off;
      const uint32_t n_chunks = (off + count + 3u) >> 2;
      for (uint32_t c = lane; c < n_chunks; c += WAVE) {
        const uint32_t lo = 4u * c;
        if (lo >= off && lo + 4u <= off + count) {
          if (p.extras_nt != 0) {
          __builtin_nontemporal_store(u32x4_t{0u, 0u, 0u, 0u}, reinterpret_cast<u32x4_t*>(aligned + lo));
        } else {
          *reinterpret_cast<uint4*>(aligned + lo) = make_uint4(0u, 0u, 0u, 0u);
        }
        } else {
#pragma unroll
          for (uint32_t w = 0; w != 4; ++w) {
            if (lo + w >= off && lo + w < off + count) {
              aligned[lo + w] = 0u;
            }
          }
        }
      }
    }
  }
  for (uint32_t i = seg_long + lane; i < seg_count; i += WAVE) {
    const ZeroSeg  sg  = p.zero_segs[seg_begin + i];
    uint32_t*      row = base + (size_t)sg.symbol * p.grid_nof_subc + sg.k0;
    for (uint32_t k = 0; k != sg.count; ++k) {
      row[k] = 0u;
    }
  }
}


#ifndef NRPHY_CB_WAVES
#define NRPHY_CB_WAVES 4
#endif
constexpr uint32_t CB_WAVES = NRPHY_CB_WAVES;

struct CbWave {
  uint32_t  lane;
  uint32_t  wave;
  uint32_t* lds;
};
__device__ __forceinline__ CbWave cb_wave(const PdschLaunch& p, uint32_t* dyn_lds)
{
  CbWave w;
  w.lane = threadIdx.x % WAVE;
  w.wave = (uint32_t)__builtin_amdgcn_readfirstlane((int)(threadIdx.x / WAVE));
  w.lds  = dyn_lds + w.wave * (p.lds_lin_words + p.lds_u_words);
  return w;
}
__host__ __device__ __forceinline__ uint32_t cb_blocks(uint32_t n_units)
{
  return (n_units + CB_WAVES - 1u) / CB_WAVES;
}

__device__ __forceinline__ bool extra_wave(const PdschLaunch& p, const CbWave& w, uint32_t* __restrict__ d_grid)
{
  const uint32_t nb = cb_blocks(p.n_work);
  if (blockIdx.x < nb) {
    return false;
  }
  const uint32_t extra = (blockIdx.x - nb) * CB_WAVES + w.wave;
  if (extra < p.n_dmrs_in_launch) {
    dmrs_wave(p, extra, d_grid, w.lane, w.lds);
  } else if (extra - p.n_dmrs_in_launch < p.n_zero_work) {
    zero_wave(p, extra - p.n_dmrs_in_launch, d_grid, w.lane);
  }
  return true;
}

__device__ __forceinline__ uint32_t xcd_work_item(uint32_t n_work, const CbWave& w)
{
  const uint32_t nb  = cb_blocks(n_work);
  const uint32_t xcd = blockIdx.x & 7u, turn = blockIdx.x >> 3;
  const uint32_t q = nb >> 3, r = nb & 7u;
  const uint32_t item = (xcd * q + (xcd < r ? xcd : r) + turn) * CB_WAVES + w.wave;
  return item < n_work ? item : n_work;
}

__device__ __forceinline__ bool codeblock_front(const PdschLaunch& p, PduRef pd, const CbWork& wk, CbShared& sh,
                                                const uint8_t* __restrict__ d_tb, uint32_t lane)
{
  const uint32_t zc = pd.zc, kb = pd.kb;
  if (NRPHY_STAGE(p) == 5 || NRPHY_STAGE(p) == 6) {
    return false;
  }
  const uint32_t total_words = (((kb + pd.nof_rows) * zc + 31u) >> 5) + 2u;
  GraphRows rows;
  rows.fetch(&p.graphs[pd.graph], pd.nof_rows, lane);
  build_codeblock(pd, wk.cb, reinterpret_cast<const uint32_t*>(d_tb + pd.tb_offset), p.tb_crc_part, p.gold, &sh,
                  total_words, lane, NRPHY_STAGE(p));
  if (NRPHY_STAGE(p) == 1 || NRPHY_STAGE(p) == 7) {
    return false;
  }
  NRPHY_WG_TRACE_MARK(1);
  rows.store(pd.nof_rows, sh.graph, lane);
  ldpc_encode_wave(&p.graphs[pd.graph], sh.graph, kb, zc, pd.nof_rows, sh.lin, sh.u, sh.ldpc, lane);
  NRPHY_WG_TRACE_MARK(2);
  return NRPHY_STAGE(p) != 2;
}

template <int QM, int L>
__global__ __launch_bounds__(WAVE * CB_WAVES) void codeblock_kernel_t(PdschLaunch p, const uint8_t* __restrict__ d_tb,
                                                              uint32_t* __restrict__ d_grid, uint32_t* __restrict__ d_cw_rm,
                                                              uint32_t* __restrict__ d_cw_scr)
{
  extern __shared__ __attribute__((aligned(16))) uint32_t dyn_lds[];
  const CbWave   w    = cb_wave(p, dyn_lds);
  const uint32_t lane = w.lane;
  CbShared       sh;
  sh.lin   = w.lds;
  sh.u     = w.lds + p.lds_lin_words;
  sh.symb  = sh.u + CB_U_QAM_WORDS;
  sh.graph = sh.u + CB_U_GRAPH_OFFSET;
  sh.ldpc  = reinterpret_cast<LdpcScratch*>(sh.u + LDPC_DBL_WORDS);
  if (NRPHY_STAGE(p) == 10 || extra_wave(p, w, d_grid)) {
    return;
  }
  const uint32_t item = xcd_work_item(p.n_work, w);
  if (item == p.n_work) {
    return;
  }
  NRPHY_WG_TRACE_MARK(0);
  NRPHY_WG_TRACE_WHERE(3);
  const auto*  wkc = to_constant(&p.work[item]);
  const CbWork wk  = {wkc->pdu, wkc->cb, wkc->re_begin, wkc->re_count};
  PduRef       pd  = *to_constant(&p.pdus[wk.pdu]);
  if (!codeblock_front(p, pd, wk, sh, d_tb, lane)) {
    return;
  }
  map_chunk<QM, L>(p, pd, &p.pdus[wk.pdu], wk, p.work_base + item, sh, lane, d_grid, d_cw_rm, d_cw_scr);
  NRPHY_WG_TRACE_MARK(6);
}

__global__ __launch_bounds__(WAVE * CB_WAVES) void codeblock_kernel(PdschLaunch p, const uint8_t* __restrict__ d_tb,
                                                         uint32_t* __restrict__ d_grid, uint32_t* __restrict__ d_cw_rm,
                                                         uint32_t* __restrict__ d_cw_scr)
{
  extern __shared__ __attribute__((aligned(16))) uint32_t dyn_lds[];
  const CbWave   w    = cb_wave(p, dyn_lds);
  const uint32_t lane = w.lane;
  CbShared       sh;
  sh.lin   = w.lds;
  sh.u     = w.lds + p.lds_lin_words;
  sh.symb  = sh.u + CB_U_QAM_WORDS;
  sh.graph = sh.u + CB_U_GRAPH_OFFSET;
  sh.ldpc  = reinterpret_cast<LdpcScratch*>(sh.u + LDPC_DBL_WORDS);
  if (NRPHY_STAGE(p) == 10 || extra_wave(p, w, d_grid)) {
    return;
  }
  const uint32_t item = xcd_work_item(p.n_work, w);
  if (item == p.n_work) {
    return;
  }
  const auto*  wkc = to_constant(&p.work[item]);
  const CbWork wk  = {wkc->pdu, wkc->cb, wkc->re_begin, wkc->re_count};
  PduRef       pd  = *to_constant(&p.pdus[wk.pdu]);
  if (!codeblock_front(p, pd, wk, sh, d_tb, lane)) {
    return;
  }
  switch (pd.qm) {
    case 2:
      map_chunk_layers<2>(p, pd, &p.pdus[wk.pdu], wk, p.work_base + item, sh, lane, d_grid, d_cw_rm, d_cw_scr);
      break;
    case 4:
      map_chunk_layers<4>(p, pd, &p.pdus[wk.pdu], wk, p.work_base + item, sh, lane, d_grid, d_cw_rm, d_cw_scr);
      break;
    case 6:
      map_chunk_layers<6>(p, pd, &p.pdus[wk.pdu], wk, p.work_base + item, sh, lane, d_grid, d_cw_rm, d_cw_scr);
      break;
    default:
      map_chunk_layers<8>(p, pd, &p.pdus[wk.pdu], wk, p.work_base + item, sh, lane, d_grid, d_cw_rm, d_cw_scr);
      break;
  }
}

typedef void (*CodeblockKernel)(PdschLaunch, const uint8_t*, uint32_t*, uint32_t*, uint32_t*);

static CodeblockKernel bucket_kernel(uint32_t bucket)
{
  static const CodeblockKernel table[CB_BUCKETS] = {
      codeblock_kernel_t<2, 1>, codeblock_kernel_t<2, 2>, codeblock_kernel_t<2, 3>, codeblock_kernel_t<2, 4>,
      codeblock_kernel_t<4, 1>, codeblock_kernel_t<4, 2>, codeblock_kernel_t<4, 3>, codeblock_kernel_t<4, 4>,
      codeblock_kernel_t<6, 1>, codeblock_kernel_t<6, 2>, codeblock_kernel_t<6, 3>, codeblock_kernel_t<6, 4>,
      codeblock_kernel_t<8, 1>, codeblock_kernel_t<8, 2>, codeblock_kernel_t<8, 3>, codeblock_kernel_t<8, 4>};
  return table[bucket];
}

bool codeblocks_take_bucket_launches(const PdschLaunch& p, const uint32_t* bucket_begin, int dispatch, uint32_t* nof_buckets)
{
  uint32_t n = 0;
  for (uint32_t b = 0; b != CB_BUCKETS; ++b) {
    n += bucket_begin[b + 1] != bucket_begin[b] ? 1u : 0u;
  }
  *nof_buckets = n;
  return !(dispatch == 1 || (dispatch == 0 && n > 1 && p.n_work < CB_MIXED_MAX_WORK));
}

hipError_t launch_codeblocks(const PdschLaunch& p, const uint32_t* bucket_begin, int dispatch, const uint8_t* d_tb,
                             uint32_t* d_grid, uint32_t* d_cw_rm, uint32_t* d_cw_scr, const hipStream_t* streams, uint32_t n_streams)
{
  if (p.n_work == 0) {
    return hipSuccess;
  }
  const size_t   lds_bytes = 4u * (size_t)(p.lds_lin_words + p.lds_u_words) * CB_WAVES;
  const uint32_t extras    = d_grid ? p.n_dmrs_in_launch + p.n_zero_work : 0u;
  uint32_t       nof_buckets = 0;
  if (!codeblocks_take_bucket_launches(p, bucket_begin, dispatch, &nof_buckets)) {
    hipLaunchKernelGGL(codeblock_kernel, dim3(cb_blocks(p.n_work) + cb_blocks(extras)), dim3(WAVE * CB_WAVES), lds_bytes, streams[0], p,
                       d_tb, d_grid, d_cw_rm, d_cw_scr);
    return hipGetLastError();
  }
  uint32_t order[CB_BUCKETS], n_order = 0;
  for (uint32_t b = 0; b != CB_BUCKETS; ++b) {
    if (bucket_begin[b + 1] != bucket_begin[b]) {
      uint32_t k = n_order++;
      for (; k != 0 && bucket_begin[order[k - 1] + 1] - bucket_begin[order[k - 1]] < bucket_begin[b + 1] - bucket_begin[b]; --k) {
        order[k] = order[k - 1];
      }
      order[k] = b;
    }
  }
  for (uint32_t i = 0; i != n_order; ++i) {
    const uint32_t b = order[i], n = bucket_begin[b + 1] - bucket_begin[b];
    PdschLaunch    q = p;
    q.work           = p.work + bucket_begin[b];
    q.work_base      = bucket_begin[b];
    q.n_work         = n;
    if (i != 0) {
      q.n_dmrs_in_launch = 0;
      q.n_zero_work      = 0;
    }
    const uint32_t blocks = cb_blocks(n) + (i == 0 ? cb_blocks(extras) : 0u);
    hipLaunchKernelGGL(bucket_kernel(b), dim3(blocks), dim3(WAVE * CB_WAVES), lds_bytes, streams[n_streams > 1 ? i % n_streams : 0], q,
                       d_tb, d_grid, d_cw_rm, d_cw_scr);
    const hipError_t e = hipGetLastError();
    if (e != hipSuccess) {
      return e;
    }
  }
  return hipSuccess;
}

__global__ __launch_bounds__(WAVE) void dmrs_kernel(PdschLaunch p, uint32_t* __restrict__ d_grid)
{
  __shared__ uint32_t tab[8 * NRPHY_MAX_PORTS * 2];
  dmrs_wave(p, blockIdx.x, d_grid, threadIdx.x, tab);
}

hipError_t launch_dmrs(const PdschLaunch& p, uint32_t* d_grid, hipStream_t stream)
{
  if (p.n_dmrs_work == 0) {
    return hipSuccess;
  }
  hipLaunchKernelGGL(dmrs_kernel, dim3(p.n_dmrs_work), dim3(WAVE), 0, stream, p, d_grid);
  return hipGetLastError();
}

__global__ __launch_bounds__(WAVE) void ldpc_encode_kernel(const LiftedGraph* graphs, uint32_t graph, uint32_t kb,
                                                           uint32_t zc, const uint8_t* __restrict__ d_msg,
                                                           uint32_t msg_stride, uint32_t out_bits,
                                                           uint8_t* __restrict__ d_out, uint32_t out_stride)
{
  __shared__ uint32_t    lin[LDPC_LIN_WORDS];
  __shared__ uint32_t    gbuf[LDPC_GRAPH_ROWPTR + MAX_BG_EDGES];
  __shared__ uint32_t    dbl[LDPC_DBL_WORDS];
  __shared__ LdpcScratch scratch;
  const uint32_t         lane = threadIdx.x;
  const uint8_t*         msg  = d_msg + (size_t)blockIdx.x * msg_stride;
  uint8_t*               out  = d_out + (size_t)blockIdx.x * out_stride;

  const uint32_t K   = kb * zc;
  uint32_t       len = out_bits + 2u * zc;
  len                = len < (kb + 4u) * zc ? (kb + 4u) * zc : len;
  const uint32_t nof_rows    = (len + zc - 1u) / zc - kb;
  const uint32_t total_words = (((kb + nof_rows) * zc + 31u) >> 5) + 2u;
  const uint32_t msg_bytes   = (K + 7u) >> 3;
  for (uint32_t j = lane; j < total_words; j += WAVE) {
    uint32_t v = 0;
    for (uint32_t k = 0; k != 4; ++k) {
      uint32_t byte = 4u * j + k;
      v             = (v << 8) | (byte < msg_bytes ? (uint32_t)msg[byte] : 0u);
    }
    uint32_t pos = 32u * j;
    v            = pos >= K ? 0u : (K - pos < 32u ? v & topmask(K - pos) : v);
    lin[j]       = v;
  }
  stage_graph(&graphs[graph], nof_rows, gbuf, lane);
  wave_sync();
  ldpc_encode_wave(&graphs[graph], gbuf, kb, zc, nof_rows, lin, dbl, &scratch, lane);
  const uint32_t out_bytes = (out_bits + 7u) >> 3;
  for (uint32_t j = lane; 4u * j < out_bytes; j += WAVE) {
    uint32_t v   = ext32(lin, 2u * zc + 32u * j);
    uint32_t pos = 32u * j;
    if (out_bits - pos < 32u) {
      v &= topmask(out_bits - pos);
    }
    for (uint32_t k = 0; k != 4 && 4u * j + k < out_bytes; ++k) {
      out[4u * j + k] = (uint8_t)(v >> (24 - 8 * k));
    }
  }
}

hipError_t launch_ldpc_encode(const LiftedGraph* graphs, uint32_t graph, uint32_t kb, uint32_t zc, uint32_t n_cb,
                              const uint8_t* d_msg, uint32_t msg_stride, uint32_t out_bits, uint8_t* d_out,
                              uint32_t out_stride, hipStream_t stream)
{
  if (n_cb == 0) {
    return hipSuccess;
  }
  hipLaunchKernelGGL(ldpc_encode_kernel, dim3(n_cb), dim3(WAVE), 0, stream, graphs, graph, kb, zc, d_msg, msg_stride,
                     out_bits, d_out, out_stride);
  return hipGetLastError();
}

}
```

Baseline: 1.257 million.

## Specialize grid mapping on table symbols, stage x1 scrambling into LDS, add resident-grid option

Splits the grid-mapping loop with a template flag so PDUs that have no table-mapped symbols skip the per-RE table gather. The x1 scrambling words are now fetched once per chunk and folded into the LDS sequence up front, so the 64-RE loop no longer issues a global load and vmcnt wait per iteration. Adds an optional persistent-workgroup launch, sized from occupancy queries, in which waves loop over work items, with an optional stagger. That launch is off by default. The restructuring adds a new per-PDU flag, more template instantiations and a more involved symbol-boundary handling path.

Measured after the change: 1.254 million. Within noise of the previous version (-0.2%).

```diff
diff --git a/profiles/check_re_loop.py b/profiles/check_re_loop.py
--- a/profiles/check_re_loop.py
+++ b/profiles/check_re_loop.py
@@ -1,29 +1,54 @@
 #!/usr/bin/env python3
 import os
+import re
 import subprocess
+import sys
 import tempfile
 
 ROOT = os.path.dirname(os.path.dirname(os.path.abspath(__file__)))
 C = os.path.join(ROOT, "srsran-edgeric-5g_amd", "csrc")
+QM, L = (int(sys.argv[1]), int(sys.argv[2])) if len(sys.argv) > 2 else (8, 4)
 with tempfile.TemporaryDirectory() as tmp:
     subprocess.run(["/opt/rocm/bin/hipcc", "--offload-arch=gfx950", "-O3", "-std=c++17", "-fPIC", "-I" + os.path.join(ROOT, "include"), "-I" + C,
                     "-ffp-contract=off", "-x", "hip", "-c", os.path.join(C, "pdsch_kernels.hip"), "-o", os.path.join(tmp, "o.o"), "-save-temps"],
                    cwd=tmp, check=True, capture_output=True)
     isa = open(os.path.join(tmp, "pdsch_kernels-hip-amdgcn-amd-amdhsa-gfx950.s")).read().split("\n")
-begin = next(i for i, l in enumerate(isa) if l.startswith("_ZN5nrphy18codeblock_kernel_tILi8ELi4EEE"))
+begin = next(i for i, l in enumerate(isa) if l.startswith("_ZN5nrphy18codeblock_kernel_tILi%dELi%dEEE" % (QM, L)))
 end = next(i for i in range(begin, len(isa)) if "s_endpgm" in isa[i])
 k = isa[begin:end + 1]
-code = [l for l in k if l.startswith("\t") and not l.strip().startswith(";")]
-print("codeblock_kernel_t<8, 4>: %d instructions, v_readlane %d, v_writelane %d (the v_readlane are the wave reductions' row folds)" % (
-    len(code), sum("v_readlane" in l for l in code), sum("v_writelane" in l for l in code)))
-idx = [i for i, l in enumerate(k) if "v_pk_mul_f32" in l and ", s[" in l][-16:]
-start = max(i for i in range(idx[0]) if "Loop Header" in k[i])
-stop = next(i for i in range(idx[-1], len(k)) if "s_cbranch" in k[i] or "s_endpgm" in k[i])
-body = [l for l in k[start:stop + 1] if l.startswith("\t") and not l.strip().startswith(";")]
-print("grid loop, four ports (from its loop header to the branch behind the last product): %d instructions" % len(body))
-for what in ("v_pk_mul_f32", "v_pk_fma_f32", "v_pk_add_f32", "v_cvt_pk_bf16_f32", "buffer_store_dword", "ds_read", "global_load", "s_load", "v_readlane", "v_writelane"):
-    print("  %-20s %d" % (what, sum(what in l for l in body)))
-print("  scalar loads in the loop region (symbol change and the rare group that straddles a symbol; none per 64 RE, none of weights):")
-for l in body:
-    if "s_load" in l:
-        print("     " + l.strip())
+is_code = lambda l: l.startswith("\t") and not l.strip().startswith(";") and not l.strip().startswith(".")
+code = [l for l in k if is_code(l)]
+print("codeblock_kernel_t<%d, %d>: %d instructions, v_readlane %d, v_writelane %d (the v_readlane are the wave reductions' row folds)" % (
+    QM, L, len(code), sum("v_readlane" in l for l in code), sum("v_writelane" in l for l in code)))
+
+loops = []
+labels = [i for i, l in enumerate(k) if re.match(r"\.LBB\d+_\d+:", l)] + [len(k)]
+for n, i in enumerate(labels[:-1]):
+    if any("Loop Header" in k[j] for j in range(i, min(i + 5, len(k)))):
+        name = re.match(r"\.L(BB\d+_\d+):", k[i]).group(1)
+        marks = ("Header=%s " % name, "Parent Loop %s " % name)
+        mine = [m for m in range(len(labels) - 1) if any(w in l for l in k[labels[m]:min(labels[m] + 6, labels[m + 1])] for w in marks)] + [n]
+        loops.append((labels[min(mine)], labels[max(mine) + 1] - 1))
+products = 4 * L
+grid_loops = []
+for a, b in loops:
+    body = [l for l in k[a:b + 1] if is_code(l)]
+    n = sum("v_pk_mul_f32" in l and ", s[" in l for l in body)
+    if n == products:
+        grid_loops.append((a, b, body))
+VMEM = ("global_load", "buffer_load", "flat_load", "scratch_load")
+for a, b, body in grid_loops:
+    gather = any(w in l for l in body for w in VMEM)
+    print("\n64-RE loop, four ports, %s (listing lines %d-%d of the kernel): %d instructions" % (
+        "WITH the table gather" if gather else "no table gather", a, b, len(body)))
+    for what in ("v_pk_mul_f32", "v_pk_fma_f32", "v_pk_add_f32", "v_cvt_pk_bf16_f32", "buffer_store_dword", "ds_read", "s_load", "v_readlane", "v_writelane"):
+        print("  %-28s %d" % (what, sum(what in l for l in body)))
+    print("  %-28s %d" % ("vector-memory loads", sum(any(w in l for w in VMEM) for l in body)))
+    waits = [l.strip() for l in body if "s_waitcnt" in l and "vmcnt" in l]
+    print("  %-28s %d%s" % ("s_waitcnt with vmcnt", len(waits), "".join("\n     " + w for w in waits)))
+    print("  scalar loads in the loop region (symbol change and the group that straddles a symbol; none per 64 RE, none of weights):")
+    for l in body:
+        if "s_load" in l:
+            print("     " + l.strip())
+clean = [g for g in grid_loops if not any(w in l for l in g[2] for w in VMEM) and not any("s_waitcnt" in l and "vmcnt" in l for l in g[2])]
+print("\nRESULT: %d four-port 64-RE loops, %d without vector-memory load and without vmcnt wait" % (len(grid_loops), len(clean)))
diff --git a/srsran-edgeric-5g_amd/csrc/nrphy_host.cpp b/srsran-edgeric-5g_amd/csrc/nrphy_host.cpp
--- a/srsran-edgeric-5g_amd/csrc/nrphy_host.cpp
+++ b/srsran-edgeric-5g_amd/csrc/nrphy_host.cpp
@@ -308,6 +308,7 @@
   bool                  dmrs_separate = false;
   uint32_t              n_work = 0, n_dmrs = 0, n_cb = 0, n_crc_work = 0;
   uint32_t              lds_lin_words = 0, lds_symb_words = 0, lds_graph_words = 0, lds_u_words = 0;
+  uint32_t              cb_resident_wgs = 0;
   uint32_t              bucket_begin[CB_BUCKETS + 1] = {};
   static constexpr uint32_t MAX_AUX = 3;
   hipStream_t           aux_stream[MAX_AUX] = {};
@@ -617,6 +618,8 @@
   t.scr_parts_big     = number("NRPHY_SCR_PARTS_BIG", 0);
   t.extras_nt         = (uint32_t)number("NRPHY_EXTRAS_NT", 1);
   t.prologue_order    = (uint32_t)number("NRPHY_PROLOGUE_ORDER", 0);
+  t.cb_resident       = std::max(0, number("NRPHY_CB_RESIDENT", 0));
+  t.cb_stagger        = number("NRPHY_CB_STAGGER", 0) == 1 ? 1U : 0U;
   t.decoder_pairs     = number("NRPHY_DECODER_PAIRS", -1);
   t.decoder_msg       = number("NRPHY_DECODER_MSG", -1);
   t.decoder_ldsmsg    = number("NRPHY_DECODER_LDSMSG", -1);
@@ -962,6 +965,7 @@
       status = NRPHY_ERR_INVALID_PDU;
       break;
     }
+    pd.sym_any_table = std::count(pd.sym_kind, pd.sym_kind + NRPHY_NSYMB, (uint32_t)SYM_TABLE) != 0 ? 1U : 0U;
     nrphy_pdsch_derived_t d;
     derive(pdu, nof_re, d, enc ? &enc[i].nref : nullptr);
     if (d.lifting_size == 0 || d.nof_codeblocks > NRPHY_MAX_CODEBLOCKS || d.nof_codeblocks > nof_re ||
@@ -1302,6 +1306,18 @@
   }
   plan->lds_lin_words = std::max<uint32_t>(plan->lds_lin_words, 64);
   plan->lds_u_words = std::max<uint32_t>({256U * NRPHY_CRC_SLICES, NRPHY_CB_U_GRAPH_OFFSET + plan->lds_graph_words, 512U + plan->lds_symb_words});
+  if (ctx->tune.cb_resident != 0) {
+    const uint32_t positions = codeblock_positions(plan->n_work, plan->n_dmrs + plan->n_zero_work);
+    uint32_t       resident  = positions;
+    if (positions > ctx->nof_cus) {
+      const uint32_t per_cu = codeblock_workgroups_per_cu(plan->bucket_begin, codeblock_lds_bytes(plan->lds_lin_words, plan->lds_u_words));
+      resident              = per_cu != 0 ? per_cu * ctx->nof_cus : positions;
+    }
+    if (ctx->tune.cb_resident >= 2) {
+      resident = std::min<uint32_t>(resident, (uint32_t)ctx->tune.cb_resident);
+    }
+    plan->cb_resident_wgs = resident;
+  }
   *out = plan;
   return NRPHY_OK;
 }
@@ -1405,6 +1421,8 @@
   p.grid_nof_subc  = plan->grid_nof_subc;
   p.lds_lin_words  = plan->lds_lin_words;
   p.lds_u_words    = plan->lds_u_words;
+  p.cb_resident_wgs = plan->cb_resident_wgs;
+  p.cb_stagger      = plan->cb_resident_wgs != 0 ? ctx->tune.cb_stagger : 0U;
   p.extras_nt      = ctx->tune.extras_nt;
   p.prologue_order = ctx->tune.prologue_order;
 #ifdef NRPHY_PROBES
diff --git a/srsran-edgeric-5g_amd/csrc/nrphy_host_internal.h b/srsran-edgeric-5g_amd/csrc/nrphy_host_internal.h
--- a/srsran-edgeric-5g_amd/csrc/nrphy_host_internal.h
+++ b/srsran-edgeric-5g_amd/csrc/nrphy_host_internal.h
@@ -126,6 +126,8 @@
   int      scr_parts_big   = 0;
   uint32_t extras_nt       = 1;
   uint32_t prologue_order  = 0;
+  int      cb_resident     = 0;
+  uint32_t cb_stagger      = 0;
   int      decoder_pairs   = -1;
   int      decoder_msg     = -1;
   int      decoder_ldsmsg  = -1;
diff --git a/srsran-edgeric-5g_amd/csrc/nrphy_internal.h b/srsran-edgeric-5g_amd/csrc/nrphy_internal.h
--- a/srsran-edgeric-5g_amd/csrc/nrphy_internal.h
+++ b/srsran-edgeric-5g_amd/csrc/nrphy_internal.h
@@ -93,6 +93,7 @@
   uint32_t end_prb;
   uint32_t crc_first;
   uint32_t crc_count;
+  uint32_t sym_any_table;
 };
 
 struct CbWork {
@@ -188,6 +189,8 @@
   uint32_t           extras_nt;
   uint32_t           prologue_order;
   uint32_t           zero_fill;
+  uint32_t           cb_resident_wgs;
+  uint32_t           cb_stagger;
 };
 
 hipError_t launch_prologue(const PdschLaunch& p, const uint8_t* d_tb, hipStream_t stream);
@@ -200,6 +203,9 @@
 bool       codeblocks_take_bucket_launches(const PdschLaunch& p, const uint32_t* bucket_begin, int dispatch, uint32_t* nof_buckets);
 hipError_t launch_codeblocks(const PdschLaunch& p, const uint32_t* bucket_begin, int dispatch, const uint8_t* d_tb,
                              uint32_t* d_grid, uint32_t* d_cw_rm, uint32_t* d_cw_scr, const hipStream_t* streams, uint32_t n_streams);
+uint32_t   codeblock_workgroups_per_cu(const uint32_t* bucket_begin, size_t lds_bytes);
+uint32_t   codeblock_lds_bytes(uint32_t lds_lin_words, uint32_t lds_u_words);
+uint32_t   codeblock_positions(uint32_t n_work, uint32_t n_extras);
 hipError_t launch_dmrs(const PdschLaunch& p, uint32_t* d_grid, hipStream_t stream);
 hipError_t launch_ldpc_encode(const LiftedGraph* graphs, uint32_t graph, uint32_t kb, uint32_t zc, uint32_t n_cb,
                               const uint8_t* d_msg, uint32_t msg_stride, uint32_t out_bits, uint8_t* d_out,
diff --git a/srsran-edgeric-5g_amd/csrc/pdsch_kernels.hip b/srsran-edgeric-5g_amd/csrc/pdsch_kernels.hip
--- a/srsran-edgeric-5g_amd/csrc/pdsch_kernels.hip
+++ b/srsran-edgeric-5g_amd/csrc/pdsch_kernels.hip
@@ -1,4 +1,8 @@
 #include "ldpc_device.h"
+
+#include <map>
+#include <mutex>
+#include <tuple>
 
 #ifndef NRPHY_PHASE_A_STAGED
 #define NRPHY_PHASE_A_STAGED 1
@@ -491,44 +495,56 @@
 };
 
 template <int QM, int L>
-__device__ __forceinline__ uint32_t x1_bits(const PdschLaunch& p, const ChunkGeom& g, const ChunkMap& cm, uint32_t re_count,
-                                            uint32_t r)
-{
-  uint32_t bits = 0;
-  if (r < re_count) {
-    if (QM * L == 32 && cm.aligned) {
-      bits = (p.x1_words + cm.word0)[r];
-    } else {
-      bits = ext32(p.x1_words, g.bit0 + r * (uint32_t)(QM * L));
-    }
-  }
-  return bits;
-}
+struct ChunkX1 {
+  static constexpr uint32_t MAX_WORDS = (31u + (uint32_t)RE_CHUNK * (uint32_t)(QM * L) + 31u) / 32u + 1u;
+  static constexpr uint32_t TRIPS     = (MAX_WORDS + WAVE - 1u) / WAVE;
+  uint32_t w[TRIPS];
+
+  __device__ __forceinline__ void request(const uint32_t* x1_words, uint32_t word0, uint32_t need, uint32_t lane)
+  {
+#pragma unroll
+    for (uint32_t k = 0; k != TRIPS; ++k) {
+      const uint32_t i = lane + WAVE * k, src = word0 + i;
+      w[k] = i < need ? x1_words[src < (uint32_t)GOLD_X1_WORDS ? src : (uint32_t)GOLD_X1_WORDS - 1u] : 0u;
+    }
+  }
+  __device__ __forceinline__ void fold(uint32_t* x2, uint32_t need, uint32_t lane) const
+  {
+#pragma unroll
+    for (uint32_t k = 0; k != TRIPS; ++k) {
+      const uint32_t i = lane + WAVE * k;
+      if (i < need) {
+        x2[i] ^= w[k];
+      }
+    }
+    wave_lds_fence();
+  }
+};
 template <int QM, int L>
-__device__ __forceinline__ uint32_t x2_bits(const uint32_t* x2, const ChunkGeom& g, const ChunkMap& cm, uint32_t r)
+__device__ __forceinline__ uint32_t scr_bits(const uint32_t* scr, const ChunkGeom& g, const ChunkMap& cm, uint32_t r)
 {
   if (QM * L == 32 && cm.aligned) {
-    return x2[r];
-  }
-  return ext32(x2, (g.bit0 & 31u) + r * (uint32_t)(QM * L));
+    return scr[r];
+  }
+  return ext32(scr, (g.bit0 & 31u) + r * (uint32_t)(QM * L));
 }
 
 template <int QM, int L>
-__device__ __forceinline__ void re_bits(const PdschLaunch& p, const CbShared& sh, const ChunkGeom& g, const ChunkMap& cm,
-                                        uint32_t re_count, uint32_t r, uint32_t& bytes, uint32_t& gbits)
+__device__ __forceinline__ void re_bits(const CbShared& sh, const ChunkGeom& g, const ChunkMap& cm, uint32_t r, uint32_t& bytes,
+                                        uint32_t& gbits)
 {
   if constexpr (L == 4) {
     bytes = sh.symb[r];
   } else {
     bytes = ext32(sh.symb, 8u * r * L);
   }
-  gbits = x1_bits<QM, L>(p, g, cm, re_count, r) ^ x2_bits<QM, L>(sh.lin, g, cm, r);
-}
-
-template <int QM, int L, int P>
-__device__ __forceinline__ void phase_b_grid(const PdschLaunch& p, PduRef pd, const PduDev* __restrict__ pd_global,
-                                             const CbWork& wk, const CbShared& sh, const ChunkGeom& g, const ChunkMap& cm,
-                                             uint32_t first_gbits, uint32_t lane, uint32_t* __restrict__ d_grid)
+  gbits = scr_bits<QM, L>(sh.lin, g, cm, r);
+}
+
+template <int QM, int L, int P, bool TABLE>
+__device__ __forceinline__ void phase_b_grid(const PdschLaunch& p, PduRef pd, const CbWork& wk, const CbShared& sh,
+                                             const ChunkGeom& g, const ChunkMap& cm, uint32_t lane,
+                                             uint32_t* __restrict__ d_grid)
 {
   const size_t   grid_base   = (size_t)pd.grid_index * p.grid_nof_ports * NRPHY_NSYMB * p.grid_nof_subc;
   const uint32_t plane_words = NRPHY_NSYMB * p.grid_nof_subc;
@@ -557,60 +573,59 @@
   while (l_cur + 1u < NRPHY_NSYMB && cm.re0 >= pd.sym_re_start[l_cur + 1u]) {
     ++l_cur;
   }
-  uint32_t cur_start = pd.sym_re_start[l_cur], cur_end = pd.sym_re_start[l_cur + 1u];
-  uint32_t cur_arg = pd.sym_arg[l_cur], cur_row = l_cur * p.grid_nof_subc;
-  bool     cur_table = pd.sym_kind[l_cur] == SYM_TABLE;
-  uint32_t gbits_next = first_gbits;
+  uint32_t cur_end = pd.sym_re_start[l_cur + 1u];
+  uint32_t cur_sub = pd.sym_arg[l_cur] - pd.sym_re_start[l_cur], cur_row = l_cur * p.grid_nof_subc;
+  uint32_t cur_kind = TABLE ? pd.sym_kind[l_cur] : (uint32_t)SYM_CONTIGUOUS;
+  auto place = [&](uint32_t re_pdu, bool inside, uint32_t& subc, uint32_t& word_offset) {
+    subc = re_pdu + cur_sub;
+    if (TABLE && cur_kind == SYM_TABLE) {
+      subc = inside ? (uint32_t)p.re_table[subc] : 0u;
+    }
+    word_offset = cur_row + subc;
+  };
 
   for (uint32_t r0 = 0; r0 < wk.re_count; r0 += WAVE) {
     const uint32_t r        = r0 + lane;
-    const uint32_t x1       = gbits_next;
-    gbits_next              = x1_bits<QM, L>(p, g, cm, wk.re_count, r + WAVE);
     const uint32_t re_first = cm.re0 + r0;
     const uint32_t re_last  = re_first + ((wk.re_count - r0 < WAVE ? wk.re_count - r0 : WAVE) - 1u);
     if (re_first >= cur_end && l_cur + 1u < NRPHY_NSYMB) {
+      uint32_t start;
 #pragma unroll 1
       do {
         ++l_cur;
-        cur_start = cur_end;
-        cur_end   = pd.sym_re_start[l_cur + 1u];
+        start   = cur_end;
+        cur_end = pd.sym_re_start[l_cur + 1u];
       } while (re_first >= cur_end && l_cur + 1u < NRPHY_NSYMB);
-      cur_arg   = pd.sym_arg[l_cur];
+      cur_sub   = pd.sym_arg[l_cur] - start;
       cur_row   = l_cur * p.grid_nof_subc;
-      cur_table = pd.sym_kind[l_cur] == SYM_TABLE;
-    }
-    if (r >= wk.re_count) {
+      cur_kind  = TABLE ? pd.sym_kind[l_cur] : (uint32_t)SYM_CONTIGUOUS;
+    }
+    const uint32_t re_pdu = re_first + lane;
+    const bool     mine   = r < wk.re_count;
+    uint32_t       subc, word_offset;
+    place(re_pdu, mine && re_pdu < cur_end, subc, word_offset);
+#pragma unroll 1
+    while (re_last >= cur_end && l_cur + 1u < NRPHY_NSYMB) {
+      ++l_cur;
+      const uint32_t start = cur_end;
+      cur_end   = pd.sym_re_start[l_cur + 1u];
+      cur_sub   = pd.sym_arg[l_cur] - start;
+      cur_row   = l_cur * p.grid_nof_subc;
+      cur_kind  = TABLE ? pd.sym_kind[l_cur] : (uint32_t)SYM_CONTIGUOUS;
+      if (re_pdu >= start) {
+        place(re_pdu, mine && (re_pdu < cur_end || l_cur + 1u == NRPHY_NSYMB), subc, word_offset);
+      }
+    }
+    if (!mine) {
       continue;
     }
     __builtin_assume(r < (uint32_t)RE_CHUNK + WAVE);
-    const uint32_t gbits = x1 ^ x2_bits<QM, L>(sh.lin, g, cm, r);
+    const uint32_t gbits = scr_bits<QM, L>(sh.lin, g, cm, r);
     uint32_t bytes;
     if constexpr (L == 4) {
       bytes = sh.symb[r];
     } else {
       bytes = ext32(sh.symb, 8u * r * L);
-    }
-    const uint32_t re_pdu = re_first + lane;
-    uint32_t       subc, word_offset;
-    if (re_last < cur_end) {
-      subc = cur_arg + (re_pdu - cur_start);
-      if (cur_table) {
-        subc = (uint32_t)p.re_table[subc];
-      }
-      word_offset = cur_row + subc;
-    } else {
-      uint32_t l_sym = l_cur, start = cur_start, end = cur_end;
-#pragma unroll 1
-      while (re_pdu >= end && l_sym + 1u < NRPHY_NSYMB) {
-        ++l_sym;
-        start = end;
-        end   = pd_global->sym_re_start[l_sym + 1u];
-      }
-      subc = pd_global->sym_arg[l_sym] + (re_pdu - start);
-      if (pd_global->sym_kind[l_sym] == SYM_TABLE) {
-        subc = (uint32_t)p.re_table[subc];
-      }
-      word_offset = l_sym * p.grid_nof_subc + subc;
     }
     cf2 x[L];
 #pragma unroll
@@ -650,10 +665,27 @@
   }
 }
 
+template <int QM, int L, bool TABLE>
+__device__ __forceinline__ void phase_b_ports(const PdschLaunch& p, PduRef pd, const CbWork& wk, const CbShared& sh,
+                                              const ChunkGeom& g, const ChunkMap& cm, uint32_t nof_ports, uint32_t lane,
+                                              uint32_t* __restrict__ d_grid)
+{
+  if (nof_ports == 4u) {
+    phase_b_grid<QM, L, 4, TABLE>(p, pd, wk, sh, g, cm, lane, d_grid);
+  } else if (L <= 3 && nof_ports == 3u) {
+    phase_b_grid<QM, (L <= 3 ? L : 1), 3, TABLE>(p, pd, wk, sh, g, cm, lane, d_grid);
+  } else if (L <= 2 && nof_ports == 2u) {
+    phase_b_grid<QM, (L <= 2 ? L : 1), 2, TABLE>(p, pd, wk, sh, g, cm, lane, d_grid);
+  } else if (L == 1 && nof_ports == 1u) {
+    phase_b_grid<QM, 1, 1, TABLE>(p, pd, wk, sh, g, cm, lane, d_grid);
+  } else {
+    phase_b_grid<QM, L, 0, TABLE>(p, pd, wk, sh, g, cm, lane, d_grid);
+  }
+}
+
 template <int QM, int L>
-__device__ __forceinline__ void phase_b(const PdschLaunch& p, PduRef pd, const PduDev* __restrict__ pd_global,
-                                        const CbWork& wk, const CbShared& sh, const ChunkGeom& g, const ChunkMap& cm,
-                                        uint32_t first_gbits, uint32_t lane, uint32_t* __restrict__ d_grid,
+__device__ __forceinline__ void phase_b(const PdschLaunch& p, PduRef pd, const CbWork& wk, const CbShared& sh,
+                                        const ChunkGeom& g, const ChunkMap& cm, uint32_t lane, uint32_t* __restrict__ d_grid,
                                         uint32_t* __restrict__ d_cw_rm, uint32_t* __restrict__ d_cw_scr)
 {
   constexpr uint32_t LQ = QM * L;
@@ -661,7 +693,7 @@
     const uint64_t cw_bit0 = pd.cw_bit_offset + g.cw_cb + (uint64_t)wk.re_begin * LQ;
     for (uint32_t r = lane; r < wk.re_count; r += WAVE) {
       uint32_t bytes, gbits;
-      re_bits<QM, L>(p, sh, g, cm, wk.re_count, r, bytes, gbits);
+      re_bits<QM, L>(sh, g, cm, r, bytes, gbits);
       uint32_t v_rm = 0;
 #pragma unroll
       for (int l = 0; l != L; ++l) {
@@ -680,23 +712,38 @@
     return;
   }
   const uint32_t nof_ports = pd.nof_prg == 1 ? pd.nof_ports : 0u;
-  if (nof_ports == 4u) {
-    phase_b_grid<QM, L, 4>(p, pd, pd_global, wk, sh, g, cm, first_gbits, lane, d_grid);
-  } else if (L <= 3 && nof_ports == 3u) {
-    phase_b_grid<QM, (L <= 3 ? L : 1), 3>(p, pd, pd_global, wk, sh, g, cm, first_gbits, lane, d_grid);
-  } else if (L <= 2 && nof_ports == 2u) {
-    phase_b_grid<QM, (L <= 2 ? L : 1), 2>(p, pd, pd_global, wk, sh, g, cm, first_gbits, lane, d_grid);
-  } else if (L == 1 && nof_ports == 1u) {
-    phase_b_grid<QM, 1, 1>(p, pd, pd_global, wk, sh, g, cm, first_gbits, lane, d_grid);
+  if (pd.sym_any_table != 0) {
+    phase_b_ports<QM, L, true>(p, pd, wk, sh, g, cm, nof_ports, lane, d_grid);
   } else {
-    phase_b_grid<QM, L, 0>(p, pd, pd_global, wk, sh, g, cm, first_gbits, lane, d_grid);
-  }
-}
+    phase_b_ports<QM, L, false>(p, pd, wk, sh, g, cm, nof_ports, lane, d_grid);
+  }
+}
+
+struct CbArgs {
+  PdschLaunch    p;
+  const uint8_t* d_tb;
+  uint32_t*      d_grid;
+  uint32_t*      d_cw_rm;
+  uint32_t*      d_cw_scr;
+  uint32_t       nof_blocks;
+};
+
+struct CbArgsRef {
+  uint32_t lo, hi;
+  __device__ __forceinline__ CbArgs load() const
+  {
+#if defined(__HIP_DEVICE_COMPILE__)
+    return *reinterpret_cast<const CbArgs NRPHY_CONSTANT*>(((uintptr_t)(uint32_t)__builtin_amdgcn_readfirstlane((int)hi) << 32) |
+                                                          (uint32_t)__builtin_amdgcn_readfirstlane((int)lo));
+#else
+    return CbArgs{};
+#endif
+  }
+};
 
 template <int QM, int L>
-__device__ __forceinline__ void map_chunk(const PdschLaunch& p, PduRef pd, const PduDev* pd_global, const CbWork& wk,
-                                          uint32_t item, const CbShared& sh, uint32_t lane, uint32_t* d_grid,
-                                          uint32_t* d_cw_rm, uint32_t* d_cw_scr)
+__device__ __forceinline__ void map_chunk(const PdschLaunch& p, PduRef pd, const CbWork& wk, uint32_t item,
+                                          const CbShared& sh, uint32_t lane, const CbArgsRef& args)
 {
   const bool is_long = wk.cb >= pd.n_short;
   ChunkGeom  g;
@@ -710,8 +757,10 @@
   cm.re0     = g.cw_cb / (uint32_t)(QM * L) + wk.re_begin;
   cm.word0   = g.bit0 >> 5;
   cm.aligned = (g.bit0 & 31u) == 0;
-  const uint32_t seed_word   = lane < 31u ? p.scr_seed[(size_t)item * 32u + lane] : 0u;
-  const uint32_t first_gbits = x1_bits<QM, L>(p, g, cm, wk.re_count, lane);
+  const uint32_t  scr_words = ((g.bit0 & 31u) + wk.re_count * (uint32_t)(QM * L) + 31u) / 32u + 1u;
+  const uint32_t  seed_word = lane < 31u ? p.scr_seed[(size_t)item * 32u + lane] : 0u;
+  ChunkX1<QM, L> x1;
+  x1.request(p.x1_words, cm.word0, scr_words, lane);
   {
     const RmIndex rm = rm_index_init(pd);
     if (rm.rank0 + g.E > rm.n_valid) {
@@ -724,28 +773,29 @@
     return;
   }
   NRPHY_WG_TRACE_MARK(3);
-  static_assert((31u + (uint32_t)RE_CHUNK * 32u + 31u) / 32u + 1u <= GOLD_EXPAND_MAX_WORDS, "a work item's scrambling words");
-  gold_expand_seed_wave(sh.lin, seed_word, ((g.bit0 & 31u) + wk.re_count * (uint32_t)(QM * L) + 31u) / 32u + 1u, lane);
-  phase_b<QM, L>(p, pd, pd_global, wk, sh, g, cm, first_gbits, lane, d_grid, d_cw_rm, d_cw_scr);
+  static_assert(ChunkX1<QM, L>::MAX_WORDS <= GOLD_EXPAND_MAX_WORDS, "a work item's scrambling words");
+  gold_expand_seed_wave(sh.lin, seed_word, scr_words, lane);
+  x1.fold(sh.lin, scr_words, lane);
+  const CbArgs late = args.load();
+  phase_b<QM, L>(late.p, pd, wk, sh, g, cm, lane, late.d_grid, late.d_cw_rm, late.d_cw_scr);
 }
 
 template <int QM>
-__device__ __forceinline__ void map_chunk_layers(const PdschLaunch& p, PduRef pd, const PduDev* pd_global,
-                                                 const CbWork& wk, uint32_t item, const CbShared& sh, uint32_t lane,
-                                                 uint32_t* d_grid, uint32_t* d_cw_rm, uint32_t* d_cw_scr)
+__device__ __forceinline__ void map_chunk_layers(const PdschLaunch& p, PduRef pd, const CbWork& wk, uint32_t item,
+                                                 const CbShared& sh, uint32_t lane, const CbArgsRef& args)
 {
   switch (pd.nof_layers) {
     case 1:
-      map_chunk<QM, 1>(p, pd, pd_global, wk, item, sh, lane, d_grid, d_cw_rm, d_cw_scr);
+      map_chunk<QM, 1>(p, pd, wk, item, sh, lane, args);
       break;
     case 2:
-      map_chunk<QM, 2>(p, pd, pd_global, wk, item, sh, lane, d_grid, d_cw_rm, d_cw_scr);
+      map_chunk<QM, 2>(p, pd, wk, item, sh, lane, args);
       break;
     case 3:
-      map_chunk<QM, 3>(p, pd, pd_global, wk, item, sh, lane, d_grid, d_cw_rm, d_cw_scr);
+      map_chunk<QM, 3>(p, pd, wk, item, sh, lane, args);
       break;
     default:
-      map_chunk<QM, 4>(p, pd, pd_global, wk, item, sh, lane, d_grid, d_cw_rm, d_cw_scr);
+      map_chunk<QM, 4>(p, pd, wk, item, sh, lane, args);
       break;
   }
 }
@@ -936,11 +986,11 @@
   uint32_t  wave;
   uint32_t* lds;
 };
-__device__ __forceinline__ CbWave cb_wave(const PdschLaunch& p, uint32_t* dyn_lds)
+__device__ __forceinline__ CbWave cb_wave(const PdschLaunch& p, uint32_t* dyn_lds, uint32_t tid)
 {
   CbWave w;
-  w.lane = threadIdx.x % WAVE;
-  w.wave = (uint32_t)__builtin_amdgcn_readfirstlane((int)(threadIdx.x / WAVE));
+  w.lane = tid % WAVE;
+  w.wave = (uint32_t)__builtin_amdgcn_readfirstlane((int)(tid / WAVE));
   w.lds  = dyn_lds + w.wave * (p.lds_lin_words + p.lds_u_words);
   return w;
 }
@@ -949,13 +999,13 @@
   return (n_units + CB_WAVES - 1u) / CB_WAVES;
 }
 
-__device__ __forceinline__ bool extra_wave(const PdschLaunch& p, const CbWave& w, uint32_t* __restrict__ d_grid)
+__device__ __forceinline__ bool extra_wave(const PdschLaunch& p, const CbWave& w, uint32_t block, uint32_t* __restrict__ d_grid)
 {
   const uint32_t nb = cb_blocks(p.n_work);
-  if (blockIdx.x < nb) {
+  if (block < nb) {
     return false;
   }
-  const uint32_t extra = (blockIdx.x - nb) * CB_WAVES + w.wave;
+  const uint32_t extra = (block - nb) * CB_WAVES + w.wave;
   if (extra < p.n_dmrs_in_launch) {
     dmrs_wave(p, extra, d_grid, w.lane, w.lds);
   } else if (extra - p.n_dmrs_in_launch < p.n_zero_work) {
@@ -964,12 +1014,12 @@
   return true;
 }
 
-__device__ __forceinline__ uint32_t xcd_work_item(uint32_t n_work, const CbWave& w)
+__device__ __forceinline__ uint32_t xcd_work_item(uint32_t n_work, const CbWave& w, uint32_t block, uint32_t round)
 {
   const uint32_t nb  = cb_blocks(n_work);
-  const uint32_t xcd = blockIdx.x & 7u, turn = blockIdx.x >> 3;
+  const uint32_t xcd = block & 7u, turn = block >> 3;
   const uint32_t q = nb >> 3, r = nb & 7u;
-  const uint32_t item = (xcd * q + (xcd < r ? xcd : r) + turn) * CB_WAVES + w.wave;
+  const uint32_t item = (xcd * q + (xcd < r ? xcd : r) + turn) * CB_WAVES + ((w.wave + round) % CB_WAVES);
   return item < n_work ? item : n_work;
 }
 
@@ -996,81 +1046,95 @@
 }
 
 template <int QM, int L>
-__global__ __launch_bounds__(WAVE * CB_WAVES) void codeblock_kernel_t(PdschLaunch p, const uint8_t* __restrict__ d_tb,
-                                                              uint32_t* __restrict__ d_grid, uint32_t* __restrict__ d_cw_rm,
-                                                              uint32_t* __restrict__ d_cw_scr)
+__device__ __forceinline__ void codeblock_waves(uint32_t* dyn_lds)
+{
+  CbArgsRef args_v;
+  uint32_t  block_v = blockIdx.x, stride_v, round_v = 0;
+  {
+    const CbArgs NRPHY_CONSTANT* args = (const CbArgs NRPHY_CONSTANT*)__builtin_amdgcn_kernarg_segment_ptr();
+    args_v.lo = (uint32_t)reinterpret_cast<uintptr_t>(args);
+    args_v.hi = (uint32_t)(reinterpret_cast<uintptr_t>(args) >> 32);
+    stride_v  = args->nof_blocks;
+    if (args->p.cb_stagger != 0) {
+      const uint32_t slot = (uint32_t)__builtin_amdgcn_s_getreg((3 << 11) | 4) & 7u;
+      for (uint32_t i = 0; i != slot; ++i) {
+        __builtin_amdgcn_s_sleep(75);
+      }
+    }
+  }
+  asm volatile("" : "+v"(args_v.lo), "+v"(args_v.hi), "+v"(block_v), "+v"(stride_v), "+v"(round_v));
+#pragma unroll 1
+  for (;; block_v += stride_v, round_v += 1u) {
+    uint32_t tid = threadIdx.x;
+    asm volatile("" : "+v"(tid));
+    const uint32_t block = (uint32_t)__builtin_amdgcn_readfirstlane((int)block_v);
+    const CbArgs   a     = args_v.load();
+    if (NRPHY_STAGE(a.p) == 10 ||
+        block >= cb_blocks(a.p.n_work) + cb_blocks(a.d_grid ? a.p.n_dmrs_in_launch + a.p.n_zero_work : 0u)) {
+      return;
+    }
+    const PdschLaunch&   p = a.p;
+    const uint8_t* const d_tb = a.d_tb;
+    uint32_t* const      d_grid = a.d_grid;
+    const CbWave         w    = cb_wave(p, dyn_lds, tid);
+    const uint32_t       lane = w.lane;
+    CbShared             sh;
+    sh.lin   = w.lds;
+    sh.u     = w.lds + p.lds_lin_words;
+    sh.symb  = sh.u + CB_U_QAM_WORDS;
+    sh.graph = sh.u + CB_U_GRAPH_OFFSET;
+    sh.ldpc  = reinterpret_cast<LdpcScratch*>(sh.u + LDPC_DBL_WORDS);
+    if (extra_wave(p, w, block, d_grid)) {
+      continue;
+    }
+    const uint32_t item = xcd_work_item(p.n_work, w, block, (uint32_t)__builtin_amdgcn_readfirstlane((int)round_v));
+    if (item == p.n_work) {
+      continue;
+    }
+    NRPHY_WG_TRACE_MARK(0);
+    NRPHY_WG_TRACE_WHERE(3);
+    const auto*  wkc = to_constant(&p.work[item]);
+    const CbWork wk  = {wkc->pdu, wkc->cb, wkc->re_begin, wkc->re_count};
+    PduRef       pd  = *to_constant(&p.pdus[wk.pdu]);
+    if (!codeblock_front(p, pd, wk, sh, d_tb, lane)) {
+      continue;
+    }
+    if constexpr (QM != 0) {
+      map_chunk<QM, L>(p, pd, wk, p.work_base + item, sh, lane, args_v);
+    } else {
+      switch (pd.qm) {
+        case 2:
+          map_chunk_layers<2>(p, pd, wk, p.work_base + item, sh, lane, args_v);
+          break;
+        case 4:
+          map_chunk_layers<4>(p, pd, wk, p.work_base + item, sh, lane, args_v);
+          break;
+        case 6:
+          map_chunk_layers<6>(p, pd, wk, p.work_base + item, sh, lane, args_v);
+          break;
+        default:
+          map_chunk_layers<8>(p, pd, wk, p.work_base + item, sh, lane, args_v);
+          break;
+      }
+    }
+    NRPHY_WG_TRACE_MARK(6);
+  }
+}
+
+template <int QM, int L>
+__global__ __launch_bounds__(WAVE * CB_WAVES) __attribute__((amdgpu_num_sgpr(98))) void codeblock_kernel_t(CbArgs)
 {
   extern __shared__ __attribute__((aligned(16))) uint32_t dyn_lds[];
-  const CbWave   w    = cb_wave(p, dyn_lds);
-  const uint32_t lane = w.lane;
-  CbShared       sh;
-  sh.lin   = w.lds;
-  sh.u     = w.lds + p.lds_lin_words;
-  sh.symb  = sh.u + CB_U_QAM_WORDS;
-  sh.graph = sh.u + CB_U_GRAPH_OFFSET;
-  sh.ldpc  = reinterpret_cast<LdpcScratch*>(sh.u + LDPC_DBL_WORDS);
-  if (NRPHY_STAGE(p) == 10 || extra_wave(p, w, d_grid)) {
-    return;
-  }
-  const uint32_t item = xcd_work_item(p.n_work, w);
-  if (item == p.n_work) {
-    return;
-  }
-  NRPHY_WG_TRACE_MARK(0);
-  NRPHY_WG_TRACE_WHERE(3);
-  const auto*  wkc = to_constant(&p.work[item]);
-  const CbWork wk  = {wkc->pdu, wkc->cb, wkc->re_begin, wkc->re_count};
-  PduRef       pd  = *to_constant(&p.pdus[wk.pdu]);
-  if (!codeblock_front(p, pd, wk, sh, d_tb, lane)) {
-    return;
-  }
-  map_chunk<QM, L>(p, pd, &p.pdus[wk.pdu], wk, p.work_base + item, sh, lane, d_grid, d_cw_rm, d_cw_scr);
-  NRPHY_WG_TRACE_MARK(6);
-}
-
-__global__ __launch_bounds__(WAVE * CB_WAVES) void codeblock_kernel(PdschLaunch p, const uint8_t* __restrict__ d_tb,
-                                                         uint32_t* __restrict__ d_grid, uint32_t* __restrict__ d_cw_rm,
-                                                         uint32_t* __restrict__ d_cw_scr)
+  codeblock_waves<QM, L>(dyn_lds);
+}
+
+__global__ __launch_bounds__(WAVE * CB_WAVES) void codeblock_kernel(CbArgs)
 {
   extern __shared__ __attribute__((aligned(16))) uint32_t dyn_lds[];
-  const CbWave   w    = cb_wave(p, dyn_lds);
-  const uint32_t lane = w.lane;
-  CbShared       sh;
-  sh.lin   = w.lds;
-  sh.u     = w.lds + p.lds_lin_words;
-  sh.symb  = sh.u + CB_U_QAM_WORDS;
-  sh.graph = sh.u + CB_U_GRAPH_OFFSET;
-  sh.ldpc  = reinterpret_cast<LdpcScratch*>(sh.u + LDPC_DBL_WORDS);
-  if (NRPHY_STAGE(p) == 10 || extra_wave(p, w, d_grid)) {
-    return;
-  }
-  const uint32_t item = xcd_work_item(p.n_work, w);
-  if (item == p.n_work) {
-    return;
-  }
-  const auto*  wkc = to_constant(&p.work[item]);
-  const CbWork wk  = {wkc->pdu, wkc->cb, wkc->re_begin, wkc->re_count};
-  PduRef       pd  = *to_constant(&p.pdus[wk.pdu]);
-  if (!codeblock_front(p, pd, wk, sh, d_tb, lane)) {
-    return;
-  }
-  switch (pd.qm) {
-    case 2:
-      map_chunk_layers<2>(p, pd, &p.pdus[wk.pdu], wk, p.work_base + item, sh, lane, d_grid, d_cw_rm, d_cw_scr);
-      break;
-    case 4:
-      map_chunk_layers<4>(p, pd, &p.pdus[wk.pdu], wk, p.work_base + item, sh, lane, d_grid, d_cw_rm, d_cw_scr);
-      break;
-    case 6:
-      map_chunk_layers<6>(p, pd, &p.pdus[wk.pdu], wk, p.work_base + item, sh, lane, d_grid, d_cw_rm, d_cw_scr);
-      break;
-    default:
-      map_chunk_layers<8>(p, pd, &p.pdus[wk.pdu], wk, p.work_base + item, sh, lane, d_grid, d_cw_rm, d_cw_scr);
-      break;
-  }
-}
-
-typedef void (*CodeblockKernel)(PdschLaunch, const uint8_t*, uint32_t*, uint32_t*, uint32_t*);
+  codeblock_waves<0, 0>(dyn_lds);
+}
+
+typedef void (*CodeblockKernel)(CbArgs);
 
 static CodeblockKernel bucket_kernel(uint32_t bucket)
 {
@@ -1092,18 +1156,67 @@
   return !(dispatch == 1 || (dispatch == 0 && n > 1 && p.n_work < CB_MIXED_MAX_WORK));
 }
 
+uint32_t codeblock_workgroups_per_cu(const uint32_t* bucket_begin, size_t lds_bytes)
+{
+  static std::mutex                                              mutex;
+  static std::map<std::tuple<int, uint32_t, size_t>, uint32_t> known;
+  int device = 0;
+  if (hipGetDevice(&device) != hipSuccess) {
+    return 0;
+  }
+  uint32_t fewest = ~0u;
+  for (uint32_t k = 0; k != CB_BUCKETS + 1u; ++k) {
+    if (k != CB_BUCKETS && bucket_begin[k + 1] == bucket_begin[k]) {
+      continue;
+    }
+    const std::lock_guard<std::mutex> lock(mutex);
+    const auto                        key = std::make_tuple(device, k, lds_bytes);
+    auto                              it  = known.find(key);
+    if (it == known.end()) {
+      int n = 0;
+      if (hipOccupancyMaxActiveBlocksPerMultiprocessor(&n, k == CB_BUCKETS ? codeblock_kernel : bucket_kernel(k), WAVE * CB_WAVES,
+                                                       lds_bytes) != hipSuccess || n < 0) {
+        (void)hipGetLastError();
+        n = 0;
+      }
+      it = known.insert({key, (uint32_t)n}).first;
+    }
+    fewest = it->second < fewest ? it->second : fewest;
+  }
+  return fewest == ~0u ? 0u : fewest;
+}
+
+uint32_t codeblock_lds_bytes(uint32_t lds_lin_words, uint32_t lds_u_words)
+{
+  return 4u * (lds_lin_words + lds_u_words) * CB_WAVES;
+}
+
+uint32_t codeblock_positions(uint32_t n_work, uint32_t n_extras)
+{
+  return cb_blocks(n_work) + cb_blocks(n_extras);
+}
+
+static uint32_t resident_grid(uint32_t positions, uint32_t share)
+{
+  if (share == 0 || share >= positions) {
+    return positions;
+  }
+  return share >= 8u ? share & ~7u : share;
+}
+
 hipError_t launch_codeblocks(const PdschLaunch& p, const uint32_t* bucket_begin, int dispatch, const uint8_t* d_tb,
                              uint32_t* d_grid, uint32_t* d_cw_rm, uint32_t* d_cw_scr, const hipStream_t* streams, uint32_t n_streams)
 {
   if (p.n_work == 0) {
     return hipSuccess;
   }
-  const size_t   lds_bytes = 4u * (size_t)(p.lds_lin_words + p.lds_u_words) * CB_WAVES;
+  const size_t   lds_bytes = codeblock_lds_bytes(p.lds_lin_words, p.lds_u_words);
   const uint32_t extras    = d_grid ? p.n_dmrs_in_launch + p.n_zero_work : 0u;
   uint32_t       nof_buckets = 0;
   if (!codeblocks_take_bucket_launches(p, bucket_begin, dispatch, &nof_buckets)) {
-    hipLaunchKernelGGL(codeblock_kernel, dim3(cb_blocks(p.n_work) + cb_blocks(extras)), dim3(WAVE * CB_WAVES), lds_bytes, streams[0], p,
-                       d_tb, d_grid, d_cw_rm, d_cw_scr);
+    const uint32_t blocks = resident_grid(codeblock_positions(p.n_work, extras), p.cb_resident_wgs);
+    hipLaunchKernelGGL(codeblock_kernel, dim3(blocks), dim3(WAVE * CB_WAVES), lds_bytes, streams[0],
+                       CbArgs{p, d_tb, d_grid, d_cw_rm, d_cw_scr, blocks});
     return hipGetLastError();
   }
   uint32_t order[CB_BUCKETS], n_order = 0;
@@ -1115,6 +1228,10 @@
       }
       order[k] = b;
     }
+  }
+  uint64_t all_positions = 0;
+  for (uint32_t i = 0; i != n_order; ++i) {
+    all_positions += codeblock_positions(bucket_begin[order[i] + 1] - bucket_begin[order[i]], i == 0 ? extras : 0u);
   }
   for (uint32_t i = 0; i != n_order; ++i) {
     const uint32_t b = order[i], n = bucket_begin[b + 1] - bucket_begin[b];
@@ -1126,9 +1243,15 @@
       q.n_dmrs_in_launch = 0;
       q.n_zero_work      = 0;
     }
-    const uint32_t blocks = cb_blocks(n) + (i == 0 ? cb_blocks(extras) : 0u);
-    hipLaunchKernelGGL(bucket_kernel(b), dim3(blocks), dim3(WAVE * CB_WAVES), lds_bytes, streams[n_streams > 1 ? i % n_streams : 0], q,
-                       d_tb, d_grid, d_cw_rm, d_cw_scr);
+    const uint32_t positions = codeblock_positions(n, i == 0 ? extras : 0u);
+    uint32_t share = p.cb_resident_wgs;
+    if (share != 0 && n_streams > 1 && n_order > 1) {
+      share = (uint32_t)((uint64_t)share * positions / all_positions);
+      share = share != 0 ? share : 1u;
+    }
+    const uint32_t blocks = resident_grid(positions, share);
+    hipLaunchKernelGGL(bucket_kernel(b), dim3(blocks), dim3(WAVE * CB_WAVES), lds_bytes,
+                       streams[n_streams > 1 ? i % n_streams : 0], CbArgs{q, d_tb, d_grid, d_cw_rm, d_cw_scr, blocks});
     const hipError_t e = hipGetLastError();
     if (e != hipSuccess) {
       return e;
```
